# carlhenrikrolf/gym-cellular

Hardware: NVIDIA B200
Metric: env-steps/sec (higher is better)
Workload: dtype int8/int32 state, f32 reward

## Files before the change

gym_cellular_b200/_lib.py:

```python
import ctypes as C
import os

_PKG = os.path.dirname(os.path.abspath(__file__))
LIB_PATH = os.path.join(os.environ.get("GC_B200_LIB_DIR") or os.path.join(_PKG, "lib"), "libgymcellular_b200.so")

ABI_VERSION = 2
KIND_CELLULAR, KIND_GRIDWORLD = 0, 1
F_NOISE, F_RNG_EPISODIC, F_REWARD_LOG2, F_GENERIC_KERNEL = 1, 4, 16, 32
MAX_CELLS, MAX_LEVELS, N_STATS = 16, 8, 8
STAT_STEPS, STAT_UNSAFE, STAT_COUNT, STAT_TRUNCATED, STAT_REWARD_Q24 = range(5)
OK, ERR_INVALID, ERR_CUDA, ERR_STATE, ERR_ACTION = 0, -1, -2, -3, -4
POLICY_RANDOM, POLICY_TABLE = 0, 1

EXPORTS = ["gc_abi_version", "gc_last_error", "gc_create", "gc_destroy", "gc_set_tables", "gc_set_final_obs",
           "gc_set_global_step", "gc_get_global_step", "gc_sync_global_step", "gc_launch_count", "gc_reset", "gc_step",
           "gc_bind_step", "gc_step_bound", "gc_step_many", "gc_prepare_step_many", "gc_step_host", "gc_rollout", "gc_collect", "gc_poll_status", "gc_encode",
           "gc_decode", "gc_encode_mixed", "gc_decode_mixed", "gc_reset_packed", "gc_step_packed", "gc_bind_step_packed",
           "gc_step_host_packed", "gc_pack_cells", "gc_unpack_cells"]
FLAG_UNSAFE, FLAG_TRUNCATED, FLAG_COUNT_SHIFT = 1, 2, 2


class GcConfig(C.Structure):
    _fields_ = [("struct_size", C.c_uint32), ("kind", C.c_int32), ("device", C.c_int32),
                ("n_cells", C.c_int32), ("n_states", C.c_int32), ("n_actions", C.c_int32),
                ("max_episode_steps", C.c_int32), ("flags", C.c_uint32),
                ("n_envs", C.c_int64), ("ld", C.c_int64), ("env_id_offset", C.c_int64),
                ("seed", C.c_uint64), ("noise_prob", C.c_double), ("dispersal_prob", C.c_double)]


class GcCellTables(C.Structure):
    _fields_ = [("move", C.c_void_p), ("noisy", C.c_void_p), ("draws", C.c_void_p),
                ("reward", C.c_void_p), ("side_effects", C.c_void_p), ("counted", C.c_void_p),
                ("initial_state", C.c_void_p), ("reward_noisy", C.c_void_p), ("radix", C.c_void_p)]


class GcRecord(C.Structure):
    _fields_ = [("struct_size", C.c_uint32), ("obs", C.c_void_p), ("action", C.c_void_p), ("reward", C.c_void_p),
                ("flags", C.c_void_p), ("next_obs", C.c_void_p)]


class GcError(RuntimeError):
    def __init__(self, code, message):
        super().__init__(f"libgymcellular_b200 error {code}: {message}")
        self.code = code
        self.message = message


_lib = None


def load():
    global _lib
    if _lib is not None:
        return _lib
    if not os.path.exists(LIB_PATH):
        raise ImportError(
            f"{LIB_PATH} is missing: the CUDA extension has not been built and there is no CPU "
            "fallback.  Run `python -m gym_cellular_b200.build` (needs nvcc).")
    L = C.CDLL(LIB_PATH)
    vp, i64 = C.c_void_p, C.c_int64
    L.gc_abi_version.restype = C.c_int
    L.gc_last_error.restype = C.c_char_p
    L.gc_create.argtypes = [C.POINTER(GcConfig), C.POINTER(vp)]
    L.gc_destroy.argtypes = [vp]
    L.gc_set_tables.argtypes = [vp, C.POINTER(GcCellTables)]
    L.gc_set_final_obs.argtypes = [vp, vp]
    L.gc_set_global_step.argtypes = [vp, i64]
    L.gc_get_global_step.argtypes = [vp]
    L.gc_get_global_step.restype = i64
    L.gc_sync_global_step.argtypes = [vp, vp]
    L.gc_launch_count.argtypes = [vp]
    L.gc_launch_count.restype = i64
    L.gc_reset.argtypes = [vp] * 6
    L.gc_step.argtypes = [vp, i64, i64] + [vp] * 13
    L.gc_bind_step.argtypes = [vp, C.c_int32] + [vp] * 11
    L.gc_step_bound.argtypes = [vp, C.c_int32, vp]
    L.gc_step_host.argtypes = [vp] * 21 + [i64]
    L.gc_rollout.argtypes = [vp, C.c_int32, C.c_int32] + [vp] * 8
    L.gc_collect.argtypes = [vp, C.c_int32, C.c_int32, vp, C.c_double, vp, vp, vp, C.POINTER(GcRecord), vp, vp]
    L.gc_poll_status.argtypes = [vp, vp]
    L.gc_encode.argtypes = [C.c_int, i64, i64, C.c_int32, C.c_int32, vp, vp, vp]
    L.gc_decode.argtypes = [C.c_int, i64, i64, C.c_int32, C.c_int32, vp, vp, vp]
    i32 = C.c_int32
    L.gc_step_many.argtypes = [vp, vp, i32, i32, vp]
    L.gc_prepare_step_many.argtypes = [vp, vp, i32]
    L.gc_encode_mixed.argtypes = [C.c_int, i64, i64, i32, vp, vp, vp, vp, vp]
    L.gc_decode_mixed.argtypes = [C.c_int, i64, i64, i32, vp, vp, vp, vp, vp]
    L.gc_reset_packed.argtypes = [vp] * 6
    L.gc_step_packed.argtypes = [vp, i64, i64] + [vp] * 10
    L.gc_bind_step_packed.argtypes = [vp, i32] + [vp] * 9
    L.gc_step_host_packed.argtypes = [vp] * 13 + [i64]
    L.gc_pack_cells.argtypes = [C.c_int, i64, i64, i32, vp, vp, vp]
    L.gc_unpack_cells.argtypes = [C.c_int, i64, i64, i32, vp, vp, vp]
    if L.gc_abi_version() != ABI_VERSION:
        raise ImportError(f"ABI version mismatch: library {L.gc_abi_version()} != binding {ABI_VERSION}")
    _lib = L
    return L


def check(rc):
    if rc != 0:
        raise GcError(rc, load().gc_last_error().decode())
```

gym_cellular_b200/csrc/gc_api.cu:

```cuda
#include <cmath>
#include <cstdarg>
#include <cstdio>
#include <cstdlib>
#include <cstring>
#include <memory>
#include <new>

#include <nvtx3/nvToolsExt.h>

#include "gc_internal.h"

namespace {

thread_local char g_err[512] = "";

struct NvtxRange {
    explicit NvtxRange(const char *name) { nvtxRangePushA(name); }
    ~NvtxRange() { nvtxRangePop(); }
};
#define GC_NVTX(name) NvtxRange nvtx_range_(name)

int fail(int code, const char *fmt, ...)
{
    va_list ap;
    va_start(ap, fmt);
    vsnprintf(g_err, sizeof(g_err), fmt, ap);
    va_end(ap);
    return code;
}

#define GC_CUDA(call)                                                                         \
    do {                                                                                      \
        cudaError_t e_ = (call);                                                              \
        if (e_ != cudaSuccess)                                                                \
            return fail(GC_ERR_CUDA, "%s failed: %s (%s:%d)", #call, cudaGetErrorString(e_),   \
                        __FILE__, __LINE__);                                                  \
    } while (0)

constexpr int kHostStreams = 3;
constexpr int kManyGraphs = 4;
constexpr int kManyGraphSteps = 16;

class DeviceGuard {
public:
    explicit DeviceGuard(int device) : prev_(-1), err_(cudaSuccess)
    {
        err_ = cudaGetDevice(&prev_);
        if (err_ == cudaSuccess && prev_ != device) err_ = cudaSetDevice(device); else prev_ = -1;
    }
    ~DeviceGuard() { if (prev_ >= 0) cudaSetDevice(prev_); }
    cudaError_t error() const { return err_; }
private:
    int prev_;
    cudaError_t err_;
};

#define GC_ON_DEVICE(dev)                                                                      \
    DeviceGuard guard_(dev);                                                                   \
    if (guard_.error() != cudaSuccess)                                                         \
        return fail(GC_ERR_CUDA, "cannot switch to device %d: %s", (dev), cudaGetErrorString(guard_.error()))

unsigned long long threshold_of(double p)
{
    if (!(p > 0.0)) return 0ull;
    if (p >= 1.0) return 1ull << 32;
    return static_cast<unsigned long long>(std::ceil(p * 4294967296.0));
}

}

struct gc_env {
    gc_config cfg;
    CellTables tab;
    GridParams grid;
    bool tables_set;
    int n_sm;
    int64_t global_step;
    int64_t launches;
    unsigned long long *d_status;
    uint32_t *d_step;
    uint32_t *d_done;
    uint2 *d_pair_lut;
    uint2 *d_packed_lut;
    uint2 *d_pair8_lut;
    bool pair8_ok;
    int8_t *final_state;
    bool fast_ok;
    StepIO bound[GC_MAX_BINDINGS];
    PackedIO bound_packed[GC_MAX_BINDINGS];
    int bound_set[GC_MAX_BINDINGS];
    cudaStream_t hstream[kHostStreams];
    cudaEvent_t hevent[kHostStreams];
    bool host_ready;
    struct ManyGraph { int32_t slots[GC_MAX_BINDINGS]; int32_t n_slots, n_steps; cudaGraphExec_t exec; } many[kManyGraphs];
    int n_many;
};

namespace {

int check_env(const gc_env *env)
{
    if (!env) return fail(GC_ERR_INVALID, "env is NULL");
    return GC_OK;
}

int check_range(const gc_env *env, int64_t begin, int64_t count)
{
    const int64_t n = env->cfg.n_envs;
    if (begin < 0 || count < 0 || begin + count > n)
        return fail(GC_ERR_INVALID, "env range [%lld, %lld) outside [0, %lld)", (long long)begin,
                    (long long)(begin + count), (long long)n);
    if (begin % 16 != 0)
        return fail(GC_ERR_INVALID, "env_begin must be a multiple of 16");
    if ((begin + count) % 16 != 0 && begin + count != n)
        return fail(GC_ERR_INVALID, "env range must end on a multiple of 16 or at n_envs");
    return GC_OK;
}

StepIO make_io(const gc_env *env, int64_t begin, int64_t count, const int8_t *actions, int8_t *state,
               int32_t *t, float *reward, uint32_t *index, uint8_t *terminated, uint8_t *truncated,
               uint8_t *unsafe, uint8_t *count_out, int8_t *se_row, const double *replay, int64_t *stats)
{
    StepIO io;
    io.actions = actions; io.state = state; io.t = t; io.reward = reward; io.index = index;
    io.terminated = terminated; io.truncated = truncated; io.unsafe = unsafe; io.count = count_out;
    io.se_row = se_row; io.replay = replay;
    io.final_state = env->final_state;
    io.stats = reinterpret_cast<unsigned long long *>(stats);
    io.status = env->d_status;
    io.begin = begin; io.end = begin + count; io.ld = env->cfg.ld;
    io.env_id_offset = env->cfg.env_id_offset;
    io.seed_lo = static_cast<uint32_t>(env->cfg.seed);
    io.seed_hi = static_cast<uint32_t>(env->cfg.seed >> 32);
    for (int r = 0; r < 10; ++r) {
        io.round_key[2 * r] = io.seed_lo + static_cast<uint32_t>(r) * 0x9E3779B9u;
        io.round_key[2 * r + 1] = io.seed_hi + static_cast<uint32_t>(r) * 0xBB67AE85u;
    }
    io.rng_counter = static_cast<uint32_t>(env->global_step);
    io.step_ctr = env->d_step;
    io.done_ctr = nullptr;
    io.episodic = (env->cfg.flags & GC_F_RNG_EPISODIC) ? 1 : 0;
    io.max_episode_steps = env->cfg.max_episode_steps;
    return io;
}

PackedIO make_packed_io(const gc_env *env, int64_t begin, int64_t count, const uint32_t *actions, uint32_t *state,
                        int32_t *t, float *reward, uint32_t *index, uint8_t *flags, uint32_t *final_state,
                        uint32_t *se_row, int64_t *stats)
{
    PackedIO io;
    io.actions = actions; io.state = state; io.t = t; io.reward = reward; io.index = index; io.flags = flags;
    io.final_state = final_state; io.se_row = se_row;
    io.stats = reinterpret_cast<unsigned long long *>(stats);
    io.status = env->d_status;
    io.begin = begin; io.end = begin + count; io.ld = env->cfg.ld;
    io.env_id_offset = env->cfg.env_id_offset;
    const uint32_t lo = static_cast<uint32_t>(env->cfg.seed), hi = static_cast<uint32_t>(env->cfg.seed >> 32);
    for (int r = 0; r < 10; ++r) {
        io.round_key[2 * r] = lo + static_cast<uint32_t>(r) * 0x9E3779B9u;
        io.round_key[2 * r + 1] = hi + static_cast<uint32_t>(r) * 0xBB67AE85u;
    }
    io.rng_counter = static_cast<uint32_t>(env->global_step);
    io.step_ctr = env->d_step;
    io.done_ctr = nullptr;
    io.episodic = (env->cfg.flags & GC_F_RNG_EPISODIC) ? 1 : 0;
    io.max_episode_steps = env->cfg.max_episode_steps;
    return io;
}

int check_packed(const gc_env *env)
{
    if (env->cfg.kind != GC_KIND_CELLULAR || !env->fast_ok)
        return fail(GC_ERR_INVALID, "the packed layout covers the cellular family with n_states, n_actions <= 4 "
                                    "(and equal side-effect tables for the cells j >= 2)");
    return GC_OK;
}

int launch_packed(gc_env *env, const PackedIO &io, cudaStream_t st)
{
    if (io.end <= io.begin) return GC_OK;
    const bool draws = (env->cfg.flags & GC_F_NOISE) && env->tab.noise_thr_nz;
    cudaError_t e = gc_launch_cell_packed_step(env->tab, io, env->d_packed_lut, draws, env->n_sm, st);
    if (e != cudaSuccess) return fail(GC_ERR_CUDA, "packed step kernel launch failed: %s", cudaGetErrorString(e));
    env->launches += 1;
    return GC_OK;
}

void drop_many_graphs(gc_env *env)
{
    for (int i = 0; i < env->n_many; ++i)
        if (env->many[i].exec) cudaGraphExecDestroy(env->many[i].exec);
    env->n_many = 0;
}

struct HostDrain {
    gc_env *env;
    bool done = false;
    ~HostDrain()
    {
        if (done) return;
        for (int i = 0; i < kHostStreams; ++i) cudaStreamSynchronize(env->hstream[i]);
        cudaGetLastError();
    }
};

int host_streams(gc_env *env)
{
    if (!env->host_ready) {
        for (int i = 0; i < kHostStreams; ++i) {
            GC_CUDA(cudaStreamCreateWithFlags(&env->hstream[i], cudaStreamNonBlocking));
            GC_CUDA(cudaEventCreateWithFlags(&env->hevent[i], cudaEventDisableTiming));
        }
        env->host_ready = true;
    }
    return GC_OK;
}

int tick_global_step(gc_env *env, cudaStream_t st)
{
    cudaError_t e = gc_launch_tick(env->d_step, 1u, st);
    if (e != cudaSuccess) return fail(GC_ERR_CUDA, "step-counter kernel launch failed: %s", cudaGetErrorString(e));
    env->global_step += 1;
    return GC_OK;
}

int launch_step(gc_env *env, const StepIO &io, cudaStream_t st)
{
    if (io.end <= io.begin) return GC_OK;
    cudaError_t e;
    if (env->cfg.kind == GC_KIND_CELLULAR) {
        const bool draws = (env->cfg.flags & GC_F_NOISE) && env->tab.noise_thr_nz;
        const int mode = io.replay ? GC_RNG_REPLAY : (draws ? GC_RNG_PHILOX : GC_RNG_NONE);
        static const bool use_tma = [] { const char *v = std::getenv("GC_B200_TMA"); return v && v[0] == '1'; }();
        if (env->fast_ok && use_tma && mode == GC_RNG_NONE && !io.se_row && !io.final_state && env->cfg.n_cells >= 8)
            e = gc_launch_cell_tma_step(env->tab, io, env->d_pair_lut, env->n_sm, st);
        else if (env->fast_ok)
            e = gc_launch_cell_pair_step(env->tab, io, env->d_pair_lut, mode, env->n_sm, st);
        else if (env->pair8_ok && mode != GC_RNG_REPLAY)
            e = gc_launch_cell_pair8_step(env->tab, io, env->d_pair8_lut, mode, env->n_sm, st);
        else
            e = gc_launch_cell_step(env->tab, io, mode, env->n_sm, st);
    } else {
        e = gc_launch_grid_step(env->grid, io, io.replay ? GC_RNG_REPLAY : GC_RNG_PHILOX, env->n_sm, st);
    }
    if (e != cudaSuccess) return fail(GC_ERR_CUDA, "step kernel launch failed: %s", cudaGetErrorString(e));
    env->launches += 1;
    return GC_OK;
}

}

extern "C" {

int gc_abi_version(void) { return GC_ABI_VERSION; }

const char *gc_last_error(void) { return g_err; }

int gc_create(const gc_config *cfg, gc_env **out)
{
    GC_NVTX("gc_create");
    if (!cfg || !out) return fail(GC_ERR_INVALID, "cfg/out is NULL");
    if (cfg->struct_size != sizeof(gc_config))
        return fail(GC_ERR_INVALID, "gc_config.struct_size %u != %zu (ABI mismatch)", cfg->struct_size, sizeof(gc_config));
    if (cfg->n_envs < 1) return fail(GC_ERR_INVALID, "n_envs must be >= 1");
    if (cfg->ld < cfg->n_envs || cfg->ld % 16 != 0)
        return fail(GC_ERR_INVALID, "ld must be a multiple of 16 and >= n_envs");
    if (cfg->max_episode_steps < 0) return fail(GC_ERR_INVALID, "max_episode_steps must be >= 0");
    if (cfg->n_cells >= 1 && cfg->ld > (int64_t(1) << 31) / cfg->n_cells)
        return fail(GC_ERR_INVALID, "n_cells * ld must not exceed 2^31 (%d cells: at most %lld envs per handle)", cfg->n_cells,
                    (long long)((int64_t(1) << 31) / cfg->n_cells));
    if (cfg->env_id_offset < 0 || cfg->env_id_offset % 4 != 0)
        return fail(GC_ERR_INVALID, "env_id_offset must be a non-negative multiple of 4");
    if (cfg->kind == GC_KIND_CELLULAR) {
        if (cfg->n_cells < 1 || cfg->n_cells > GC_MAX_CELLS)
            return fail(GC_ERR_INVALID, "n_cells must be in 1..%d", GC_MAX_CELLS);
        if (cfg->n_states < 2 || cfg->n_states > GC_MAX_LEVELS || cfg->n_actions < 1 || cfg->n_actions > GC_MAX_LEVELS)
            return fail(GC_ERR_INVALID, "n_states must be in 2..%d and n_actions in 1..%d", GC_MAX_LEVELS, GC_MAX_LEVELS);
        if (cfg->n_cells * std::log2((double)cfg->n_states) > 32.0 + 1e-9)
            return fail(GC_ERR_INVALID, "n_states^n_cells does not fit the 32-bit tabular index");
    } else if (cfg->kind == GC_KIND_GRIDWORLD) {
        if (cfg->n_cells != 2 || cfg->n_states != 20 || cfg->n_actions != 5)
            return fail(GC_ERR_INVALID, "grid world is 2 jurisdictions x 20 codes x 5 actions");
    } else {
        return fail(GC_ERR_INVALID, "unknown kind %d", cfg->kind);
    }
    int n_dev = 0;
    GC_CUDA(cudaGetDeviceCount(&n_dev));
    if (cfg->device < 0 || cfg->device >= n_dev)
        return fail(GC_ERR_INVALID, "device %d not in [0, %d)", cfg->device, n_dev);
    GC_ON_DEVICE(cfg->device);
    int n_sm = 0;
    GC_CUDA(cudaDeviceGetAttribute(&n_sm, cudaDevAttrMultiProcessorCount, cfg->device));
    gc_env *env = new (std::nothrow) gc_env();
    if (!env) return fail(GC_ERR_INVALID, "out of host memory");
    std::memset(env, 0, sizeof(*env));
    env->cfg = *cfg;
    env->n_sm = n_sm;
    env->grid.dispersal_thr = threshold_of(cfg->dispersal_prob);
    env->grid.dispersal_thr_nz = env->grid.dispersal_thr != 0ull;
    env->grid.dispersal_thr_m1 = env->grid.dispersal_thr_nz ? static_cast<uint32_t>(env->grid.dispersal_thr - 1ull) : 0u;
    env->grid.dispersal_prob = cfg->dispersal_prob;
    env->tables_set = (cfg->kind == GC_KIND_GRIDWORLD);
    cudaError_t e = cudaMalloc(&env->d_status, 2 * sizeof(unsigned long long));
    if (e == cudaSuccess) e = cudaMemset(env->d_status, 0, 2 * sizeof(unsigned long long));
    if (e == cudaSuccess) {
        env->d_step = reinterpret_cast<uint32_t *>(env->d_status + 1);
        env->d_done = env->d_step + 1;
    }
    if (e == cudaSuccess && cfg->kind == GC_KIND_GRIDWORLD) {
        std::unique_ptr<uint32_t[]> lut(new (std::nothrow) uint32_t[GC_GRID_LUT_ENTRIES]);
        uint32_t *d_lut = nullptr;
        if (!lut) e = cudaErrorMemoryAllocation;
        if (e == cudaSuccess) {
            gc_build_grid_lut(lut.get());
            e = cudaMalloc(&d_lut, GC_GRID_LUT_ALLOC * sizeof(uint32_t));
        }
        if (e == cudaSuccess) e = cudaMemset(d_lut, 0, GC_GRID_LUT_ALLOC * sizeof(uint32_t));
        if (e == cudaSuccess) e = cudaMemcpy(d_lut, lut.get(), GC_GRID_LUT_ENTRIES * sizeof(uint32_t), cudaMemcpyHostToDevice);
        env->grid.lut = d_lut;
    }
    if (e != cudaSuccess) {
        if (env->d_status) cudaFree(env->d_status);
        if (env->grid.lut) cudaFree(const_cast<uint32_t *>(env->grid.lut));
        delete env;
        return fail(GC_ERR_CUDA, "device table allocation failed: %s", cudaGetErrorString(e));
    }
    *out = env;
    return GC_OK;
}

int gc_destroy(gc_env *env)
{
    if (!env) return GC_OK;
    DeviceGuard guard_(env->cfg.device);
    drop_many_graphs(env);
    if (env->host_ready)
        for (int i = 0; i < kHostStreams; ++i) {
            cudaStreamDestroy(env->hstream[i]);
            cudaEventDestroy(env->hevent[i]);
        }
    if (env->d_status) cudaFree(env->d_status);
    if (env->d_pair_lut) cudaFree(env->d_pair_lut);
    if (env->d_packed_lut) cudaFree(env->d_packed_lut);
    if (env->d_pair8_lut) cudaFree(env->d_pair8_lut);
    if (env->grid.lut) cudaFree(const_cast<uint32_t *>(env->grid.lut));
    delete env;
    return GC_OK;
}

int gc_set_tables(gc_env *env, const gc_cell_tables *t)
{
    GC_NVTX("gc_set_tables");
    if (int rc = check_env(env)) return rc;
    if (env->cfg.kind != GC_KIND_CELLULAR) return fail(GC_ERR_INVALID, "tables apply to the cellular family only");
    if (!t || !t->move || !t->reward || !t->side_effects || !t->counted || !t->initial_state)
        return fail(GC_ERR_INVALID, "move, reward, side_effects, counted and initial_state are required");
    const int C = env->cfg.n_cells, S = env->cfg.n_states, A = env->cfg.n_actions;
    const bool noise = (env->cfg.flags & GC_F_NOISE) != 0;
    if (noise && (!t->noisy || !t->draws)) return fail(GC_ERR_INVALID, "GC_F_NOISE needs the noisy and draws tables");
    CellTables tab;
    std::memset(&tab, 0, sizeof(tab));
    for (int s = 0; s < S; ++s)
        for (int a = 0; a < A; ++a) {
            const int mv = t->move[s * A + a];
            const int nz = t->noisy ? t->noisy[s * A + a] : mv;
            const int dr = (noise && t->draws) ? (t->draws[s * A + a] != 0) : 0;
            if (mv < 0 || mv >= S || nz < 0 || nz >= S)
                return fail(GC_ERR_INVALID, "move/noisy[%d][%d] outside [0, %d)", s, a, S);
            tab.sa[s * GC_LVL_PAD + a] = (uint32_t)mv | ((uint32_t)nz << 4) | ((uint32_t)dr << 8);
            tab.reward[s * GC_LVL_PAD + a] = t->reward[s * A + a];
            tab.reward_noisy[s * GC_LVL_PAD + a] = (t->reward_noisy ? t->reward_noisy : t->reward)[s * A + a];
        }
    for (int j = 0; j < C; ++j)
        for (int s0 = 0; s0 < S; ++s0)
            for (int sp = 0; sp < S; ++sp) {
                const int code = t->side_effects[(j * S + s0) * S + sp];
                if (code < 0 || code > 2) return fail(GC_ERR_INVALID, "side_effects code %d not in {0,1,2}", code);
                tab.se[j][s0 * GC_LVL_PAD + sp] = (uint8_t)code;
            }
    bool ragged = false;
    if (t->radix) {
        double bits = 0.0;
        for (int c = 0; c < C; ++c) {
            if (t->radix[c] < 1 || t->radix[c] > S) return fail(GC_ERR_INVALID, "radix[%d] = %d not in 1..n_states", c, t->radix[c]);
            bits += std::log2((double)t->radix[c]);
            ragged = ragged || t->radix[c] != S;
        }
        if (bits > 32.0 + 1e-9) return fail(GC_ERR_INVALID, "the ragged state space does not fit the 32-bit tabular index");
    }
    uint32_t place = 1, init_index = 0;
    for (int c = 0; c < C; ++c) {
        const int lv = t->initial_state[c];
        const int radix_c = t->radix ? t->radix[c] : S;
        if (lv < 0 || lv >= radix_c) return fail(GC_ERR_INVALID, "initial_state[%d] outside [0, %d)", c, radix_c);
        tab.place[c] = place;
        tab.init[c] = (int8_t)lv;
        init_index += (uint32_t)lv * place;
        place *= (uint32_t)radix_c;
    }
    tab.init_index = init_index;
    for (int s = 0; s < S; ++s) if (t->counted[s]) tab.counted_mask |= 1u << s;
    tab.n_cells = C; tab.n_states = S; tab.n_actions = A;
    tab.reward_log2 = (env->cfg.flags & GC_F_REWARD_LOG2) ? 1 : 0;
    tab.noise_thr = threshold_of(env->cfg.noise_prob);
    tab.noise_prob = env->cfg.noise_prob;

    tab.noise_thr_nz = tab.noise_thr != 0ull;
    tab.noise_thr_m1 = tab.noise_thr_nz ? static_cast<uint32_t>(tab.noise_thr - 1ull) : 0u;
    {
        uint32_t k16 = static_cast<uint32_t>(tab.noise_thr >> 16), r16 = static_cast<uint32_t>(tab.noise_thr & 0xFFFFull);
        if (k16 > 65535u) { k16 = 65535u; r16 = 1u << 16; }
        tab.noise_kk15 = (k16 & 0x7FFFu) * 0x00010001u;
        tab.noise_kmask = (k16 & 0x8000u) ? 0xFFFFFFFFu : 0u;
        tab.noise_kk = k16 * 0x00010001u;
        tab.noise_r16 = r16;
    }

    bool fast_ok = S <= 4 && A <= 4 && !ragged && !(env->cfg.flags & GC_F_GENERIC_KERNEL);
    for (int j = 3; j < C && fast_ok; ++j)
        if (std::memcmp(t->side_effects + (size_t)j * S * S, t->side_effects + (size_t)2 * S * S, (size_t)S * S) != 0)
            fast_ok = false;
    if (fast_ok) {
        uint2 lut[GC_PAIR_LUT_ENTRIES];
        gc_build_pair_lut(t, C, S, A, noise, lut, &tab.unsafe_rows);
        uint32_t p4 = 1;
        for (int i = 0; i < 4; ++i) { tab.place4[i] = p4; p4 *= (uint32_t)S; }
        GC_ON_DEVICE(env->cfg.device);
        if (!env->d_pair_lut) GC_CUDA(cudaMalloc(&env->d_pair_lut, sizeof(lut)));
        GC_CUDA(cudaMemcpy(env->d_pair_lut, lut, sizeof(lut), cudaMemcpyHostToDevice));
        gc_build_packed_lut(t, C, S, A, noise, lut);
        tab.init_packed = 0;
        for (int c = 0; c < C; ++c) tab.init_packed |= (uint32_t)(tab.init[c] & 3) << (2 * c);
        if (!env->d_packed_lut) GC_CUDA(cudaMalloc(&env->d_packed_lut, sizeof(lut)));
        GC_CUDA(cudaMemcpy(env->d_packed_lut, lut, sizeof(lut), cudaMemcpyHostToDevice));
    }
    bool pair8_ok = !fast_ok && S <= 8 && A <= 8 && !ragged && !(env->cfg.flags & GC_F_GENERIC_KERNEL);
    for (int j = 3; j < C && pair8_ok; ++j)
        if (std::memcmp(t->side_effects + (size_t)j * S * S, t->side_effects + (size_t)2 * S * S, (size_t)S * S) != 0)
            pair8_ok = false;
    if (pair8_ok) {
        std::unique_ptr<uint2[]> lut8(new (std::nothrow) uint2[GC_PAIR8_ENTRIES]);
        if (!lut8) return fail(GC_ERR_INVALID, "out of host memory");
        gc_build_pair8_lut(t, C, S, A, noise, lut8.get(), &tab.unsafe_rows8, &tab.unsafe01_rows8);
        GC_ON_DEVICE(env->cfg.device);
        if (!env->d_pair8_lut) GC_CUDA(cudaMalloc(&env->d_pair8_lut, GC_PAIR8_ENTRIES * sizeof(uint2)));
        GC_CUDA(cudaMemcpy(env->d_pair8_lut, lut8.get(), GC_PAIR8_ENTRIES * sizeof(uint2), cudaMemcpyHostToDevice));
    }
    drop_many_graphs(env);
    env->tab = tab;
    env->fast_ok = fast_ok;
    env->pair8_ok = pair8_ok;
    env->tables_set = true;
    return GC_OK;
}

int gc_set_final_obs(gc_env *env, int8_t *final_state)
{
    if (int rc = check_env(env)) return rc;
    env->final_state = final_state;
    drop_many_graphs(env);
    for (int i = 0; i < GC_MAX_BINDINGS; ++i)
        if (env->bound_set[i] == 1) env->bound[i].final_state = final_state;
    return GC_OK;
}

int gc_set_global_step(gc_env *env, int64_t step)
{
    if (int rc = check_env(env)) return rc;
    env->global_step = step;
    const uint32_t v = static_cast<uint32_t>(step);
    GC_ON_DEVICE(env->cfg.device);
    GC_CUDA(cudaMemcpy(env->d_step, &v, sizeof(v), cudaMemcpyHostToDevice));
    return GC_OK;
}

int64_t gc_get_global_step(const gc_env *env) { return env ? env->global_step : -1; }

int gc_sync_global_step(gc_env *env, void *stream)
{
    if (int rc = check_env(env)) return rc;
    GC_ON_DEVICE(env->cfg.device);
    uint32_t v = 0;
    GC_CUDA(cudaMemcpyAsync(&v, env->d_step, sizeof(v), cudaMemcpyDeviceToHost, static_cast<cudaStream_t>(stream)));
    GC_CUDA(cudaStreamSynchronize(static_cast<cudaStream_t>(stream)));
    env->global_step = (env->global_step & ~0xFFFFFFFFll) | v;
    return GC_OK;
}

int64_t gc_launch_count(const gc_env *env) { return env ? env->launches : -1; }

int gc_reset(gc_env *env, const uint8_t *mask, int8_t *state, int32_t *t, uint32_t *index, void *stream)
{
    GC_NVTX("gc_reset");
    if (int rc = check_env(env)) return rc;
    if (!env->tables_set) return fail(GC_ERR_STATE, "gc_set_tables has not been called");
    if (!state || !t) return fail(GC_ERR_INVALID, "state/t is NULL");
    GC_ON_DEVICE(env->cfg.device);
    int8_t init[GC_MAX_CELLS] = {0};
    uint32_t init_index;
    if (env->cfg.kind == GC_KIND_GRIDWORLD) {
        init[0] = 15; init[1] = 18; init_index = 15 + 20 * 18;
    } else {
        std::memcpy(init, env->tab.init, sizeof(init));
        init_index = env->tab.init_index;
    }
    const int64_t n_pad = (env->cfg.n_envs + 3) / 4 * 4;
    cudaError_t e = gc_launch_reset(env->cfg.n_cells, init, init_index, mask, state, t, index, n_pad,
                                    env->cfg.ld, static_cast<cudaStream_t>(stream));
    if (e != cudaSuccess) return fail(GC_ERR_CUDA, "reset kernel launch failed: %s", cudaGetErrorString(e));
    env->launches += 1;
    return GC_OK;
}

int gc_step(gc_env *env, int64_t env_begin, int64_t env_count, const int8_t *actions, int8_t *state,
            int32_t *t, float *reward, uint32_t *index, uint8_t *terminated, uint8_t *truncated,
            uint8_t *unsafe, uint8_t *count, int8_t *se_row, const double *replay_u, int64_t *stats,
            void *stream)
{
    GC_NVTX("gc_step");
    if (int rc = check_env(env)) return rc;
    if (!env->tables_set) return fail(GC_ERR_STATE, "gc_set_tables has not been called");
    if (!actions || !state || !t || !reward || !index || !terminated || !truncated || !unsafe || !count)
        return fail(GC_ERR_INVALID, "a required device pointer is NULL");
    if (int rc = check_range(env, env_begin, env_count)) return rc;
    GC_ON_DEVICE(env->cfg.device);
    StepIO io = make_io(env, env_begin, env_count, actions, state, t, reward, index, terminated,
                        truncated, unsafe, count, se_row, replay_u, stats);
    const bool full = env_begin == 0 && env_count == env->cfg.n_envs;
    if (full) io.done_ctr = env->d_done;
    if (int rc = launch_step(env, io, static_cast<cudaStream_t>(stream))) return rc;
    if (full) {
        env->global_step += 1;
    } else if (env_begin + env_count == env->cfg.n_envs) {
        if (int rc = tick_global_step(env, static_cast<cudaStream_t>(stream))) return rc;
    }
    return GC_OK;
}

int gc_bind_step(gc_env *env, int32_t slot, const int8_t *actions, int8_t *state, int32_t *t, float *reward,
                 uint32_t *index, uint8_t *terminated, uint8_t *truncated, uint8_t *unsafe, uint8_t *count,
                 int8_t *se_row, int64_t *stats)
{
    if (int rc = check_env(env)) return rc;
    if (slot < 0 || slot >= GC_MAX_BINDINGS) return fail(GC_ERR_INVALID, "slot must be in [0, %d)", GC_MAX_BINDINGS);
    if (!actions || !state || !t || !reward || !index || !terminated || !truncated || !unsafe || !count)
        return fail(GC_ERR_INVALID, "a required device pointer is NULL");
    env->bound[slot] = make_io(env, 0, env->cfg.n_envs, actions, state, t, reward, index, terminated, truncated,
                               unsafe, count, se_row, nullptr, stats);
    env->bound[slot].done_ctr = env->d_done;
    env->bound_set[slot] = 1;
    drop_many_graphs(env);
    return GC_OK;
}

namespace {
int launch_bound(gc_env *env, int32_t slot, cudaStream_t st)
{
    if (slot < 0 || slot >= GC_MAX_BINDINGS || !env->bound_set[slot])
        return fail(GC_ERR_INVALID, "no binding in slot %d", slot);
    if (int rc = env->bound_set[slot] == 2 ? launch_packed(env, env->bound_packed[slot], st)
                                           : launch_step(env, env->bound[slot], st))
        return rc;
    env->global_step += 1;
    return GC_OK;
}
}

int gc_step_bound(gc_env *env, int32_t slot, void *stream)
{
    if (!env) return fail(GC_ERR_INVALID, "gc_step_bound: env is NULL");
    if (!env->tables_set) return fail(GC_ERR_STATE, "gc_set_tables has not been called");
    GC_ON_DEVICE(env->cfg.device);
    return launch_bound(env, slot, static_cast<cudaStream_t>(stream));
}

namespace {
const gc_env::ManyGraph *many_graph(gc_env *env, const int32_t *slots, int32_t n_slots)
{
    for (int i = 0; i < env->n_many; ++i)
        if (env->many[i].n_slots == n_slots && std::memcmp(env->many[i].slots, slots, n_slots * sizeof(int32_t)) == 0)
            return &env->many[i];
    if (n_slots > GC_MAX_BINDINGS || host_streams(env) != GC_OK) return nullptr;
    if (env->n_many == kManyGraphs) drop_many_graphs(env);
    static const int graph_steps = [] {
        const char *v = std::getenv("GC_B200_STEP_MANY_GRAPH_STEPS");
        const int k = v ? std::atoi(v) : 0;
        return k > 0 ? k : kManyGraphSteps;
    }();
    const int32_t passes = (graph_steps + n_slots - 1) / n_slots;
    cudaStream_t cap = env->hstream[0];
    const int64_t launches = env->launches, step = env->global_step;
    if (cudaStreamBeginCapture(cap, cudaStreamCaptureModeRelaxed) != cudaSuccess) { cudaGetLastError(); return nullptr; }
    int rc = GC_OK;
    for (int32_t p = 0; p < passes && rc == GC_OK; ++p)
        for (int32_t i = 0; i < n_slots && rc == GC_OK; ++i) rc = launch_bound(env, slots[i], cap);
    cudaGraph_t graph = nullptr;
    cudaError_t e = cudaStreamEndCapture(cap, &graph);
    env->launches = launches; env->global_step = step;
    cudaGraphExec_t exec = nullptr;
    if (rc == GC_OK && e == cudaSuccess && graph) e = cudaGraphInstantiate(&exec, graph, 0);
    if (graph) cudaGraphDestroy(graph);
    if (rc != GC_OK || e != cudaSuccess || !exec) { cudaGetLastError(); return nullptr; }
    gc_env::ManyGraph &m = env->many[env->n_many++];
    std::memcpy(m.slots, slots, n_slots * sizeof(int32_t));
    m.n_slots = n_slots;
    m.n_steps = passes * n_slots;
    m.exec = exec;
    return &m;
}

constexpr int64_t kManyGraphMaxEnvs = 1 << 21;

bool many_graphs_enabled(const gc_env *env)
{
    static const bool on = [] { const char *v = std::getenv("GC_B200_STEP_MANY_GRAPH"); return !(v && v[0] == '0'); }();
    return on && env->cfg.n_envs <= kManyGraphMaxEnvs;
}

bool many_fusable(const gc_env *env, const int32_t *slots, int32_t n_slots)
{
    const char *v = std::getenv("GC_B200_STEP_MANY_FUSED");
    if ((v && v[0] == '0') || env->cfg.n_envs > kManyGraphMaxEnvs || env->final_state) return false;
    if (env->cfg.kind == GC_KIND_CELLULAR) {
        if (!env->fast_ok || env->cfg.n_cells > GC_MANY_MAX_CELLS) return false;
    }
    const int layout = env->bound_set[slots[0]];
    for (int32_t i = 0; i < n_slots; ++i)
        if (env->bound_set[slots[i]] != layout) return false;
    if (layout == 2) {
        if (env->cfg.kind != GC_KIND_CELLULAR) return false;
        const PackedIO &a = env->bound_packed[slots[0]];
        for (int32_t i = 1; i < n_slots; ++i) {
            const PackedIO &b = env->bound_packed[slots[i]];
            if (a.state != b.state || a.t != b.t || a.reward != b.reward || a.index != b.index || a.flags != b.flags ||
                a.se_row != b.se_row || a.stats != b.stats || a.final_state != b.final_state)
                return false;
        }
        return a.final_state == nullptr;
    }
    const StepIO &a = env->bound[slots[0]];
    for (int32_t i = 1; i < n_slots; ++i) {
        const StepIO &b = env->bound[slots[i]];
        if (a.state != b.state || a.t != b.t || a.reward != b.reward || a.index != b.index || a.terminated != b.terminated ||
            a.truncated != b.truncated || a.unsafe != b.unsafe || a.count != b.count || a.se_row != b.se_row ||
            a.stats != b.stats || a.final_state != b.final_state)
            return false;
    }
    return a.final_state == nullptr && a.replay == nullptr;
}

constexpr int32_t kManyFusedMaxSteps = 4096;

int launch_many_fused(gc_env *env, const int32_t *slots, int32_t n_slots, int32_t first, int32_t n_steps, cudaStream_t st)
{
    const bool draws = (env->cfg.flags & GC_F_NOISE) && env->tab.noise_thr_nz;
    if (env->bound_set[slots[0]] == 2) {
        PackedManyIO pio;
        pio.io = env->bound_packed[slots[0]];
        for (int32_t i = 0; i < GC_MAX_BINDINGS; ++i)
            pio.tape[i] = i < n_slots ? env->bound_packed[slots[(first + i) % n_slots]].actions : nullptr;
        pio.n_tape = n_slots;
        pio.n_steps = n_steps;
        const cudaError_t e = gc_launch_cell_packed_many(env->tab, pio, env->d_packed_lut, draws, env->n_sm, st);
        if (e != cudaSuccess) return fail(GC_ERR_CUDA, "many-step kernel launch failed: %s", cudaGetErrorString(e));
        env->launches += 1;
        env->global_step += n_steps;
        return GC_OK;
    }
    ManyIO mio;
    mio.io = env->bound[slots[0]];
    for (int32_t i = 0; i < n_slots; ++i) mio.tape[i] = env->bound[slots[(first + i) % n_slots]].actions;
    for (int32_t i = n_slots; i < GC_MAX_BINDINGS; ++i) mio.tape[i] = nullptr;
    mio.n_tape = n_slots;
    mio.n_steps = n_steps;
    const cudaError_t e = env->cfg.kind == GC_KIND_CELLULAR
        ? gc_launch_cell_pair_many(env->tab, mio, env->d_pair_lut, draws ? GC_RNG_PHILOX : GC_RNG_NONE, env->n_sm, st)
        : gc_launch_grid_many(env->grid, mio, env->n_sm, st);
    if (e != cudaSuccess) return fail(GC_ERR_CUDA, "many-step kernel launch failed: %s", cudaGetErrorString(e));
    env->launches += 1;
    env->global_step += n_steps;
    return GC_OK;
}
}

int gc_prepare_step_many(gc_env *env, const int32_t *slots, int32_t n_slots)
{
    if (!env || !slots || n_slots < 1) return fail(GC_ERR_INVALID, "gc_prepare_step_many: bad arguments");
    if (!env->tables_set) return fail(GC_ERR_STATE, "gc_set_tables has not been called");
    for (int32_t i = 0; i < n_slots; ++i)
        if (slots[i] < 0 || slots[i] >= GC_MAX_BINDINGS || !env->bound_set[slots[i]])
            return fail(GC_ERR_INVALID, "no binding in slot %d", slots[i]);
    GC_ON_DEVICE(env->cfg.device);
    if (n_slots <= GC_MAX_BINDINGS && many_fusable(env, slots, n_slots)) return GC_OK;
    if (many_graphs_enabled(env) && n_slots >= 2) many_graph(env, slots, n_slots);
    return GC_OK;
}

int gc_step_many(gc_env *env, const int32_t *slots, int32_t n_slots, int32_t n_steps, void *stream)
{
    GC_NVTX("gc_step_many");
    if (!env || !slots || n_slots < 1 || n_steps < 0) return fail(GC_ERR_INVALID, "gc_step_many: bad arguments");
    if (!env->tables_set) return fail(GC_ERR_STATE, "gc_set_tables has not been called");
    GC_ON_DEVICE(env->cfg.device);
    cudaStream_t st = static_cast<cudaStream_t>(stream);
    int32_t done = 0;
    for (int32_t i = 0; i < n_slots; ++i)
        if (slots[i] < 0 || slots[i] >= GC_MAX_BINDINGS || !env->bound_set[slots[i]])
            return fail(GC_ERR_INVALID, "no binding in slot %d", slots[i]);
    if (n_steps >= 2 && n_slots <= GC_MAX_BINDINGS && many_fusable(env, slots, n_slots)) {
        for (; done < n_steps;) {
            const int32_t k = n_steps - done < kManyFusedMaxSteps ? n_steps - done : kManyFusedMaxSteps;
            if (int rc = launch_many_fused(env, slots, n_slots, done % n_slots, k, st)) return rc;
            done += k;
        }
        return GC_OK;
    }
    cudaStreamCaptureStatus capturing = cudaStreamCaptureStatusNone;
    if (many_graphs_enabled(env) && n_slots >= 2 && n_steps >= 2 * n_slots &&
        cudaStreamIsCapturing(st, &capturing) == cudaSuccess && capturing == cudaStreamCaptureStatusNone) {
        if (const gc_env::ManyGraph *m = many_graph(env, slots, n_slots)) {
            for (; done + m->n_steps <= n_steps; done += m->n_steps) {
                GC_CUDA(cudaGraphLaunch(m->exec, st));
                env->launches += m->n_steps;
                env->global_step += m->n_steps;
            }
        }
    }
    for (int32_t i = done; i < n_steps; ++i)
        if (int rc = launch_bound(env, slots[i % n_slots], st)) return rc;
    return GC_OK;
}

int gc_step_host(gc_env *env, const int8_t *h_actions, int8_t *h_state, float *h_reward,
                 uint32_t *h_index, uint8_t *h_terminated, uint8_t *h_truncated, uint8_t *h_unsafe,
                 uint8_t *h_count, int8_t *h_se_row, int8_t *d_actions, int8_t *d_state, int32_t *d_t,
                 float *d_reward, uint32_t *d_index, uint8_t *d_terminated, uint8_t *d_truncated,
                 uint8_t *d_unsafe, uint8_t *d_count, int8_t *d_se_row, int64_t *d_stats,
                 int64_t chunk_envs)
{
    GC_NVTX("gc_step_host");
    if (int rc = check_env(env)) return rc;
    if (!env->tables_set) return fail(GC_ERR_STATE, "gc_set_tables has not been called");
    if (!h_actions || !d_actions || !d_state || !d_t || !d_reward || !d_index || !d_terminated ||
        !d_truncated || !d_unsafe || !d_count)
        return fail(GC_ERR_INVALID, "a required pointer is NULL");
    if (h_se_row && !d_se_row) return fail(GC_ERR_INVALID, "h_se_row needs d_se_row");
    GC_ON_DEVICE(env->cfg.device);
    if (int rc = host_streams(env)) return rc;
    const int64_t n = env->cfg.n_envs, ld = env->cfg.ld;
    const int C = env->cfg.n_cells;
    if (chunk_envs <= 0) chunk_envs = 1 << 20;
    chunk_envs = (chunk_envs + 15) / 16 * 16;
    HostDrain drain{env};
    int k = 0;
    for (int64_t b = 0; b < n; b += chunk_envs, ++k) {
        const int64_t cnt = (b + chunk_envs < n) ? chunk_envs : (n - b);
        const int64_t cnt_pad = (cnt + 3) / 4 * 4;
        cudaStream_t st = env->hstream[k % kHostStreams];
        GC_CUDA(cudaMemcpy2DAsync(d_actions + b, ld, h_actions + b, ld, cnt_pad, C, cudaMemcpyHostToDevice, st));
        const StepIO io = make_io(env, b, cnt, d_actions, d_state, d_t, d_reward, d_index, d_terminated,
                                  d_truncated, d_unsafe, d_count, d_se_row, nullptr, d_stats);
        if (int rc = launch_step(env, io, st)) return rc;
        if (h_state) GC_CUDA(cudaMemcpy2DAsync(h_state + b, ld, d_state + b, ld, cnt, C, cudaMemcpyDeviceToHost, st));
        if (h_reward) GC_CUDA(cudaMemcpyAsync(h_reward + b, d_reward + b, cnt * sizeof(float), cudaMemcpyDeviceToHost, st));
        if (h_index) GC_CUDA(cudaMemcpyAsync(h_index + b, d_index + b, cnt * sizeof(uint32_t), cudaMemcpyDeviceToHost, st));
        if (h_terminated) GC_CUDA(cudaMemcpyAsync(h_terminated + b, d_terminated + b, cnt, cudaMemcpyDeviceToHost, st));
        if (h_truncated) GC_CUDA(cudaMemcpyAsync(h_truncated + b, d_truncated + b, cnt, cudaMemcpyDeviceToHost, st));
        if (h_unsafe) GC_CUDA(cudaMemcpyAsync(h_unsafe + b, d_unsafe + b, cnt, cudaMemcpyDeviceToHost, st));
        if (h_count) GC_CUDA(cudaMemcpyAsync(h_count + b, d_count + b, cnt, cudaMemcpyDeviceToHost, st));
        if (h_se_row)
            GC_CUDA(cudaMemcpy2DAsync(h_se_row + b, ld, d_se_row + b, ld, cnt, C, cudaMemcpyDeviceToHost, st));
    }
    for (int i = 0; i < kHostStreams && i < k; ++i) GC_CUDA(cudaStreamSynchronize(env->hstream[i]));
    if (int rc = tick_global_step(env, env->hstream[0])) return rc;
    GC_CUDA(cudaStreamSynchronize(env->hstream[0]));
    drain.done = true;
    return GC_OK;
}

namespace {

RolloutIO make_rollout_io(const gc_env *env, int32_t n_steps, int32_t policy_kind, const int32_t *policy, int8_t *state,
                          int32_t *t, uint32_t *index, int64_t *stats)
{
    RolloutIO io;
    std::memset(&io, 0, sizeof(io));
    io.state = state; io.t = t; io.index = index; io.policy = policy;
    io.stats = reinterpret_cast<unsigned long long *>(stats);
    io.status = env->d_status;
    io.n = env->cfg.n_envs; io.ld = env->cfg.ld; io.env_id_offset = env->cfg.env_id_offset;
    const uint32_t lo = static_cast<uint32_t>(env->cfg.seed), hi = static_cast<uint32_t>(env->cfg.seed >> 32);
    for (int r = 0; r < 10; ++r) {
        io.round_key[2 * r] = lo + static_cast<uint32_t>(r) * 0x9E3779B9u;
        io.round_key[2 * r + 1] = hi + static_cast<uint32_t>(r) * 0xBB67AE85u;
    }
    io.step_ctr = env->d_step; io.done_ctr = env->d_done;
    io.episodic = (env->cfg.flags & GC_F_RNG_EPISODIC) ? 1 : 0;
    io.max_episode_steps = env->cfg.max_episode_steps;
    io.n_steps = n_steps; io.policy_kind = policy_kind;
    return io;
}

bool misaligned(const void *p) { return p && (reinterpret_cast<uintptr_t>(p) & 15u) != 0; }

}

int gc_rollout(gc_env *env, int32_t n_steps, int32_t policy_kind, const int32_t *policy, int8_t *state,
               int32_t *t, uint32_t *index, float *ret, int32_t *n_unsafe, int64_t *stats, void *stream)
{
    GC_NVTX("gc_rollout");
    if (int rc = check_env(env)) return rc;
    if (!env->tables_set) return fail(GC_ERR_STATE, "gc_set_tables has not been called");
    if (!state || !t || !index || !ret || !n_unsafe) return fail(GC_ERR_INVALID, "a required device pointer is NULL");
    if (n_steps < 1) return fail(GC_ERR_INVALID, "n_steps must be >= 1");
    if (policy_kind != GC_POLICY_RANDOM && policy_kind != GC_POLICY_TABLE) return fail(GC_ERR_INVALID, "unknown policy kind");
    if (policy_kind == GC_POLICY_TABLE && !policy) return fail(GC_ERR_INVALID, "GC_POLICY_TABLE needs a policy table");
    if (env->cfg.kind == GC_KIND_CELLULAR && !env->fast_ok)
        return fail(GC_ERR_INVALID, "gc_rollout supports the cellular family with n_states, n_actions <= 4 only");
    GC_ON_DEVICE(env->cfg.device);
    RolloutIO io = make_rollout_io(env, n_steps, policy_kind, policy, state, t, index, stats);
    io.ret = ret; io.n_unsafe = n_unsafe;
    cudaError_t e;
    if (env->cfg.kind == GC_KIND_CELLULAR)
        e = gc_launch_cell_rollout(env->tab, io, env->d_pair_lut, (env->cfg.flags & GC_F_NOISE) != 0, env->n_sm,
                                   static_cast<cudaStream_t>(stream));
    else
        e = gc_launch_grid_rollout(env->grid, io, env->n_sm, static_cast<cudaStream_t>(stream));
    if (e != cudaSuccess) return fail(GC_ERR_CUDA, "rollout kernel launch failed: %s", cudaGetErrorString(e));
    env->launches += 1;
    env->global_step += n_steps;
    return GC_OK;
}


int gc_collect(gc_env *env, int32_t n_steps, int32_t policy_kind, const int32_t *policy, double epsilon,
               int8_t *state, int32_t *t, uint32_t *index, const gc_record *record, int64_t *stats, void *stream)
{
    GC_NVTX("gc_collect");
    if (int rc = check_env(env)) return rc;
    if (!env->tables_set) return fail(GC_ERR_STATE, "gc_set_tables has not been called");
    if (!state || !t || !index || !record) return fail(GC_ERR_INVALID, "a required pointer is NULL");
    if (n_steps < 1) return fail(GC_ERR_INVALID, "n_steps must be >= 1");
    if (policy_kind != GC_POLICY_RANDOM && policy_kind != GC_POLICY_TABLE) return fail(GC_ERR_INVALID, "unknown policy kind");
    if (policy_kind == GC_POLICY_TABLE && !policy) return fail(GC_ERR_INVALID, "GC_POLICY_TABLE needs a policy table");
    if (!(epsilon >= 0.0 && epsilon <= 1.0)) return fail(GC_ERR_INVALID, "epsilon must lie in [0, 1] (got %g)", epsilon);
    if (policy_kind == GC_POLICY_RANDOM && epsilon != 0.0)
        return fail(GC_ERR_INVALID, "epsilon applies to GC_POLICY_TABLE only (GC_POLICY_RANDOM needs epsilon 0)");
    if (record->struct_size != sizeof(gc_record))
        return fail(GC_ERR_INVALID, "record->struct_size %u != sizeof(gc_record) %zu", record->struct_size, sizeof(gc_record));
    if (misaligned(record->obs) || misaligned(record->action) || misaligned(record->reward) || misaligned(record->flags) ||
        misaligned(record->next_obs))
        return fail(GC_ERR_INVALID, "record pointers must be 16-byte aligned");
    if (env->cfg.kind == GC_KIND_CELLULAR && !env->fast_ok)
        return fail(GC_ERR_INVALID, "gc_collect supports the cellular family with n_states, n_actions <= 4 only");
    GC_ON_DEVICE(env->cfg.device);
    RolloutIO io = make_rollout_io(env, n_steps, policy_kind, policy, state, t, index, stats);
    io.rec_obs = record->obs; io.rec_action = record->action; io.rec_reward = record->reward;
    io.rec_flags = record->flags; io.rec_next_obs = record->next_obs;
    unsigned long long joint = 1;
    for (int c = 0; c < env->cfg.n_cells; ++c) joint *= static_cast<unsigned long long>(env->cfg.n_actions);
    io.joint_actions = joint;
    const unsigned long long thr = threshold_of(epsilon);
    io.explore_thr_nz = thr != 0 ? 1u : 0u;
    io.explore_thr_m1 = static_cast<uint32_t>(thr - 1);
    cudaError_t e;
    if (env->cfg.kind == GC_KIND_CELLULAR)
        e = gc_launch_cell_collect(env->tab, io, env->d_pair_lut, (env->cfg.flags & GC_F_NOISE) != 0, env->n_sm,
                                   static_cast<cudaStream_t>(stream));
    else
        e = gc_launch_grid_collect(env->grid, io, env->n_sm, static_cast<cudaStream_t>(stream));
    if (e != cudaSuccess) return fail(GC_ERR_CUDA, "collect kernel launch failed: %s", cudaGetErrorString(e));
    env->launches += 1;
    env->global_step += n_steps;
    return GC_OK;
}

int gc_poll_status(gc_env *env, void *stream)
{
    GC_NVTX("gc_poll_status");
    if (int rc = check_env(env)) return rc;
    GC_ON_DEVICE(env->cfg.device);
    unsigned long long word = 0;
    cudaStream_t st = static_cast<cudaStream_t>(stream);
    GC_CUDA(cudaMemcpyAsync(&word, env->d_status, sizeof(word), cudaMemcpyDeviceToHost, st));
    GC_CUDA(cudaStreamSynchronize(st));
    if (word) {
        GC_CUDA(cudaMemsetAsync(env->d_status, 0, sizeof(word), st));
        return fail(GC_ERR_ACTION, "'position': a grid-world action named no go-to position in any jurisdiction");
    }
    return GC_OK;
}

int gc_encode(int device, int64_t n, int64_t ld, int32_t n_cells, int32_t radix, const int8_t *cells,
              uint32_t *index, void *stream)
{
    if (!cells || !index || n < 0 || ld < n || ld % 16 != 0 || n_cells < 1 || radix < 1)
        return fail(GC_ERR_INVALID, "gc_encode: bad arguments");
    GC_ON_DEVICE(device);
    cudaError_t e = gc_launch_encode((n + 3) / 4 * 4, ld, n_cells, (uint32_t)radix, cells, index,
                                     static_cast<cudaStream_t>(stream));
    if (e != cudaSuccess) return fail(GC_ERR_CUDA, "encode kernel launch failed: %s", cudaGetErrorString(e));
// ... 172 lines not shown
```

gym_cellular_b200/csrc/gc_cell_fast.cu:

```cuda
#include "gc_device.cuh"

namespace {


#ifndef GC_PAIR_MINB
#define GC_PAIR_MINB 4
#endif
#ifndef GC_PAIR_MINB_NARROW
#define GC_PAIR_MINB_NARROW GC_PAIR_MINB
#endif
constexpr int pair_min_blocks(int c, int rng)
{
#ifdef GC_PAIR_MINB_ALL
    return GC_PAIR_MINB_ALL;
#endif
    if (rng != GC_RNG_NONE && c > 4) return 3;
    if (rng == GC_RNG_NONE && ((c >= 4 && c <= 8) || c == 10 || c == 11)) return GC_PAIR_MINB < 3 ? GC_PAIR_MINB : 3;
    return c < 4 ? GC_PAIR_MINB_NARROW : GC_PAIR_MINB;
}

#ifndef GC_PAIR_REP_LOG2
#define GC_PAIR_REP_LOG2 0
#endif
#ifndef GC_PAIR_REP_MIN_C
#define GC_PAIR_REP_MIN_C 12
#endif
__host__ __device__ constexpr int pair_rep_log2(int c, int rng)
{
    return (rng == GC_RNG_NONE && c >= GC_PAIR_REP_MIN_C) ? GC_PAIR_REP_LOG2 : 0;
}

struct EnvAcc {
    float r[kEPT];
    uint32_t sum01, sum23;
    uint32_t or01, or23;
    uint32_t idx[kEPT];
    uint32_t s0w, s1w;
};

template <int N, int C, int RNG, bool WITH_SE, bool FIRST>
__device__ __forceinline__ void do_cells(const CellTables &tab, const StepIO &io, const uint2 *s_pair,
                                         const uint2 *s_single, const uint8_t (*s_se)[GC_TBL], int c0,
                                         uint32_t e0, int rem, uint32_t gid_lo, uint32_t gid_hi, uint32_t step_counter,
                                         const int (&tin)[kEPT], uint32_t keep, const uint32_t (&sw)[4],
                                         const uint32_t (&aw)[4], const uint32_t (&fire16)[kEPT], EnvAcc &acc,
                                         uint32_t (&next)[4])
{
    uint32_t fb[kEPT] = {0, 0, 0, 0};
    if (RNG == GC_RNG_PHILOX && C > GC_NARROW_CELLS) {
#pragma unroll
        for (int e = 0; e < kEPT; ++e) fb[e] = (fire16[e] >> c0) & 15u;
    } else if (RNG == GC_RNG_PHILOX) {
#pragma unroll
        for (int e = 0; e < kEPT; ++e) {
            uint32_t w[4];
            const uint32_t ctr = io.episodic ? static_cast<uint32_t>(tin[e]) : step_counter;
            philox4x32_10(gid_lo | e, gid_hi, ctr, static_cast<uint32_t>(c0 >> 2), io.round_key, w);
            const uint32_t thr = tab.noise_thr_m1;
            fb[e] = (w[0] <= thr ? 1u : 0u) | (w[1] <= thr ? 2u : 0u) | (w[2] <= thr ? 4u : 0u) | (w[3] <= thr ? 8u : 0u);
        }
    } else if (RNG == GC_RNG_REPLAY) {
#pragma unroll
        for (int e = 0; e < kEPT; ++e)
            if (e < rem)
#pragma unroll
                for (int i = 0; i < N; ++i)
                    fb[e] |= (io.replay[static_cast<size_t>(e0 + e) * C + c0 + i] < tab.noise_prob ? 1u : 0u) << i;
    }
    const uint32_t ld = static_cast<uint32_t>(io.ld);
    uint32_t q = 0;
    uint32_t rows[4];
#pragma unroll
    for (int i = 0; i < N; i += 2) {
        const bool pair = i + 1 < N;
        uint32_t inf[kEPT];
        if (pair) {
            const uint32_t pidx = ((aw[i + 1] & 0x03030303u) * 4u + (sw[i + 1] & 0x03030303u)) * 16u +
                                  (aw[i] & 0x03030303u) * 4u + (sw[i] & 0x03030303u);
#pragma unroll
            for (int e = 0; e < kEPT; ++e) {
                uint32_t ix = byte_of(pidx, e);
                if (RNG != GC_RNG_NONE) ix |= ((fb[e] >> i) & 3u) << 8;
                const uint2 ent = s_pair[ix << pair_rep_log2(C, RNG)];
                if (FIRST && i == 0) acc.r[e] = __uint_as_float(ent.y); else acc.r[e] += __uint_as_float(ent.y);
                inf[e] = ent.x;
            }
        } else {
            const uint32_t sidx = (aw[i] & 0x03030303u) * 4u + (sw[i] & 0x03030303u);
#pragma unroll
            for (int e = 0; e < kEPT; ++e) {
                uint32_t ix = byte_of(sidx, e) & 15u;
                if (RNG != GC_RNG_NONE) ix |= ((fb[e] >> i) & 1u) << 4;
                const uint2 ent = s_single[ix];
                if (FIRST && i == 0) acc.r[e] = __uint_as_float(ent.y); else acc.r[e] += __uint_as_float(ent.y);
                inf[e] = ent.x;
            }
        }
        const uint32_t w01 = prmt(inf[0], inf[1], 0x5410), w23 = prmt(inf[2], inf[3], 0x5410);
        acc.sum01 += w01; acc.sum23 += w23;
        const uint32_t keep_bits = (FIRST && i == 0) ? 0x10001000u : 0x0F000F00u;
        acc.or01 |= w01 & keep_bits; acc.or23 |= w23 & keep_bits;
        const uint32_t u = prmt(inf[0], inf[1], 0x7362), v = prmt(inf[2], inf[3], 0x7362);
        rows[i] = prmt(u, v, 0x5410);
        if (pair) rows[i + 1] = prmt(u, v, 0x7632);
        if (FIRST && i == 0) { acc.s0w = rows[0]; acc.s1w = pair ? rows[1] : rows[0]; }
    }
#pragma unroll
    for (int i = 0; i < N; ++i) {
        if (WITH_SE) {
            uint32_t sew = 0;
#pragma unroll
            for (int e = 0; e < kEPT; ++e) {
                const uint32_t s0n = byte_of(acc.s0w, e);
                const uint32_t partner = (FIRST && i == 0) ? byte_of(acc.s1w, e) : byte_of(rows[i], e);
                sew |= static_cast<uint32_t>(s_se[c0 + i][(s0n * GC_LVL_PAD + partner) & (GC_TBL - 1)]) << (8 * e);
            }
            st_stream_u32(io.se_row + ((c0 + i) * ld + e0), sew);
        }
        const uint32_t out = (rows[i] & keep) | ((0x01010101u * static_cast<uint8_t>(tab.init[c0 + i])) & ~keep);
        next[i] = out;
        st_stream_u32(io.state + ((c0 + i) * ld + e0), out);
        if (io.final_state) st_stream_u32(io.final_state + ((c0 + i) * ld + e0), rows[i]);
        q += out * tab.place4[i];
    }
    const uint32_t place = tab.place[c0];
#pragma unroll
    for (int e = 0; e < kEPT; ++e) acc.idx[e] += byte_of(q, e) * place;
}

template <int N>
__device__ __forceinline__ void load_cells(const StepIO &io, int c0, uint32_t e0, uint32_t (&sw)[4], uint32_t (&aw)[4])
{
    const uint32_t ld = static_cast<uint32_t>(io.ld);
#pragma unroll
    for (int i = 0; i < N; ++i) {
        sw[i] = ld_stream_u32(io.state + ((c0 + i) * ld + e0));
        aw[i] = ld_stream_u32(io.actions + ((c0 + i) * ld + e0));
    }
}

template <int C, int RNG, bool WITH_SE>
__global__ void __launch_bounds__(kThreads, pair_min_blocks(C, RNG))
cell_pair_kernel(const __grid_constant__ CellTables tab, const __grid_constant__ StepIO io,
                 const uint2 *__restrict__ lut)
{
    constexpr int NG = C / 4, R = C % 4;
    constexpr int N_PAIR = (RNG == GC_RNG_NONE) ? 256 : GC_PAIR_LUT_PAIRS;
    constexpr int N_SINGLE = (RNG == GC_RNG_NONE) ? 16 : 32;
    constexpr int REP_LOG2 = pair_rep_log2(C, RNG), REP = 1 << REP_LOG2;
    __shared__ uint2 s_pair_all[N_PAIR * REP];
    const uint2 *const s_pair = s_pair_all + (threadIdx.x & (REP - 1));
    __shared__ uint2 s_single[N_SINGLE];
    __shared__ uint8_t s_se[WITH_SE ? C : 1][GC_TBL];
    __shared__ unsigned long long s_stats[5];

    __shared__ StepCounterShared s_ctr;

    const uint32_t stride = gridDim.x * kThreads * kEPT, e_end = static_cast<uint32_t>(io.end);
#ifndef GC_PAIR_PREFETCH_WIDE
#define GC_PAIR_PREFETCH_WIDE 0
#endif
    constexpr bool PREFETCH = NG == 0 || GC_PAIR_PREFETCH_WIDE;
    constexpr int G0 = NG > 0 ? 4 : R;
    uint32_t e0 = static_cast<uint32_t>(io.begin) + (blockIdx.x * kThreads + threadIdx.x) * kEPT;
    constexpr int LUT_PER_THREAD = N_PAIR / kThreads;
    uint2 lut_pair[LUT_PER_THREAD], lut_single = make_uint2(0u, 0u);
#pragma unroll
    for (int k = 0; k < LUT_PER_THREAD; ++k) lut_pair[k] = lut[threadIdx.x + k * kThreads];
    if (threadIdx.x < N_SINGLE) lut_single = lut[GC_PAIR_LUT_PAIRS + threadIdx.x];
    pdl_launch_dependents();
    pdl_wait();
    uint32_t ps[4], pa[4];
    int4 pt = make_int4(0, 0, 0, 0);
    if constexpr (PREFETCH) if (e0 < e_end) {
        load_cells<G0>(io, 0, e0, ps, pa);
        pt = ld_stream_v4(io.t + e0);
    }
    step_counter_read(io, &s_ctr);
#pragma unroll
    for (int k = 0; k < LUT_PER_THREAD; ++k)
#pragma unroll
        for (int r = 0; r < REP; ++r) s_pair_all[((threadIdx.x + k * kThreads) << REP_LOG2) + r] = lut_pair[k];
    if (threadIdx.x < N_SINGLE) s_single[threadIdx.x] = lut_single;
    if (WITH_SE)
        for (int i = threadIdx.x; i < C * GC_TBL; i += kThreads) s_se[i / GC_TBL][i % GC_TBL] = tab.se[i / GC_TBL][i % GC_TBL];
    if (threadIdx.x < 5) s_stats[threadIdx.x] = 0;
    __syncthreads();

    const uint32_t step_now = step_counter_arrive(io, &s_ctr);
    const uint32_t step_counter = (RNG == GC_RNG_PHILOX) ? step_now : 0u;
    uint32_t st_steps = 0, st_unsafe = 0, st_count = 0, st_trunc = 0;
    long long st_reward = 0;
#pragma unroll 1
    for (; e0 < e_end; e0 += stride) {
        const int rem = static_cast<int>(e_end - e0 < kEPT ? e_end - e0 : kEPT);
        const uint64_t gid0 = static_cast<uint64_t>(io.env_id_offset) + e0;
        const uint32_t gid_lo = static_cast<uint32_t>(gid0), gid_hi = static_cast<uint32_t>(gid0 >> 32);

        uint32_t sa[4], aa[4], sb[4], ab[4];
        int4 t4;
        if constexpr (PREFETCH) {
#pragma unroll
            for (int i = 0; i < 4; ++i) { sa[i] = ps[i]; aa[i] = pa[i]; }
            t4 = pt;
            if (NG > 1) load_cells<4>(io, 4, e0, sb, ab); else if (NG == 1 && R > 0) load_cells<R>(io, 4, e0, sb, ab);
            if (e0 + stride < e_end) {
                load_cells<G0>(io, 0, e0 + stride, ps, pa);
                pt = ld_stream_v4(io.t + (e0 + stride));
            }
        } else {
            load_cells<4>(io, 0, e0, sa, aa);
            t4 = ld_stream_v4(io.t + e0);
            if (NG > 1) load_cells<4>(io, 4, e0, sb, ab); else if (R > 0) load_cells<R>(io, 4, e0, sb, ab);
        }

        const int tin[kEPT] = {t4.x, t4.y, t4.z, t4.w};
        int tn[kEPT] = {t4.x + 1, t4.y + 1, t4.z + 1, t4.w + 1};
        uint32_t trunc_w = 0, keep = 0xFFFFFFFFu;
        if (io.max_episode_steps > 0) {
#pragma unroll
            for (int e = 0; e < kEPT; ++e)
                if (tn[e] >= io.max_episode_steps) { tn[e] = 0; trunc_w |= 1u << (8 * e); keep &= ~(0xFFu << (8 * e)); }
        }
        uint32_t fire16[kEPT] = {0, 0, 0, 0};
        if (RNG == GC_RNG_PHILOX && C > GC_NARROW_CELLS) {
#pragma unroll
            for (int e = 0; e < kEPT; ++e)
                fire16[e] = fire_bits_wide<(C + 7) / 8>(tab, gid_lo | e, gid_hi, io.episodic ? static_cast<uint32_t>(tin[e]) : step_counter,
                                                        io.round_key);
        }
        EnvAcc acc;
#pragma unroll
        for (int e = 0; e < kEPT; ++e) { acc.r[e] = 0.f; acc.idx[e] = 0; }
        acc.sum01 = acc.sum23 = acc.or01 = acc.or23 = acc.s0w = acc.s1w = 0;
        uint32_t nx[4];

        if (NG == 0) {
            do_cells<R, C, RNG, WITH_SE, true>(tab, io, s_pair, s_single, s_se, 0, e0, rem, gid_lo, gid_hi, step_counter, tin, keep, sa, aa, fire16, acc, nx);
        } else {
            do_cells<4, C, RNG, WITH_SE, true>(tab, io, s_pair, s_single, s_se, 0, e0, rem, gid_lo, gid_hi, step_counter, tin, keep, sa, aa, fire16, acc, nx);
#pragma unroll 1
            for (int g = 1; g < NG; ++g) {
#pragma unroll
                for (int i = 0; i < 4; ++i) { sa[i] = sb[i]; aa[i] = ab[i]; }
                if (g + 1 < NG) load_cells<4>(io, 4 * (g + 1), e0, sb, ab);
                else if (R > 0) load_cells<R>(io, 4 * NG, e0, sb, ab);
                do_cells<4, C, RNG, WITH_SE, false>(tab, io, s_pair, s_single, s_se, 4 * g, e0, rem, gid_lo, gid_hi, step_counter, tin, keep, sa, aa, fire16, acc, nx);
            }
            if (R > 0)
                do_cells<R, C, RNG, WITH_SE, false>(tab, io, s_pair, s_single, s_se, 4 * NG, e0, rem, gid_lo, gid_hi, step_counter, tin, keep, sb, ab, fire16, acc, nx);
        }

        float rout[kEPT];
        log2_1p_x4(tab.reward_log2, acc.r, rout);
        const uint32_t count_w = prmt(acc.sum01, acc.sum23, 0x6420) & 0x1F1F1F1Fu;
        const uint32_t present = prmt(acc.or01, acc.or23, 0x7531);
        const uint32_t nib = acc.s0w | (acc.s0w >> 4);
        const uint32_t rowmask = prmt(tab.unsafe_rows, 0u, prmt(nib, 0u, 0x4420) & 0x3333u);
        const uint32_t unsafe_w = ((((present & rowmask) + 0x0F0F0F0Fu) | present) >> 4) & 0x01010101u;
#pragma unroll
        for (int e = 0; e < kEPT; ++e)
            if (e < rem) st_reward += __float2int_rn(rout[e] * 16777216.0f);
        {
            const uint32_t vb = valid_bytes(rem);
            st_steps += rem;
            st_unsafe = add_bytes(unsafe_w & vb, st_unsafe);
            st_count = add_bytes(count_w & vb, st_count);
            st_trunc = add_bytes(trunc_w & vb, st_trunc);
        }
        st_stream_v4(io.t + e0, make_int4(tn[0], tn[1], tn[2], tn[3]));
        st_stream_v4(io.reward + e0, make_int4(__float_as_int(rout[0]), __float_as_int(rout[1]),
                                               __float_as_int(rout[2]), __float_as_int(rout[3])));
        st_stream_v4(io.index + e0, make_int4(acc.idx[0], acc.idx[1], acc.idx[2], acc.idx[3]));
        st_stream_u32(io.terminated + e0, 0u);
        st_stream_u32(io.truncated + e0, trunc_w);
        st_stream_u32(io.unsafe + e0, unsafe_w);
        st_stream_u32(io.count + e0, count_w);
    }
    if (io.stats) {
        const ThreadStats ts = {st_steps, st_unsafe, st_count, st_trunc, st_reward};
        block_flush_stats(ts, s_stats, io.stats);
    }
    step_counter_finish(io, &s_ctr);
}

template <int C, int RNG>
cudaError_t launch_pair_cr(const CellTables &tab, const StepIO &io, const uint2 *lut, int n_sm, cudaStream_t st)
{
    const int64_t n = io.end - io.begin;
    if (io.se_row)
        return launch_step_kernel(cell_pair_kernel<C, RNG, true>, grid_for<cell_pair_kernel<C, RNG, true>>(n, n_sm), kThreads, 0, st, tab, io, lut);
    else
        return launch_step_kernel(cell_pair_kernel<C, RNG, false>, grid_for<cell_pair_kernel<C, RNG, false>>(n, n_sm), kThreads, 0, st, tab, io, lut);
    return cudaGetLastError();
}

#ifndef GC_MANY_SMALL_THREADS
#define GC_MANY_SMALL_THREADS 64
#endif
template <int C, int RNG, bool WITH_SE, int THREADS>
__global__ void __launch_bounds__(THREADS, 256 / THREADS * 2)
cell_pair_many_kernel(const __grid_constant__ CellTables tab, const __grid_constant__ ManyIO mio, const uint2 *__restrict__ lut)
{
    const StepIO &io = mio.io;
    constexpr int NG = C / 4, R = C % 4, G = (C + 3) / 4;
    constexpr int N_PAIR = (RNG == GC_RNG_NONE) ? 256 : GC_PAIR_LUT_PAIRS;
    constexpr int N_SINGLE = (RNG == GC_RNG_NONE) ? 16 : 32;
    __shared__ uint2 s_pair[N_PAIR];
    __shared__ uint2 s_single[N_SINGLE];
    __shared__ uint8_t s_se[WITH_SE ? C : 1][GC_TBL];
    __shared__ unsigned long long s_stats[5];
    __shared__ StepCounterShared s_ctr;

    for (int i = threadIdx.x; i < N_PAIR; i += THREADS) s_pair[i] = lut[i];
    if (threadIdx.x < N_SINGLE) s_single[threadIdx.x] = lut[GC_PAIR_LUT_PAIRS + threadIdx.x];
    if (WITH_SE)
        for (int i = threadIdx.x; i < C * GC_TBL; i += THREADS) s_se[i / GC_TBL][i % GC_TBL] = tab.se[i / GC_TBL][i % GC_TBL];
    if (threadIdx.x < 5) s_stats[threadIdx.x] = 0;
    pdl_launch_dependents();
    pdl_wait();
    step_counter_read(io, &s_ctr);
    __syncthreads();
    const uint32_t step0 = step_counter_arrive(io, &s_ctr);

    const uint32_t ld = static_cast<uint32_t>(io.ld);
    const uint32_t stride = gridDim.x * THREADS * kEPT, e_end = static_cast<uint32_t>(io.end);
    uint32_t st_steps = 0, st_unsafe = 0, st_count = 0, st_trunc = 0;
    long long st_reward = 0;
#pragma unroll 1
    for (uint32_t e0 = static_cast<uint32_t>(io.begin) + (blockIdx.x * THREADS + threadIdx.x) * kEPT; e0 < e_end; e0 += stride) {
        const int rem = static_cast<int>(e_end - e0 < kEPT ? e_end - e0 : kEPT);
        const uint64_t gid0 = static_cast<uint64_t>(io.env_id_offset) + e0;
        const uint32_t gid_lo = static_cast<uint32_t>(gid0), gid_hi = static_cast<uint32_t>(gid0 >> 32);
        uint32_t sw[G][4], an[G][4];
#pragma unroll
        for (int c = 0; c < C; ++c) {
            sw[c / 4][c % 4] = ld_stream_u32(io.state + (c * ld + e0));
            an[c / 4][c % 4] = ld_stream_u32(mio.tape[0] + (c * ld + e0));
        }
        const int4 t4 = ld_stream_v4(io.t + e0);
        int t[kEPT] = {t4.x, t4.y, t4.z, t4.w};
        int slot = 0;
#pragma unroll 1
        for (int k = 0; k < mio.n_steps; ++k) {
            uint32_t aa[G][4];
#pragma unroll
            for (int c = 0; c < C; ++c) aa[c / 4][c % 4] = an[c / 4][c % 4];
            slot = slot + 1 == mio.n_tape ? 0 : slot + 1;
            if (k + 1 < mio.n_steps) {
                const int8_t *const nxt = mio.tape[slot];
#pragma unroll
                for (int c = 0; c < C; ++c) an[c / 4][c % 4] = ld_stream_u32(nxt + (c * ld + e0));
            }
            const int tin[kEPT] = {t[0], t[1], t[2], t[3]};
            int tn[kEPT] = {t[0] + 1, t[1] + 1, t[2] + 1, t[3] + 1};
            uint32_t trunc_w = 0, keep = 0xFFFFFFFFu;
            if (io.max_episode_steps > 0) {
#pragma unroll
                for (int e = 0; e < kEPT; ++e)
                    if (tn[e] >= io.max_episode_steps) { tn[e] = 0; trunc_w |= 1u << (8 * e); keep &= ~(0xFFu << (8 * e)); }
            }
            const uint32_t step_counter = (RNG == GC_RNG_PHILOX) ? step0 + static_cast<uint32_t>(k) : 0u;
            uint32_t fire16[kEPT] = {0, 0, 0, 0};
            if (RNG == GC_RNG_PHILOX && C > GC_NARROW_CELLS) {
#pragma unroll
                for (int e = 0; e < kEPT; ++e)
                    fire16[e] = fire_bits_wide<(C + 7) / 8>(tab, gid_lo | e, gid_hi, io.episodic ? static_cast<uint32_t>(tin[e]) : step_counter,
                                                            io.round_key);
            }
            EnvAcc acc;
#pragma unroll
            for (int e = 0; e < kEPT; ++e) { acc.r[e] = 0.f; acc.idx[e] = 0; }
            acc.sum01 = acc.sum23 = acc.or01 = acc.or23 = acc.s0w = acc.s1w = 0;
            uint32_t nx[G][4];
            if constexpr (NG == 0) {
                do_cells<R, C, RNG, WITH_SE, true>(tab, io, s_pair, s_single, s_se, 0, e0, rem, gid_lo, gid_hi, step_counter, tin, keep, sw[0], aa[0], fire16, acc, nx[0]);
            } else {
                do_cells<4, C, RNG, WITH_SE, true>(tab, io, s_pair, s_single, s_se, 0, e0, rem, gid_lo, gid_hi, step_counter, tin, keep, sw[0], aa[0], fire16, acc, nx[0]);
#pragma unroll
                for (int g = 1; g < NG; ++g)
                    do_cells<4, C, RNG, WITH_SE, false>(tab, io, s_pair, s_single, s_se, 4 * g, e0, rem, gid_lo, gid_hi, step_counter, tin, keep, sw[g], aa[g], fire16, acc, nx[g]);
                if constexpr (R > 0)
                    do_cells<R, C, RNG, WITH_SE, false>(tab, io, s_pair, s_single, s_se, 4 * NG, e0, rem, gid_lo, gid_hi, step_counter, tin, keep, sw[NG], aa[NG], fire16, acc, nx[NG]);
            }
            float rout[kEPT];
            log2_1p_x4(tab.reward_log2, acc.r, rout);
            const uint32_t count_w = prmt(acc.sum01, acc.sum23, 0x6420) & 0x1F1F1F1Fu;
            const uint32_t present = prmt(acc.or01, acc.or23, 0x7531);
            const uint32_t nib = acc.s0w | (acc.s0w >> 4);
            const uint32_t rowmask = prmt(tab.unsafe_rows, 0u, prmt(nib, 0u, 0x4420) & 0x3333u);
            const uint32_t unsafe_w = ((((present & rowmask) + 0x0F0F0F0Fu) | present) >> 4) & 0x01010101u;
#pragma unroll
            for (int e = 0; e < kEPT; ++e)
                if (e < rem) st_reward += __float2int_rn(rout[e] * 16777216.0f);
            {
                const uint32_t vb = valid_bytes(rem);
                st_steps += rem;
                st_unsafe = add_bytes(unsafe_w & vb, st_unsafe);
                st_count = add_bytes(count_w & vb, st_count);
                st_trunc = add_bytes(trunc_w & vb, st_trunc);
            }
            st_stream_v4(io.t + e0, make_int4(tn[0], tn[1], tn[2], tn[3]));
            st_stream_v4(io.reward + e0, make_int4(__float_as_int(rout[0]), __float_as_int(rout[1]),
                                                   __float_as_int(rout[2]), __float_as_int(rout[3])));
            st_stream_v4(io.index + e0, make_int4(acc.idx[0], acc.idx[1], acc.idx[2], acc.idx[3]));
            st_stream_u32(io.terminated + e0, 0u);
            st_stream_u32(io.truncated + e0, trunc_w);
            st_stream_u32(io.unsafe + e0, unsafe_w);
            st_stream_u32(io.count + e0, count_w);
#pragma unroll
            for (int c = 0; c < C; ++c) sw[c / 4][c % 4] = nx[c / 4][c % 4];
#pragma unroll
            for (int e = 0; e < kEPT; ++e) t[e] = tn[e];
        }
    }
    if (io.stats) {
        const ThreadStats ts = {st_steps, st_unsafe, st_count, st_trunc, st_reward};
        block_flush_stats(ts, s_stats, io.stats);
    }
    if (threadIdx.x == 0 && io.done_ctr != nullptr && s_ctr.arrived == gridDim.x - 1) {
        *io.done_ctr = 0u;
        *const_cast<uint32_t *>(io.step_ctr) = s_ctr.step + static_cast<uint32_t>(mio.n_steps);
    }
}

template <int C, int RNG, bool WITH_SE, int THREADS>
cudaError_t launch_pair_many_t(const CellTables &tab, const ManyIO &mio, const uint2 *lut, int n_sm, cudaStream_t st)
{
    const int64_t n = mio.io.end - mio.io.begin;
    return launch_step_kernel(cell_pair_many_kernel<C, RNG, WITH_SE, THREADS>,
                              grid_for<cell_pair_many_kernel<C, RNG, WITH_SE, THREADS>, THREADS>(n, n_sm), THREADS, 0, st, tab, mio, lut);
}

template <int C, int RNG>
cudaError_t launch_pair_many_cr(const CellTables &tab, const ManyIO &mio, const uint2 *lut, int n_sm, cudaStream_t st)
{
    const int64_t n = mio.io.end - mio.io.begin;
    const bool small = (n + kThreads * kEPT - 1) / (kThreads * kEPT) < n_sm;
    if (mio.io.se_row)
        return small ? launch_pair_many_t<C, RNG, true, GC_MANY_SMALL_THREADS>(tab, mio, lut, n_sm, st)
                     : launch_pair_many_t<C, RNG, true, kThreads>(tab, mio, lut, n_sm, st);
    return small ? launch_pair_many_t<C, RNG, false, GC_MANY_SMALL_THREADS>(tab, mio, lut, n_sm, st)
                 : launch_pair_many_t<C, RNG, false, kThreads>(tab, mio, lut, n_sm, st);
}

template <int C>
cudaError_t launch_pair_c(const CellTables &tab, const StepIO &io, const uint2 *lut, int rng_mode, int n_sm,
                          cudaStream_t st)
{
    switch (rng_mode) {
    case GC_RNG_NONE: return launch_pair_cr<C, GC_RNG_NONE>(tab, io, lut, n_sm, st);
    case GC_RNG_PHILOX: return launch_pair_cr<C, GC_RNG_PHILOX>(tab, io, lut, n_sm, st);
    default: return launch_pair_cr<C, GC_RNG_REPLAY>(tab, io, lut, n_sm, st);
    }
}

}

cudaError_t gc_launch_cell_pair_step(const CellTables &tab, const StepIO &io, const uint2 *lut, int rng_mode,
                                     int n_sm, cudaStream_t st)
{
    switch (tab.n_cells) {
#define GC_CASE(C) case C: return launch_pair_c<C>(tab, io, lut, rng_mode, n_sm, st);
        GC_CASE(1) GC_CASE(2) GC_CASE(3) GC_CASE(4) GC_CASE(5) GC_CASE(6) GC_CASE(7) GC_CASE(8)
        GC_CASE(9) GC_CASE(10) GC_CASE(11) GC_CASE(12) GC_CASE(13) GC_CASE(14) GC_CASE(15) GC_CASE(16)
#undef GC_CASE
    default: return cudaErrorInvalidValue;
    }
}

cudaError_t gc_launch_cell_pair_many(const CellTables &tab, const ManyIO &mio, const uint2 *lut, int rng_mode, int n_sm,
                                     cudaStream_t st)
{
    if (rng_mode != GC_RNG_NONE && rng_mode != GC_RNG_PHILOX) return cudaErrorInvalidValue;
    switch (tab.n_cells) {
#define GC_CASE(C) case C: return rng_mode == GC_RNG_PHILOX ? launch_pair_many_cr<C, GC_RNG_PHILOX>(tab, mio, lut, n_sm, st) \
                                                            : launch_pair_many_cr<C, GC_RNG_NONE>(tab, mio, lut, n_sm, st);
        GC_CASE(1) GC_CASE(2) GC_CASE(3) GC_CASE(4) GC_CASE(5) GC_CASE(6) GC_CASE(7) GC_CASE(8)
#undef GC_CASE
    default: return cudaErrorInvalidValue;
    }
}
```

gym_cellular_b200/csrc/gc_cell_packed.cu:

```cuda
#include "gc_device.cuh"

namespace {

constexpr int kPackThreads = 256;

__device__ __forceinline__ uint32_t bitselect(uint32_t a, uint32_t b, uint32_t m)
{
    uint32_t d;
    asm("lop3.b32 %0, %1, %2, %3, 0xE4;" : "=r"(d) : "r"(a), "r"(b), "r"(m));
    return d;
}

__device__ __forceinline__ uint2 lds64(uint32_t addr)
{
    uint2 v;
    asm("ld.shared.v2.u32 {%0, %1}, [%2];" : "=r"(v.x), "=r"(v.y) : "r"(addr));
    return v;
}

#ifndef GC_PACKED_MINB
#define GC_PACKED_MINB 4
#endif

__host__ __device__ constexpr int packed_rep_log2(int rng, bool big) { return big ? (rng == GC_RNG_NONE ? 4 : 2) : 0; }
__host__ __device__ constexpr int packed_pairs(int rng) { return rng == GC_RNG_NONE ? 256 : GC_PAIR_LUT_PAIRS; }
__host__ __device__ constexpr int packed_singles(int rng) { return rng == GC_RNG_NONE ? 16 : 32; }
constexpr size_t packed_smem_bytes(int rng, bool big)
{
    return (static_cast<size_t>(packed_pairs(rng) + packed_singles(rng)) << packed_rep_log2(rng, big)) * sizeof(uint2) +
           GC_MAX_CELLS * GC_TBL;
}

__host__ __device__ constexpr int packed_min_blocks(int c, int rng, bool extra)
{
    return (rng != GC_RNG_NONE || extra || c == 15) ? (GC_PACKED_MINB < 3 ? GC_PACKED_MINB : 3) : GC_PACKED_MINB;
}

template <int C, int RNG, bool EXTRA>
__device__ __forceinline__ void packed_word(const CellTables &tab, const PackedIO &io, const uint8_t (*s_se)[GC_TBL],
                                            uint32_t pair_base, uint32_t single_base, uint32_t lut_mul, uint32_t e0, int rem,
                                            uint32_t gid_lo, uint32_t gid_hi, uint32_t step_counter,
                                            const uint32_t (&sw4)[kEPT], const uint32_t (&aw4)[kEPT], const int (&tin)[kEPT],
                                            uint32_t &st_steps, uint32_t &st_unsafe, uint32_t &st_count, uint32_t &st_trunc,
                                            long long &st_reward, uint32_t (&nstate)[kEPT], int (&tn)[kEPT])
{
    constexpr int NP = C / 2;
    constexpr bool ODD = (C & 1) != 0;
    uint32_t fin[kEPT], idx[kEPT], sew[kEPT];
    uint32_t flags_w = 0;
    float rew[kEPT];
#pragma unroll
    for (int e = 0; e < kEPT; ++e) {
        const uint32_t sw = sw4[e], aw = aw4[e];
        uint32_t fire = 0;
        if (RNG == GC_RNG_PHILOX) {
            const uint32_t ctr = io.episodic ? static_cast<uint32_t>(tin[e]) : step_counter;
            if (C > GC_NARROW_CELLS) {
                fire = fire_bits_wide<(C + 7) / 8>(tab, gid_lo | e, gid_hi, ctr, io.round_key);
            } else {
                const uint32_t thr = tab.noise_thr_m1;
                uint32_t w[4];
                philox4x32_10(gid_lo | e, gid_hi, ctr, 0u, io.round_key, w);
                fire = (w[0] <= thr ? 1u : 0u) | (w[1] <= thr ? 2u : 0u) | (w[2] <= thr ? 4u : 0u) | (w[3] <= thr ? 8u : 0u);
            }
        }
        const uint32_t x = bitselect(aw << 4, sw, 0xF0F0F0F0u);
        const uint32_t y = bitselect(aw, sw >> 4, 0xF0F0F0F0u);
        constexpr int NL = NP + (ODD ? 1 : 0);
        uint32_t info[NL];
        float r = 0.f;
#pragma unroll
        for (int i = 0; i < NP; ++i) {
            uint32_t ix = prmt((i & 1) ? y : x, 0u, 0x4440u + (i >> 1));
            if (RNG != GC_RNG_NONE) ix |= ((fire >> (2 * i)) & 3u) << 8;
            const uint2 ent = lds64(ix * lut_mul + pair_base);
            r = (i == 0) ? __uint_as_float(ent.y) : r + __uint_as_float(ent.y);
            info[i] = ent.x;
        }
        if (ODD) {
            const uint32_t b = prmt((NP & 1) ? y : x, 0u, 0x4440u + (NP >> 1));
            uint32_t ix = (b & 3u) | ((b >> 2) & 12u);
            if (RNG != GC_RNG_NONE) ix |= ((fire >> (2 * NP)) & 1u) << 4;
            const uint2 ent = lds64(ix * lut_mul + single_base);
            r = (NP == 0) ? __uint_as_float(ent.y) : r + __uint_as_float(ent.y);
            info[NP] = ent.x;
        }
        uint32_t ns = 0, acc = 0;
#pragma unroll
        for (int i = NL - 1; i >= 0; --i) {
            ns = __funnelshift_l(info[i], ns, 4);
            acc += info[i];
        }
        const uint32_t lv = acc - info[0];
        const uint32_t uns2 = ((lv >> (5u * (ns & 3u))) & 31u) ? 1u : 0u;
        const uint32_t uns = ((info[0] >> 25) & 1u) | uns2;
        const uint32_t cnt = (acc >> 20) & 31u;
        uint32_t se_code = 0;
        if (EXTRA && io.se_row) {
            const uint32_t s0n = ns & 3u;
#pragma unroll
            for (int j = 0; j < C; ++j) {
                const uint32_t p = (j == 0) ? (C > 1 ? 1 : 0) : j;
                const uint32_t sp = (ns >> (2 * p)) & 3u;
                se_code |= static_cast<uint32_t>(s_se[j][s0n * GC_LVL_PAD + sp]) << (2 * j);
            }
        }
        nstate[e] = ns; tn[e] = tin[e] + 1;
        if (EXTRA) { fin[e] = ns; sew[e] = se_code; }
        rew[e] = r;
        flags_w |= (uns | (cnt << 2)) << (8 * e);
    }
    if (io.max_episode_steps > 0) {
#pragma unroll
        for (int e = 0; e < kEPT; ++e)
            if (tn[e] >= io.max_episode_steps) { tn[e] = 0; nstate[e] = tab.init_packed; flags_w |= 2u << (8 * e); }
    }
#pragma unroll
    for (int e = 0; e < kEPT; ++e) {
        const uint32_t out = nstate[e];
        if (EXTRA) {
            uint32_t ix = out;
            if (io.index && tab.n_states != 4) {
                ix = 0;
#pragma unroll
                for (int c = 0; c < C; ++c) ix += ((out >> (2 * c)) & 3u) * tab.place[c];
            }
            idx[e] = ix;
        }
    }
    float rout[kEPT];
    log2_1p_x4(tab.reward_log2, rew, rout);
#pragma unroll
    for (int e = 0; e < kEPT; ++e)
        if (e < rem) st_reward += __float2int_rn(rout[e] * 16777216.0f);
    {
        const uint32_t fw = flags_w & valid_bytes(rem);
        st_steps += rem;
        st_unsafe += __popc(fw & 0x01010101u);
        st_trunc += __popc(fw & 0x02020202u);
        st_count = add_bytes((fw >> 2) & 0x1F1F1F1Fu, st_count);
    }
    st_stream_v4(io.state + e0, make_int4(nstate[0], nstate[1], nstate[2], nstate[3]));
    st_stream_v4(io.t + e0, make_int4(tn[0], tn[1], tn[2], tn[3]));
    st_stream_v4(io.reward + e0, make_int4(__float_as_int(rout[0]), __float_as_int(rout[1]),
                                           __float_as_int(rout[2]), __float_as_int(rout[3])));
    st_stream_u32(io.flags + e0, flags_w);
    if (EXTRA) {
        if (io.index) st_stream_v4(io.index + e0, make_int4(idx[0], idx[1], idx[2], idx[3]));
        if (io.final_state) st_stream_v4(io.final_state + e0, make_int4(fin[0], fin[1], fin[2], fin[3]));
        if (io.se_row) st_stream_v4(io.se_row + e0, make_int4(sew[0], sew[1], sew[2], sew[3]));
    } else if (io.index) {
        st_stream_v4(io.index + e0, make_int4(nstate[0], nstate[1], nstate[2], nstate[3]));
    }
}

template <int C, int RNG, bool EXTRA>
__global__ void __launch_bounds__(kPackThreads, packed_min_blocks(C, RNG, EXTRA))
cell_packed_kernel(const __grid_constant__ CellTables tab, const __grid_constant__ PackedIO io,
                   const uint2 *__restrict__ lut, const int REP_LOG2)
{
    constexpr int N_PAIR = packed_pairs(RNG), N_SINGLE = packed_singles(RNG);
    extern __shared__ __align__(16) uint2 s_tab[];
    uint2 *const s_pair = s_tab;
    uint2 *const s_single = s_tab + (N_PAIR << REP_LOG2);
    uint8_t (*const s_se)[GC_TBL] = reinterpret_cast<uint8_t (*)[GC_TBL]>(s_single + (N_SINGLE << REP_LOG2));
    __shared__ unsigned long long s_stats[5];
    __shared__ StepCounterShared s_ctr;
    const uint32_t REP = 1u << REP_LOG2;

    const uint32_t stride = gridDim.x * kPackThreads * kEPT, e_end = static_cast<uint32_t>(io.end);
    uint32_t e0 = static_cast<uint32_t>(io.begin) + (blockIdx.x * kPackThreads + threadIdx.x) * kEPT;
    for (int i = threadIdx.x; i < (N_PAIR << REP_LOG2); i += kPackThreads) s_pair[i] = lut[i >> REP_LOG2];
    for (int i = threadIdx.x; i < (N_SINGLE << REP_LOG2); i += kPackThreads) s_single[i] = lut[GC_PAIR_LUT_PAIRS + (i >> REP_LOG2)];
    if (EXTRA && io.se_row)
        for (int i = threadIdx.x; i < C * GC_TBL; i += kPackThreads) s_se[i / GC_TBL][i % GC_TBL] = tab.se[i / GC_TBL][i % GC_TBL];
    if (threadIdx.x < 5) s_stats[threadIdx.x] = 0;
    pdl_launch_dependents();
    pdl_wait();
    int4 ps = make_int4(0, 0, 0, 0), pa = ps, pt = ps;
    if (e0 < e_end) {
        ps = ld_stream_v4(io.state + e0);
        pa = ld_stream_v4(io.actions + e0);
        pt = ld_stream_v4(io.t + e0);
    }
    step_counter_read(io, &s_ctr);
    __syncthreads();
    const uint32_t step_now = step_counter_arrive(io, &s_ctr);
    const uint32_t step_counter = (RNG == GC_RNG_PHILOX) ? step_now : 0u;
    const uint32_t rep = threadIdx.x & (REP - 1u);
    const uint32_t lut_mul = 8u << REP_LOG2;
    const uint32_t pair_base = static_cast<uint32_t>(__cvta_generic_to_shared(s_pair)) + rep * 8u;
    const uint32_t single_base = static_cast<uint32_t>(__cvta_generic_to_shared(s_single)) + rep * 8u;

    uint32_t st_steps = 0, st_unsafe = 0, st_count = 0, st_trunc = 0;
    long long st_reward = 0;
    for (; e0 < e_end; e0 += stride) {
        const int rem = static_cast<int>(e_end - e0 < kEPT ? e_end - e0 : kEPT);
        const uint64_t gid0 = static_cast<uint64_t>(io.env_id_offset) + e0;
        const uint32_t gid_lo = static_cast<uint32_t>(gid0), gid_hi = static_cast<uint32_t>(gid0 >> 32);
        const uint32_t sw4[kEPT] = {(uint32_t)ps.x, (uint32_t)ps.y, (uint32_t)ps.z, (uint32_t)ps.w};
        const uint32_t aw4[kEPT] = {(uint32_t)pa.x, (uint32_t)pa.y, (uint32_t)pa.z, (uint32_t)pa.w};
        const int tin[kEPT] = {pt.x, pt.y, pt.z, pt.w};
        if (e0 + stride < e_end) {
            ps = ld_stream_v4(io.state + (e0 + stride));
            pa = ld_stream_v4(io.actions + (e0 + stride));
            pt = ld_stream_v4(io.t + (e0 + stride));
        }
        uint32_t nstate[kEPT];
        int tn[kEPT];
        packed_word<C, RNG, EXTRA>(tab, io, s_se, pair_base, single_base, lut_mul, e0, rem, gid_lo, gid_hi, step_counter, sw4, aw4, tin,
                                   st_steps, st_unsafe, st_count, st_trunc, st_reward, nstate, tn);
    }
    if (io.stats) {
        const ThreadStats ts = {st_steps, st_unsafe, st_count, st_trunc, st_reward};
        block_flush_stats(ts, s_stats, io.stats);
    }
    step_counter_finish(io, &s_ctr);
}

#ifndef GC_MANY_SMALL_THREADS
#define GC_MANY_SMALL_THREADS 64
#endif
template <int C, int RNG, bool EXTRA, int THREADS>
__global__ void __launch_bounds__(THREADS, 256 / THREADS * 2)
cell_packed_many_kernel(const __grid_constant__ CellTables tab, const __grid_constant__ PackedManyIO mio,
                        const uint2 *__restrict__ lut, const int REP_LOG2)
{
    const PackedIO &io = mio.io;
    constexpr int N_PAIR = packed_pairs(RNG), N_SINGLE = packed_singles(RNG);
    extern __shared__ __align__(16) uint2 s_tab[];
    uint2 *const s_pair = s_tab;
    uint2 *const s_single = s_tab + (N_PAIR << REP_LOG2);
    uint8_t (*const s_se)[GC_TBL] = reinterpret_cast<uint8_t (*)[GC_TBL]>(s_single + (N_SINGLE << REP_LOG2));
    __shared__ unsigned long long s_stats[5];
    __shared__ StepCounterShared s_ctr;
    const uint32_t REP = 1u << REP_LOG2;
    const uint32_t stride = gridDim.x * THREADS * kEPT, e_end = static_cast<uint32_t>(io.end);
    for (int i = threadIdx.x; i < (N_PAIR << REP_LOG2); i += THREADS) s_pair[i] = lut[i >> REP_LOG2];
    for (int i = threadIdx.x; i < (N_SINGLE << REP_LOG2); i += THREADS) s_single[i] = lut[GC_PAIR_LUT_PAIRS + (i >> REP_LOG2)];
    if (EXTRA && io.se_row)
        for (int i = threadIdx.x; i < C * GC_TBL; i += THREADS) s_se[i / GC_TBL][i % GC_TBL] = tab.se[i / GC_TBL][i % GC_TBL];
    if (threadIdx.x < 5) s_stats[threadIdx.x] = 0;
    pdl_launch_dependents();
    pdl_wait();
    step_counter_read(io, &s_ctr);
    __syncthreads();
    const uint32_t step0 = step_counter_arrive(io, &s_ctr);
    const uint32_t rep = threadIdx.x & (REP - 1u);
    const uint32_t lut_mul = 8u << REP_LOG2;
    const uint32_t pair_base = static_cast<uint32_t>(__cvta_generic_to_shared(s_pair)) + rep * 8u;
    const uint32_t single_base = static_cast<uint32_t>(__cvta_generic_to_shared(s_single)) + rep * 8u;

    uint32_t st_steps = 0, st_unsafe = 0, st_count = 0, st_trunc = 0;
    long long st_reward = 0;
#pragma unroll 1
    for (uint32_t e0 = static_cast<uint32_t>(io.begin) + (blockIdx.x * THREADS + threadIdx.x) * kEPT; e0 < e_end; e0 += stride) {
        const int rem = static_cast<int>(e_end - e0 < kEPT ? e_end - e0 : kEPT);
        const uint64_t gid0 = static_cast<uint64_t>(io.env_id_offset) + e0;
        const uint32_t gid_lo = static_cast<uint32_t>(gid0), gid_hi = static_cast<uint32_t>(gid0 >> 32);
        const int4 ps = ld_stream_v4(io.state + e0), pt = ld_stream_v4(io.t + e0);
        int4 an = ld_stream_v4(mio.tape[0] + e0);
        uint32_t sw4[kEPT] = {(uint32_t)ps.x, (uint32_t)ps.y, (uint32_t)ps.z, (uint32_t)ps.w};
        int tin[kEPT] = {pt.x, pt.y, pt.z, pt.w};
        int slot = 0;
#pragma unroll 1
        for (int k = 0; k < mio.n_steps; ++k) {
            const uint32_t aw4[kEPT] = {(uint32_t)an.x, (uint32_t)an.y, (uint32_t)an.z, (uint32_t)an.w};
            slot = slot + 1 == mio.n_tape ? 0 : slot + 1;
            if (k + 1 < mio.n_steps) an = ld_stream_v4(mio.tape[slot] + e0);
            const uint32_t step_counter = (RNG == GC_RNG_PHILOX) ? step0 + static_cast<uint32_t>(k) : 0u;
            uint32_t nstate[kEPT];
            int tn[kEPT];
            packed_word<C, RNG, EXTRA>(tab, io, s_se, pair_base, single_base, lut_mul, e0, rem, gid_lo, gid_hi, step_counter, sw4, aw4,
                                       tin, st_steps, st_unsafe, st_count, st_trunc, st_reward, nstate, tn);
#pragma unroll
            for (int e = 0; e < kEPT; ++e) { sw4[e] = nstate[e]; tin[e] = tn[e]; }
        }
    }
    if (io.stats) {
        const ThreadStats ts = {st_steps, st_unsafe, st_count, st_trunc, st_reward};
        block_flush_stats(ts, s_stats, io.stats);
    }
    if (threadIdx.x == 0 && io.done_ctr != nullptr && s_ctr.arrived == gridDim.x - 1) {
        *io.done_ctr = 0u;
        *const_cast<uint32_t *>(io.step_ctr) = s_ctr.step + static_cast<uint32_t>(mio.n_steps);
    }
}

template <int C, int RNG, bool EXTRA, int THREADS>
cudaError_t launch_packed_many_t(const CellTables &tab, const PackedManyIO &mio, const uint2 *lut, int n_sm, cudaStream_t st)
{
    const auto kernel = cell_packed_many_kernel<C, RNG, EXTRA, THREADS>;
    const int64_t n = mio.io.end - mio.io.begin;
    const size_t smem = packed_smem_bytes(RNG, true);
    static int per_sm = 0;
    if (per_sm == 0 &&
        (cudaOccupancyMaxActiveBlocksPerMultiprocessor(&per_sm, kernel, THREADS, smem) != cudaSuccess || per_sm < 1))
        per_sm = 1;
    const int64_t need = (n + THREADS * kEPT - 1) / (THREADS * kEPT);
    const int64_t cap = static_cast<int64_t>(n_sm) * per_sm;
    const int grid = static_cast<int>(need < cap ? (need < 1 ? 1 : need) : cap);
    return launch_step_kernel(kernel, grid, THREADS, smem, st, tab, mio, lut, packed_rep_log2(RNG, true));
}

template <int C, int RNG, bool EXTRA>
cudaError_t launch_packed_many_cre(const CellTables &tab, const PackedManyIO &mio, const uint2 *lut, int n_sm, cudaStream_t st)
{
    const int64_t n = mio.io.end - mio.io.begin;
    const bool small = (n + kPackThreads * kEPT - 1) / (kPackThreads * kEPT) < n_sm;
    return small ? launch_packed_many_t<C, RNG, EXTRA, GC_MANY_SMALL_THREADS>(tab, mio, lut, n_sm, st)
                 : launch_packed_many_t<C, RNG, EXTRA, kPackThreads>(tab, mio, lut, n_sm, st);
}

template <int C, int RNG>
cudaError_t launch_packed_many_cr(const CellTables &tab, const PackedManyIO &mio, const uint2 *lut, int n_sm, cudaStream_t st)
{
    const PackedIO &io = mio.io;
    const bool extra = io.final_state || io.se_row || (io.index && tab.n_states != 4);
    return extra ? launch_packed_many_cre<C, RNG, true>(tab, mio, lut, n_sm, st)
                 : launch_packed_many_cre<C, RNG, false>(tab, mio, lut, n_sm, st);
}

#ifndef GC_PACKED_BIG_ENVS
#define GC_PACKED_BIG_ENVS (1 << 21)
#endif

template <int C, int RNG, bool EXTRA>
cudaError_t launch_packed_cre(const CellTables &tab, const PackedIO &io, const uint2 *lut, int n_sm, cudaStream_t st)
{
    const auto kernel = cell_packed_kernel<C, RNG, EXTRA>;
    const int64_t n = io.end - io.begin;
    const bool big = n >= GC_PACKED_BIG_ENVS;
    const size_t smem = packed_smem_bytes(RNG, big);
    static int per_sm[2] = {0, 0};
    if (per_sm[big] == 0 &&
        (cudaOccupancyMaxActiveBlocksPerMultiprocessor(&per_sm[big], kernel, kPackThreads, smem) != cudaSuccess || per_sm[big] < 1))
        per_sm[big] = 1;
    const int64_t need = (n + kPackThreads * kEPT - 1) / (kPackThreads * kEPT);
    const int64_t cap = static_cast<int64_t>(n_sm) * per_sm[big];
    const int grid = static_cast<int>(need < cap ? (need < 1 ? 1 : need) : cap);
    return launch_step_kernel(kernel, grid, kPackThreads, smem, st, tab, io, lut, packed_rep_log2(RNG, big));
}

template <int C, int RNG>
cudaError_t launch_packed_cr(const CellTables &tab, const PackedIO &io, const uint2 *lut, int n_sm, cudaStream_t st)
{
    const bool extra = io.final_state || io.se_row || (io.index && tab.n_states != 4);
    return extra ? launch_packed_cre<C, RNG, true>(tab, io, lut, n_sm, st)
                 : launch_packed_cre<C, RNG, false>(tab, io, lut, n_sm, st);
}

__global__ void __launch_bounds__(kPackThreads)
reset_packed_kernel(uint32_t init_packed, uint32_t init_index, const uint8_t *__restrict__ mask, uint32_t *state,
                    int32_t *t, uint32_t *index, int64_t n)
{
    const int64_t stride = static_cast<int64_t>(gridDim.x) * kPackThreads;
    for (int64_t e = static_cast<int64_t>(blockIdx.x) * kPackThreads + threadIdx.x; e < n; e += stride) {
        if (mask != nullptr && mask[e] == 0) continue;
        state[e] = init_packed;
        t[e] = 0;
        if (index) index[e] = init_index;
    }
}

__global__ void __launch_bounds__(kPackThreads)
pack_kernel(int64_t n, int64_t ld, int n_cells, const int8_t *__restrict__ cells, uint32_t *__restrict__ packed)
{
    const int64_t stride = static_cast<int64_t>(gridDim.x) * kPackThreads * kEPT;
    for (int64_t e0 = (static_cast<int64_t>(blockIdx.x) * kPackThreads + threadIdx.x) * kEPT; e0 < n; e0 += stride) {
        uint32_t w[kEPT] = {0, 0, 0, 0};
        for (int c = 0; c < n_cells; ++c) {
            const uint32_t row = ld_stream_u32(cells + c * ld + e0);
#pragma unroll
            for (int e = 0; e < kEPT; ++e) w[e] |= (byte_of(row, e) & 3u) << (2 * c);
        }
        st_stream_v4(packed + e0, make_int4(w[0], w[1], w[2], w[3]));
    }
}

__global__ void __launch_bounds__(kPackThreads)
unpack_kernel(int64_t n, int64_t ld, int n_cells, const uint32_t *__restrict__ packed, int8_t *__restrict__ cells)
{
    const int64_t stride = static_cast<int64_t>(gridDim.x) * kPackThreads * kEPT;
    for (int64_t e0 = (static_cast<int64_t>(blockIdx.x) * kPackThreads + threadIdx.x) * kEPT; e0 < n; e0 += stride) {
        const int4 v = ld_stream_v4(packed + e0);
        const uint32_t w[kEPT] = {(uint32_t)v.x, (uint32_t)v.y, (uint32_t)v.z, (uint32_t)v.w};
        for (int c = 0; c < n_cells; ++c) {
            uint32_t row = 0;
#pragma unroll
            for (int e = 0; e < kEPT; ++e) row |= ((w[e] >> (2 * c)) & 3u) << (8 * e);
            st_stream_u32(cells + c * ld + e0, row);
        }
    }
}

int aux_grid(int64_t n, int per_thread)
{
    const int64_t need = (n + static_cast<int64_t>(kPackThreads) * per_thread - 1) / (static_cast<int64_t>(kPackThreads) * per_thread);
    return static_cast<int>(need < 1 ? 1 : (need > 65535 ? 65535 : need));
}

}

cudaError_t gc_launch_cell_packed_step(const CellTables &tab, const PackedIO &io, const uint2 *lut, bool noise,
                                       int n_sm, cudaStream_t st)
{
    switch (tab.n_cells) {
#define GC_CASE(C)                                                                                  \
    case C:                                                                                         \
        return noise ? launch_packed_cr<C, GC_RNG_PHILOX>(tab, io, lut, n_sm, st)                   \
                     : launch_packed_cr<C, GC_RNG_NONE>(tab, io, lut, n_sm, st);
        GC_CASE(1) GC_CASE(2) GC_CASE(3) GC_CASE(4) GC_CASE(5) GC_CASE(6) GC_CASE(7) GC_CASE(8)
        GC_CASE(9) GC_CASE(10) GC_CASE(11) GC_CASE(12) GC_CASE(13) GC_CASE(14) GC_CASE(15) GC_CASE(16)
#undef GC_CASE
    default: return cudaErrorInvalidValue;
    }
}

cudaError_t gc_launch_cell_packed_many(const CellTables &tab, const PackedManyIO &mio, const uint2 *lut, bool noise, int n_sm,
                                       cudaStream_t st)
{
    switch (tab.n_cells) {
#define GC_CASE(C)                                                                                  \
    case C:                                                                                         \
        return noise ? launch_packed_many_cr<C, GC_RNG_PHILOX>(tab, mio, lut, n_sm, st)             \
                     : launch_packed_many_cr<C, GC_RNG_NONE>(tab, mio, lut, n_sm, st);
        GC_CASE(1) GC_CASE(2) GC_CASE(3) GC_CASE(4) GC_CASE(5) GC_CASE(6) GC_CASE(7) GC_CASE(8)
#undef GC_CASE
    default: return cudaErrorInvalidValue;
    }
}

cudaError_t gc_launch_reset_packed(uint32_t init_packed, uint32_t init_index, const uint8_t *mask, uint32_t *state,
                                   int32_t *t, uint32_t *index, int64_t n, cudaStream_t st)
{
    reset_packed_kernel<<<aux_grid(n, 1), kPackThreads, 0, st>>>(init_packed, init_index, mask, state, t, index, n);
    return cudaGetLastError();
}

cudaError_t gc_launch_pack(int64_t n, int64_t ld, int n_cells, const int8_t *cells, uint32_t *packed, cudaStream_t st)
{
    pack_kernel<<<aux_grid(n, kEPT), kPackThreads, 0, st>>>(n, ld, n_cells, cells, packed);
    return cudaGetLastError();
}

cudaError_t gc_launch_unpack(int64_t n, int64_t ld, int n_cells, const uint32_t *packed, int8_t *cells, cudaStream_t st)
{
    unpack_kernel<<<aux_grid(n, kEPT), kPackThreads, 0, st>>>(n, ld, n_cells, packed, cells);
    return cudaGetLastError();
}
```

gym_cellular_b200/csrc/gc_cell_pair8.cu:

```cuda
#include "gc_device.cuh"

namespace {

#ifndef GC_PAIR8_MINB
#define GC_PAIR8_MINB 4
#endif

template <int RNG, bool WITH_SE>
#ifndef GC_PAIR8_NOISE_MINB
#define GC_PAIR8_NOISE_MINB 4
#endif
__global__ void __launch_bounds__(kThreads, RNG == GC_RNG_NONE ? GC_PAIR8_MINB : GC_PAIR8_NOISE_MINB)
cell_pair8_kernel(const __grid_constant__ CellTables tab, const __grid_constant__ StepIO io, const uint2 *__restrict__ lut)
{
    constexpr bool NOISE = RNG == GC_RNG_PHILOX;
    constexpr int N_SINGLE = NOISE ? 128 : 64;
    __shared__ uint2 s_pair[NOISE ? 1 : GC_PAIR8_PAIRS];
    __shared__ uint2 s_single[N_SINGLE];
    __shared__ uint8_t s_se[WITH_SE ? GC_MAX_CELLS : 1][GC_TBL];
    __shared__ unsigned long long s_stats[5];
    __shared__ StepCounterShared s_ctr;
    const int C = tab.n_cells;
    const uint32_t ld = static_cast<uint32_t>(io.ld);
    const uint32_t stride = gridDim.x * kThreads * kEPT, e_end = static_cast<uint32_t>(io.end);
    uint32_t e0 = static_cast<uint32_t>(io.begin) + (blockIdx.x * kThreads + threadIdx.x) * kEPT;

    if constexpr (!NOISE)
        for (int i = threadIdx.x; i < GC_PAIR8_PAIRS; i += kThreads) s_pair[i] = lut[i];
    if (threadIdx.x < N_SINGLE) s_single[threadIdx.x] = lut[GC_PAIR8_PAIRS + threadIdx.x];
    if constexpr (WITH_SE)
        for (int i = threadIdx.x; i < tab.n_cells * GC_TBL; i += kThreads) s_se[i / GC_TBL][i % GC_TBL] = tab.se[i / GC_TBL][i % GC_TBL];
    if (threadIdx.x < 5) s_stats[threadIdx.x] = 0;
    pdl_launch_dependents();
    pdl_wait();
    step_counter_read(io, &s_ctr);
    __syncthreads();
    [[maybe_unused]] const uint32_t step_counter = step_counter_arrive(io, &s_ctr);

    uint32_t st_steps = 0, st_unsafe = 0, st_count = 0, st_trunc = 0;
    long long st_reward = 0;
#pragma unroll 1
    for (; e0 < e_end; e0 += stride) {
        const int rem = static_cast<int>(e_end - e0 < kEPT ? e_end - e0 : kEPT);
        uint32_t sw[4] = {0, 0, 0, 0}, aw[4] = {0, 0, 0, 0};
#pragma unroll
        for (int i = 0; i < 4; ++i)
            if (i < C) { sw[i] = ld_stream_u32(io.state + (i * ld + e0)); aw[i] = ld_stream_u32(io.actions + (i * ld + e0)); }
        const int4 t4 = ld_stream_v4(io.t + e0);
        int tn[kEPT] = {t4.x + 1, t4.y + 1, t4.z + 1, t4.w + 1};
        uint32_t trunc_w = 0, keep = 0xFFFFFFFFu;
        if (io.max_episode_steps > 0) {
#pragma unroll
            for (int e = 0; e < kEPT; ++e)
                if (tn[e] >= io.max_episode_steps) { tn[e] = 0; trunc_w |= 1u << (8 * e); keep &= ~(0xFFu << (8 * e)); }
        }
        float r[kEPT] = {0.f, 0.f, 0.f, 0.f};
        uint32_t idx[kEPT] = {0, 0, 0, 0};
        uint32_t sum01 = 0, sum23 = 0;
        uint32_t or01 = 0, or23 = 0;
        uint32_t s0w = 0;
        [[maybe_unused]] uint32_t s1w = 0;
        [[maybe_unused]] uint32_t fire[kEPT] = {0, 0, 0, 0};
        if constexpr (NOISE) {
            const uint64_t gid0 = static_cast<uint64_t>(io.env_id_offset) + e0;
            const uint32_t gid_lo = static_cast<uint32_t>(gid0), gid_hi = static_cast<uint32_t>(gid0 >> 32);
            const int tin[kEPT] = {t4.x, t4.y, t4.z, t4.w};
#pragma unroll
            for (int e = 0; e < kEPT; ++e) {
                const uint32_t ctr = io.episodic ? static_cast<uint32_t>(tin[e]) : step_counter;
                if (C > GC_NARROW_CELLS) {
                    fire[e] = fire_bits_wide<2>(tab, gid_lo | e, gid_hi, ctr, io.round_key);
                } else {
                    uint32_t w[4];
                    philox4x32_10(gid_lo | e, gid_hi, ctr, 0u, io.round_key, w);
                    const uint32_t thr = tab.noise_thr_m1;
                    fire[e] = (w[0] <= thr ? 1u : 0u) | (w[1] <= thr ? 2u : 0u) | (w[2] <= thr ? 4u : 0u) | (w[3] <= thr ? 8u : 0u);
                }
            }
        }

        [[maybe_unused]] auto emit_se = [&](int j, uint32_t partner_row) {
            uint32_t sew = 0;
#pragma unroll
            for (int e = 0; e < kEPT; ++e)
                sew |= static_cast<uint32_t>(s_se[j][((byte_of(s0w, e) & 7u) * GC_LVL_PAD + (byte_of(partner_row, e) & 7u))]) << (8 * e);
            st_stream_u32(io.se_row + (j * ld + e0), sew);
        };
        auto account = [&](const uint2 (&ent)[kEPT], int c, bool pair, uint32_t keep_bits) {
#pragma unroll
            for (int e = 0; e < kEPT; ++e) r[e] += __uint_as_float(ent[e].y);
            const uint32_t w01 = prmt(ent[0].x, ent[1].x, 0x5410), w23 = prmt(ent[2].x, ent[3].x, 0x5410);
            sum01 += w01 & 0x001F001Fu; sum23 += w23 & 0x001F001Fu;
            or01 |= w01 & keep_bits; or23 |= w23 & keep_bits;
            const uint32_t u = prmt(ent[0].x, ent[1].x, 0x7362), v = prmt(ent[2].x, ent[3].x, 0x7362);
            const uint32_t row_c = prmt(u, v, 0x5410), row_d = prmt(u, v, 0x7632);
            if (c == 0) s0w = row_c;
            if (NOISE && c == 1) s1w = row_c;
            if constexpr (WITH_SE) {
                if (c == 0) {
                    if (pair) { emit_se(0, row_d); emit_se(1, row_d); }
                    else if (C == 1) emit_se(0, row_c);
                } else if (c == 1) {
                    emit_se(0, row_c); emit_se(1, row_c);
                } else {
                    emit_se(c, row_c);
                    if (pair) emit_se(c + 1, row_d);
                }
            }
            const uint32_t out_c = (row_c & keep) | ((0x01010101u * static_cast<uint8_t>(tab.init[c])) & ~keep);
            st_stream_u32(io.state + (c * ld + e0), out_c);
            if (io.final_state) st_stream_u32(io.final_state + (c * ld + e0), row_c);
            const uint32_t pc = tab.place[c];
#pragma unroll
            for (int e = 0; e < kEPT; ++e) idx[e] += byte_of(out_c, e) * pc;
            if (pair) {
                const uint32_t out_d = (row_d & keep) | ((0x01010101u * static_cast<uint8_t>(tab.init[c + 1])) & ~keep);
                st_stream_u32(io.state + ((c + 1) * ld + e0), out_d);
                if (io.final_state) st_stream_u32(io.final_state + ((c + 1) * ld + e0), row_d);
                const uint32_t pd = tab.place[c + 1];
#pragma unroll
                for (int e = 0; e < kEPT; ++e) idx[e] += byte_of(out_d, e) * pd;
            }
        };
        auto do_pair = [&](int c, int i) {
            const uint32_t code_c = (aw[i] & 0x07070707u) * 8u + (sw[i] & 0x07070707u);
            uint2 ent[kEPT];
            if (c + 1 < C) {
                const uint32_t code_d = (aw[i + 1] & 0x07070707u) * 8u + (sw[i + 1] & 0x07070707u);
                const uint32_t p02 = (code_c & 0x00FF00FFu) + (code_d & 0x00FF00FFu) * 64u;
                const uint32_t p13 = ((code_c >> 8) & 0x00FF00FFu) + ((code_d >> 8) & 0x00FF00FFu) * 64u;
                ent[0] = s_pair[p02 & 0xFFFu]; ent[2] = s_pair[(p02 >> 16) & 0xFFFu];
                ent[1] = s_pair[p13 & 0xFFFu]; ent[3] = s_pair[(p13 >> 16) & 0xFFFu];
                account(ent, c, true, c == 0 ? 0x00800080u : 0xFF00FF00u);
            } else {
#pragma unroll
                for (int e = 0; e < kEPT; ++e) ent[e] = s_single[byte_of(code_c, e) & 63u];
                account(ent, c, false, c == 0 ? 0x00800080u : 0xFF00FF00u);
            }
        };
        auto do_single = [&](int c, int i) {
            const uint32_t code = (aw[i] & 0x07070707u) * 8u + (sw[i] & 0x07070707u);
            uint2 ent[kEPT];
#pragma unroll
            for (int e = 0; e < kEPT; ++e) ent[e] = s_single[(byte_of(code, e) & 63u) | (((fire[e] >> c) & 1u) << 6)];
            account(ent, c, false, c >= 2 ? 0xFF00FF00u : 0u);
        };

#pragma unroll 1
        for (int c = 0; c < C; c += 4) {
            uint32_t ns[4] = {0, 0, 0, 0}, na[4] = {0, 0, 0, 0};
#pragma unroll
            for (int i = 0; i < 4; ++i)
                if (c + 4 + i < C) {
                    ns[i] = ld_stream_u32(io.state + ((c + 4 + i) * ld + e0));
                    na[i] = ld_stream_u32(io.actions + ((c + 4 + i) * ld + e0));
                }
            if constexpr (NOISE) {
#pragma unroll
                for (int i = 0; i < 4; ++i)
                    if (c + i < C) do_single(c + i, i);
            } else {
                do_pair(c, 0);
                if (c + 2 < C) do_pair(c + 2, 2);
            }
#pragma unroll
            for (int i = 0; i < 4; ++i) { sw[i] = ns[i]; aw[i] = na[i]; }
        }

        const uint32_t count_w = prmt(sum01, sum23, 0x6420) & 0x1F1F1F1Fu;
        const uint32_t present = prmt(or01, or23, 0x7531);
        uint32_t unsafe_w = NOISE ? 0u : (prmt(or01, or23, 0x6420) >> 7) & 0x01010101u;
#pragma unroll
        for (int e = 0; e < kEPT; ++e) {
            if constexpr (NOISE) {
                const uint32_t s1n = byte_of(C >= 2 ? s1w : s0w, e) & 7u;
                unsafe_w |= (static_cast<uint32_t>(tab.unsafe01_rows8 >> (8u * (byte_of(s0w, e) & 7u) + s1n)) & 1u) << (8 * e);
            }
            const uint32_t rowmask = static_cast<uint32_t>(tab.unsafe_rows8 >> (8u * (byte_of(s0w, e) & 7u))) & 0xFFu;
            unsafe_w |= ((byte_of(present, e) & rowmask) ? 1u : 0u) << (8 * e);
        }
        float rout[kEPT];
        log2_1p_x4(tab.reward_log2, r, rout);
#pragma unroll
        for (int e = 0; e < kEPT; ++e)
            if (e < rem) st_reward += __float2int_rn(rout[e] * 16777216.0f);
        {
            const uint32_t vb = valid_bytes(rem);
            st_steps += rem;
            st_unsafe = add_bytes(unsafe_w & vb, st_unsafe);
            st_count = add_bytes(count_w & vb, st_count);
            st_trunc = add_bytes(trunc_w & vb, st_trunc);
        }
        st_stream_v4(io.t + e0, make_int4(tn[0], tn[1], tn[2], tn[3]));
        st_stream_v4(io.reward + e0, make_int4(__float_as_int(rout[0]), __float_as_int(rout[1]),
                                               __float_as_int(rout[2]), __float_as_int(rout[3])));
        st_stream_v4(io.index + e0, make_int4(idx[0], idx[1], idx[2], idx[3]));
        st_stream_u32(io.terminated + e0, 0u);
        st_stream_u32(io.truncated + e0, trunc_w);
        st_stream_u32(io.unsafe + e0, unsafe_w);
        st_stream_u32(io.count + e0, count_w);
    }
    if (io.stats) {
        const ThreadStats ts = {st_steps, st_unsafe, st_count, st_trunc, st_reward};
        block_flush_stats(ts, s_stats, io.stats);
    }
    step_counter_finish(io, &s_ctr);
}

}

cudaError_t gc_launch_cell_pair8_step(const CellTables &tab, const StepIO &io, const uint2 *lut, int rng_mode, int n_sm,
                                      cudaStream_t st)
{
    const int64_t n = io.end - io.begin;
#define GC_PAIR8_LAUNCH(RNG, SE) \
    return launch_step_kernel(cell_pair8_kernel<RNG, SE>, grid_for<cell_pair8_kernel<RNG, SE>>(n, n_sm), kThreads, 0, st, tab, io, lut)
    if (rng_mode == GC_RNG_PHILOX) {
        if (io.se_row) GC_PAIR8_LAUNCH(GC_RNG_PHILOX, true);
        GC_PAIR8_LAUNCH(GC_RNG_PHILOX, false);
    }
    if (io.se_row) GC_PAIR8_LAUNCH(GC_RNG_NONE, true);
    GC_PAIR8_LAUNCH(GC_RNG_NONE, false);
#undef GC_PAIR8_LAUNCH
}
```

gym_cellular_b200/csrc/gc_device.cuh:

```cuda
#pragma once
#include "gc_internal.h"
#include <cstdlib>
#include <utility>

namespace {

constexpr int kThreads = 256;
constexpr int kEPT = 4;

__device__ __forceinline__ void philox4x32_10(uint32_t c0, uint32_t c1, uint32_t c2, uint32_t c3,
                                              const uint32_t (&rk)[20], uint32_t (&out)[4])
{
#pragma unroll
    for (int r = 0; r < 10; ++r) {
        const unsigned long long p0 = static_cast<unsigned long long>(0xD2511F53u) * c0;
        const unsigned long long p1 = static_cast<unsigned long long>(0xCD9E8D57u) * c2;
        c0 = static_cast<uint32_t>(p1 >> 32) ^ c1 ^ rk[2 * r];
        c1 = static_cast<uint32_t>(p1);
        c2 = static_cast<uint32_t>(p0 >> 32) ^ c3 ^ rk[2 * r + 1];
        c3 = static_cast<uint32_t>(p0);
    }
    out[0] = c0; out[1] = c1; out[2] = c2; out[3] = c3;
}

__device__ __forceinline__ uint32_t prmt(uint32_t a, uint32_t b, uint32_t sel) { return __byte_perm(a, b, sel); }


__device__ __forceinline__ void philox4x32_10_seeded(uint32_t (&c)[4], uint32_t k0, uint32_t k1)
{
#pragma unroll
    for (int r = 0; r < 10; ++r) {
        const unsigned long long p0 = static_cast<unsigned long long>(0xD2511F53u) * c[0];
        const unsigned long long p1 = static_cast<unsigned long long>(0xCD9E8D57u) * c[2];
        c[0] = static_cast<uint32_t>(p1 >> 32) ^ c[1] ^ k0;
        c[1] = static_cast<uint32_t>(p1);
        c[2] = static_cast<uint32_t>(p0 >> 32) ^ c[3] ^ k1;
        c[3] = static_cast<uint32_t>(p0);
        k0 += 0x9E3779B9u;
        k1 += 0xBB67AE85u;
    }
}

__device__ __noinline__ uint32_t noise_fire_with_ties(int n_blocks, uint32_t k16, uint32_t r16, uint32_t gid_lo, uint32_t gid_hi,
                                                      uint32_t ctr, uint32_t seed_lo, uint32_t seed_hi)
{
    uint32_t fire = 0, ties = 0;
#pragma unroll 1
    for (int b = 0; b < n_blocks; ++b) {
        uint32_t w[4] = {gid_lo, gid_hi, ctr, static_cast<uint32_t>(b)};
        philox4x32_10_seeded(w, seed_lo, seed_hi);
#pragma unroll
        for (int h = 0; h < 8; ++h) {
            const uint32_t half = (h & 1) ? w[h >> 1] >> 16 : w[h >> 1] & 0xFFFFu;
            if (half < k16) fire |= (1u << h) << (8 * b);
            if (half == k16) ties |= (1u << h) << (8 * b);
        }
    }
    while (ties) {
        const uint32_t c = static_cast<uint32_t>(__ffs(static_cast<int>(ties))) - 1u;
        ties &= ties - 1u;
        uint32_t lo[4] = {gid_lo, gid_hi, ctr, GC_NOISE_LOW_STREAM + c};
        philox4x32_10_seeded(lo, seed_lo, seed_hi);
        if ((lo[0] >> 16) < r16) fire |= 1u << c;
    }
    return fire;
}

template <int NB>
__device__ __forceinline__ uint32_t fire_bits_wide(const CellTables &tab, uint32_t gid_lo, uint32_t gid_hi, uint32_t ctr,
                                                   const uint32_t (&rk)[20])
{
    constexpr uint32_t H = 0x80008000u, L = 0x7FFF7FFFu, GATHER = 0x00008001u;
    uint32_t zmin = 0xFFFFFFFFu, fire = 0;
#pragma unroll
    for (int b = NB - 1; b >= 0; --b) {
        uint32_t w[4];
        philox4x32_10(gid_lo, gid_hi, ctr, static_cast<uint32_t>(b), rk, w);
#pragma unroll
        for (int i = 3; i >= 0; --i) {
            const uint32_t x = w[i];
            const uint32_t d = (x | H) - tab.noise_kk15;
            const uint32_t lt = ~((x & d) | ((x | d) & ~tab.noise_kmask)) & H;
            fire = __funnelshift_l(lt * GATHER, fire, 2);
        }
        zmin = __vimin3_u16x2(zmin, w[0] ^ tab.noise_kk, w[1] ^ tab.noise_kk);
        zmin = __vimin3_u16x2(zmin, w[2] ^ tab.noise_kk, w[3] ^ tab.noise_kk);
    }
    if (~(((zmin & L) + L) | zmin) & H)
        fire = noise_fire_with_ties(NB, tab.noise_kk & 0xFFFFu, tab.noise_r16, gid_lo, gid_hi, ctr, rk[0], rk[1]);
    return fire;
}

__device__ __forceinline__ uint32_t byte_of(uint32_t w, int e)
{
#ifdef GC_BYTE_OF_PRMT
    return __byte_perm(w, 0u, 0x4440u + static_cast<uint32_t>(e));
#else
    return (w >> (8 * e)) & 0xFFu;
#endif
}

__device__ __forceinline__ uint32_t ld_stream_u32(const void *p)
{
    return __ldcs(reinterpret_cast<const unsigned int *>(p));
}
__device__ __forceinline__ void st_stream_u32(void *p, uint32_t v)
{
    __stcs(reinterpret_cast<unsigned int *>(p), v);
}
__device__ __forceinline__ int4 ld_stream_v4(const void *p) { return __ldcs(reinterpret_cast<const int4 *>(p)); }
__device__ __forceinline__ void st_stream_v4(void *p, int4 v) { __stcs(reinterpret_cast<int4 *>(p), v); }

struct ThreadStats {
    uint32_t steps, unsafe, count, truncated;
    long long reward_q24;
};

template <class IO>
__device__ __forceinline__ uint32_t launch_step_counter(const IO &io)
{
    uint32_t v = io.rng_counter;
    if (io.step_ctr != nullptr) v = *reinterpret_cast<const volatile uint32_t *>(io.step_ctr);
    return v;
}

__device__ __forceinline__ void tick_step_counter(const uint32_t *step_ctr, uint32_t *done_ctr, uint32_t inc)
{
    if (done_ctr == nullptr) return;
    __syncthreads();
    if (threadIdx.x == 0) {
        const uint32_t arrived = atomicAdd(done_ctr, 1u);
        if (arrived == gridDim.x - 1) {
            *done_ctr = 0u;
            *const_cast<uint32_t *>(step_ctr) = *reinterpret_cast<const volatile uint32_t *>(step_ctr) + inc;
        }
    }
}

template <class IO>
__device__ __forceinline__ void tick_step_counter(const IO &io) { tick_step_counter(io.step_ctr, io.done_ctr, 1u); }

struct StepCounterShared { uint32_t step, arrived; };

template <class IO>
__device__ __forceinline__ void step_counter_read(const IO &io, StepCounterShared *s)
{
    if (threadIdx.x == 0) s->step = launch_step_counter(io);
}

template <class IO>
__device__ __forceinline__ uint32_t step_counter_arrive(const IO &io, StepCounterShared *s)
{
    if (threadIdx.x == 0 && io.done_ctr != nullptr) s->arrived = atomicAdd(io.done_ctr, 1u);
    return s->step;
}

template <class IO>
__device__ __forceinline__ void step_counter_finish(const IO &io, const StepCounterShared *s)
{
    if (threadIdx.x == 0 && io.done_ctr != nullptr && s->arrived == gridDim.x - 1) {
        *io.done_ctr = 0u;
        *const_cast<uint32_t *>(io.step_ctr) = s->step + 1u;
    }
}

__device__ __forceinline__ float log2_1p_small(float r)
{
    float s;
    asm("div.approx.ftz.f32 %0, %1, %2;" : "=f"(s) : "f"(r), "f"(2.0f + r));
    const float z = s * s;
    constexpr float k = 2.88539008177792681f;
    float p = k / 13.0f;
    p = fmaf(p, z, k / 11.0f);
    p = fmaf(p, z, k / 9.0f);
    p = fmaf(p, z, k / 7.0f);
    p = fmaf(p, z, k / 5.0f);
    p = fmaf(p, z, k / 3.0f);
    p = fmaf(p, z, k);
    return s * p;
}

__device__ __forceinline__ float log2_1p(float r)
{
    if (r >= -0.5f && r <= 1.0f) return log2_1p_small(r);
    return log1pf(r) * 1.44269504088896341f;
}

__device__ __forceinline__ void log2_1p_x4(int enabled, const float (&r)[4], float (&out)[4])
{
    if (!enabled) {
#pragma unroll
        for (int e = 0; e < 4; ++e) out[e] = r[e];
        return;
    }
    const float hi = fmaxf(fmaxf(r[0], r[1]), fmaxf(r[2], r[3])), lo = fminf(fminf(r[0], r[1]), fminf(r[2], r[3]));
    if (lo >= -0.5f && hi <= 1.0f) {
#pragma unroll
        for (int e = 0; e < 4; ++e) out[e] = log2_1p_small(r[e]);
    } else {
#pragma unroll
        for (int e = 0; e < 4; ++e) out[e] = log1pf(r[e]) * 1.44269504088896341f;
    }
}

__device__ __forceinline__ uint32_t valid_bytes(int rem) { return rem >= 4 ? 0xFFFFFFFFu : ((1u << (8 * rem)) - 1u); }

__device__ __forceinline__ uint32_t add_bytes(uint32_t w, uint32_t acc) { return __dp4a(w, 0x01010101u, acc); }

__device__ __forceinline__ unsigned long long warp_sum(unsigned long long v)
{
    const uint32_t lo = static_cast<uint32_t>(v), hi = static_cast<uint32_t>(v >> 32);
    const uint32_t a = __reduce_add_sync(0xffffffffu, lo & 0xFFFFu);
    const uint32_t b = __reduce_add_sync(0xffffffffu, lo >> 16);
    const uint32_t c = __reduce_add_sync(0xffffffffu, hi);
    return static_cast<unsigned long long>(a) + (static_cast<unsigned long long>(b) << 16) +
           (static_cast<unsigned long long>(c) << 32);
}

__device__ __forceinline__ unsigned long long warp_sum(uint32_t v)
{
    const uint32_t a = __reduce_add_sync(0xffffffffu, v & 0xFFFFu);
    const uint32_t b = __reduce_add_sync(0xffffffffu, v >> 16);
    return static_cast<unsigned long long>(a) + (static_cast<unsigned long long>(b) << 16);
}

__device__ __forceinline__ void block_flush_stats(const ThreadStats &ts, unsigned long long *s_stats,
                                                  unsigned long long *g_stats)
{
    const unsigned long long w[5] = {warp_sum(ts.steps), warp_sum(ts.unsafe), warp_sum(ts.count), warp_sum(ts.truncated),
                                     warp_sum(static_cast<unsigned long long>(ts.reward_q24))};
    if ((threadIdx.x & 31) == 0) {
#pragma unroll
        for (int i = 0; i < 5; ++i)
            if (w[i]) atomicAdd(&s_stats[i], w[i]);
    }
    __syncthreads();
    if (threadIdx.x < 5 && s_stats[threadIdx.x]) atomicAdd(&g_stats[threadIdx.x], s_stats[threadIdx.x]);
}

__device__ __forceinline__ void block_flush_stats_grid(uint32_t count, uint32_t truncated, uint32_t reward,
                                                       unsigned long long launch_steps, unsigned long long *s_stats,
                                                       unsigned long long *g_stats)
{
    const unsigned long long w[3] = {warp_sum(count), warp_sum(truncated), warp_sum(reward) << 24};
    if ((threadIdx.x & 31) == 0) {
#pragma unroll
        for (int i = 0; i < 3; ++i)
            if (w[i]) atomicAdd(&s_stats[2 + i], w[i]);
    }
    __syncthreads();
    if (threadIdx.x >= 2 && threadIdx.x < 5 && s_stats[threadIdx.x]) atomicAdd(&g_stats[threadIdx.x], s_stats[threadIdx.x]);
    if (blockIdx.x == 0 && threadIdx.x == 0) atomicAdd(&g_stats[0], launch_steps);
}

__device__ __forceinline__ void pdl_launch_dependents() { asm volatile("griddepcontrol.launch_dependents;" ::: "memory"); }
__device__ __forceinline__ void pdl_wait() { asm volatile("griddepcontrol.wait;" ::: "memory"); }

constexpr int kMaxDevices = 64;
inline int current_device_slot()
{
    int dev = 0;
    if (cudaGetDevice(&dev) != cudaSuccess || dev < 0) dev = 0;
    return dev < kMaxDevices ? dev : kMaxDevices - 1;
}

inline bool pdl_enabled()
{
    static const bool on = [] { const char *v = std::getenv("GC_B200_PDL"); return !(v && v[0] == '0'); }();
    return on;
}

template <typename... KArgs, typename... Args>
cudaError_t launch_step_kernel(void (*kernel)(KArgs...), int grid, int threads, size_t smem, cudaStream_t st, Args &&...args)
{
    cudaLaunchConfig_t cfg = {};
    cfg.gridDim = dim3(static_cast<unsigned>(grid));
    cfg.blockDim = dim3(static_cast<unsigned>(threads));
    cfg.dynamicSmemBytes = smem;
    cfg.stream = st;
    cudaLaunchAttribute attr[1];
    attr[0].id = cudaLaunchAttributeProgrammaticStreamSerialization;
    attr[0].val.programmaticStreamSerializationAllowed = 1;
    cfg.attrs = attr;
    cfg.numAttrs = pdl_enabled() ? 1 : 0;
    return cudaLaunchKernelEx(&cfg, kernel, std::forward<Args>(args)...);
}

#ifndef GC_OVERSUB
#define GC_OVERSUB 1
#endif
template <auto Kernel, int THREADS = kThreads>
int grid_for(int64_t n_envs, int n_sm)
{
    const auto kernel = Kernel;
    static int per_sm = 0;
    if (per_sm == 0 &&
        (cudaOccupancyMaxActiveBlocksPerMultiprocessor(&per_sm, kernel, THREADS, 0) != cudaSuccess || per_sm < 1))
        per_sm = 1;
    const int64_t need = (n_envs + THREADS * kEPT - 1) / (THREADS * kEPT);
    const int64_t cap = static_cast<int64_t>(n_sm) * per_sm * GC_OVERSUB;
    return static_cast<int>(need < cap ? (need < 1 ? 1 : need) : cap);
}

}
```

gym_cellular_b200/csrc/gc_grid.cu:

```cuda
#include "gc_device.cuh"

namespace {


#ifndef GC_GRID_THREADS
#define GC_GRID_THREADS 512
#endif
#ifndef GC_GRID_MINB
#define GC_GRID_MINB 2
#endif
#ifndef GC_GRID_SMALL_ITERS
#define GC_GRID_SMALL_ITERS 3
#endif
#ifndef GC_GRID_OVERSUB
#define GC_GRID_OVERSUB 1
#endif
constexpr int kGridThreads = GC_GRID_THREADS;
constexpr int kGridLutAlloc = GC_GRID_LUT_ALLOC;
constexpr int kGridSmemBytes = kGridLutAlloc * 4;

template <int RNG, bool LUT_GLOBAL>
__global__ void __launch_bounds__(kGridThreads, GC_GRID_MINB)
grid_step_kernel(const __grid_constant__ GridParams gp, const __grid_constant__ StepIO io)
{
    extern __shared__ __align__(16) uint32_t s_lut[];
    __shared__ unsigned long long s_stats[5];
    __shared__ StepCounterShared s_ctr;
    const uint32_t ld = static_cast<uint32_t>(io.ld);
    const uint32_t w_lo = blockIdx.x * kGridThreads, e_end = static_cast<uint32_t>(io.end);
    const uint32_t stride = gridDim.x * kGridThreads * kEPT;
    uint32_t e0 = static_cast<uint32_t>(io.begin) + (w_lo + threadIdx.x) * kEPT;
    constexpr int LUT_VEC = GC_GRID_LUT_ENTRIES / 4, LUT_PER_THREAD = (LUT_VEC + kGridThreads - 1) / kGridThreads;
    uint4 lut_reg[LUT_GLOBAL ? 1 : LUT_PER_THREAD];
    if (!LUT_GLOBAL) {
        const uint4 *src = reinterpret_cast<const uint4 *>(gp.lut);
#pragma unroll
        for (int k = 0; k < LUT_PER_THREAD; ++k) {
            const int i = threadIdx.x + k * kGridThreads;
            if (i < LUT_VEC) lut_reg[k] = src[i];
        }
    }
    pdl_launch_dependents();
    pdl_wait();
    uint32_t p_s0 = 0, p_s1 = 0, p_a0 = 0, p_a1 = 0;
    int4 p_t = make_int4(0, 0, 0, 0);
    if (e0 < e_end) {
        p_s0 = ld_stream_u32(io.state + e0); p_s1 = ld_stream_u32(io.state + (ld + e0));
        p_a0 = ld_stream_u32(io.actions + e0); p_a1 = ld_stream_u32(io.actions + (ld + e0));
        p_t = ld_stream_v4(io.t + e0);
    }
    step_counter_read(io, &s_ctr);
    if (!LUT_GLOBAL) {
        uint4 *dst = reinterpret_cast<uint4 *>(s_lut);
#pragma unroll
        for (int k = 0; k < LUT_PER_THREAD; ++k) {
            const int i = threadIdx.x + k * kGridThreads;
            if (i < LUT_VEC) dst[i] = lut_reg[k];
        }
    }
    if (threadIdx.x < 5) s_stats[threadIdx.x] = 0;
    __syncthreads();

    const uint32_t step_counter = step_counter_arrive(io, &s_ctr);
    uint32_t st_count = 0, st_trunc = 0, st_reward = 0, bad_bits = 0;
    for (; e0 < e_end; e0 += stride) {
        const int rem = static_cast<int>(e_end - e0 < kEPT ? e_end - e0 : kEPT);
        const uint64_t gid0 = static_cast<uint64_t>(io.env_id_offset) + e0;
        const uint32_t s0w = p_s0, s1w = p_s1;
        uint32_t a0w = p_a0, a1w = p_a1;
        const int4 t4 = p_t;
        if (e0 + stride < e_end) {
            const uint32_t en = e0 + stride;
            p_s0 = ld_stream_u32(io.state + en); p_s1 = ld_stream_u32(io.state + (ld + en));
            p_a0 = ld_stream_u32(io.actions + en); p_a1 = ld_stream_u32(io.actions + (ld + en));
            p_t = ld_stream_v4(io.t + en);
        }
        const int tin[kEPT] = {t4.x, t4.y, t4.z, t4.w};
        const uint32_t s0m = s0w & 0x1F1F1F1Fu, s1m = s1w & 0x1F1F1F1Fu;
        const uint32_t actw = (a0w & 0x07070707u) + (a1w & 0x07070707u) * 5u;
        const uint32_t i02 = ((s0m & 0x00FF00FFu) + 20u * (s1m & 0x00FF00FFu)) * 25u + (actw & 0x00FF00FFu);
        const uint32_t i13 = (((s0m >> 8) & 0x00FF00FFu) + 20u * ((s1m >> 8) & 0x00FF00FFu)) * 25u + ((actw >> 8) & 0x00FF00FFu);
        uint32_t ent[kEPT];
        if (LUT_GLOBAL) {
            ent[0] = __ldg(gp.lut + (i02 & 0xFFFFu)); ent[1] = __ldg(gp.lut + (i13 & 0xFFFFu));
            ent[2] = __ldg(gp.lut + (i02 >> 16)); ent[3] = __ldg(gp.lut + (i13 >> 16));
        } else {
            ent[0] = s_lut[i02 & 0xFFFFu]; ent[1] = s_lut[i13 & 0xFFFFu];
            ent[2] = s_lut[i02 >> 16]; ent[3] = s_lut[i13 >> 16];
        }
        uint32_t trig[kEPT];
        if (RNG == GC_RNG_PHILOX) {
            const uint64_t grp = gid0 >> 2;
            const bool same_t = !io.episodic || (tin[0] == tin[1] && tin[1] == tin[2] && tin[2] == tin[3]);
            if (same_t) {
                const uint32_t ctr = io.episodic ? static_cast<uint32_t>(tin[0]) : step_counter;
                philox4x32_10(static_cast<uint32_t>(grp), static_cast<uint32_t>(grp >> 32), ctr, 0u, io.round_key, trig);
            } else {
#pragma unroll 1
                for (int e = 0; e < kEPT; ++e) {
                    uint32_t w[4];
                    philox4x32_10(static_cast<uint32_t>(grp), static_cast<uint32_t>(grp >> 32),
                                  static_cast<uint32_t>(tin[e]), 0u, io.round_key, w);
                    trig[e] = w[e];
                }
            }
        }
        if (RNG == GC_RNG_PHILOX) {
            const uint32_t thr = gp.dispersal_thr_m1;
            if (gp.dispersal_thr_nz && (trig[0] <= thr || trig[1] <= thr || trig[2] <= thr || trig[3] <= thr)) {
#pragma unroll
                for (int e = 0; e < kEPT; ++e) {
                    uint32_t x = ent[e];
                    const uint32_t w = trig[e];
                    if (w <= thr && ((x >> 18) & 3u) < 2u) {
                        const uint32_t Nk = ((w >> 1) & 1u) | ((w & 1u) << 1);
                        const uint32_t sh = (w & 4u) << 1;
                        x = (x & ~(3u << sh)) | (Nk << sh);
                        const uint32_t Tp = (byte_of(s0w, e) & 3u) | ((byte_of(s1w, e) & 3u) << 8);
                        const uint32_t Np = x & 0x0303u;
                        const uint32_t rew = __popc(Tp & ~Np);
                        const uint32_t se1 = (Np & 3u) ? 1u : 0u, se0 = (se1 && (Np & 0x0300u)) ? 1u : 0u;
                        ent[e] = (x & ~((3u << 16) | (3u << 20))) | (rew << 16) | (se0 << 20) | (se1 << 21);
                    }
                }
            }
        } else {
#pragma unroll
            for (int e = 0; e < kEPT; ++e) {
                const uint32_t nb = (ent[e] >> 18) & 3u;
                const bool valid = e < rem;
                const double *u = io.replay + (valid ? static_cast<size_t>(e0 + e) * 6 : 0);
                if (nb < 2u && valid && u[0] < gp.dispersal_prob) {
                    const uint32_t b00 = static_cast<uint32_t>(u[1] * 2.0), b10 = static_cast<uint32_t>(u[3] * 2.0);
                    const uint32_t k = static_cast<uint32_t>(u[5] * 2.0);
                    const uint32_t T0 = byte_of(s0w, e) & 3u, T1 = byte_of(s1w, e) & 3u;
                    uint32_t nc0 = ent[e] & 0xFFu, nc1 = (ent[e] >> 8) & 0xFFu;
                    const uint32_t Nk = b10 | (b00 << 1);
                    if (k == 0u) nc0 = (nc0 & ~3u) | Nk; else nc1 = (nc1 & ~3u) | Nk;
                    const uint32_t N0 = nc0 & 3u, N1 = nc1 & 3u;
                    const uint32_t rew = __popc(T0 & ~N0) + __popc(T1 & ~N1);
                    const uint32_t se0 = (N0 > 0u && N1 > 0u) ? 1u : 0u, se1 = (N0 > 0u) ? 1u : 0u;
                    ent[e] = nc0 | (nc1 << 8) | (rew << 16) | (nb << 18) | (se0 << 20) | (se1 << 21) |
                             (ent[e] & (1u << 22));
                }
            }
        }
        const uint32_t m01 = prmt(ent[0], ent[1], 0x0062), m23 = prmt(ent[2], ent[3], 0x0062);
        const uint32_t miscw = prmt(m01, m23, 0x5410);
        const uint32_t vbytes = valid_bytes(rem);
        bad_bits |= miscw & vbytes;
        const uint32_t rew_w = miscw & 0x03030303u, count_w = (miscw >> 2) & 0x03030303u;
        const uint32_t se0w = (miscw >> 4) & 0x01010101u, se1w = (miscw >> 5) & 0x01010101u;
        const uint32_t u = prmt(ent[0], ent[1], 0x5140), v = prmt(ent[2], ent[3], 0x5140);
        uint32_t row0 = prmt(u, v, 0x5410), row1 = prmt(u, v, 0x7632);
        uint32_t trunc_w = 0;
        int tout[kEPT] = {tin[0] + 1, tin[1] + 1, tin[2] + 1, tin[3] + 1};
        if (io.final_state) {
            st_stream_u32(io.final_state + e0, row0);
            st_stream_u32(io.final_state + (ld + e0), row1);
        }
        if (io.max_episode_steps > 0) {
#pragma unroll
            for (int e = 0; e < kEPT; ++e) {
                const bool tr = tout[e] >= io.max_episode_steps;
                tout[e] = tr ? 0 : tout[e];
                trunc_w |= (tr ? 1u : 0u) << (8 * e);
            }
            const uint32_t gone = trunc_w * 0xFFu;
            row0 = (row0 & ~gone) | (0x0F0F0F0Fu & gone);
            row1 = (row1 & ~gone) | (0x12121212u & gone);
        }
        float rout[kEPT];
#pragma unroll
        for (int e = 0; e < kEPT; ++e) rout[e] = __uint_as_float(prmt(rew_w, 0x4B000000u, 0x7540u + e)) - 8388608.0f;
        const uint32_t x02 = (row0 & 0x00FF00FFu) + 20u * (row1 & 0x00FF00FFu);
        const uint32_t x13 = ((row0 >> 8) & 0x00FF00FFu) + 20u * ((row1 >> 8) & 0x00FF00FFu);
        const uint32_t iout[kEPT] = {x02 & 0xFFFFu, x13 & 0xFFFFu, x02 >> 16, x13 >> 16};
        {
            const uint32_t vb = valid_bytes(rem);
            st_count = add_bytes(count_w & vb, st_count);
            st_trunc = add_bytes(trunc_w & vb, st_trunc);
            st_reward = add_bytes(rew_w & vb, st_reward);
        }
        st_stream_u32(io.state + e0, row0);
        st_stream_u32(io.state + (ld + e0), row1);
        if (io.se_row) {
            st_stream_u32(io.se_row + e0, se0w);
            st_stream_u32(io.se_row + (ld + e0), se1w);
        }
        st_stream_v4(io.t + e0, make_int4(tout[0], tout[1], tout[2], tout[3]));
        st_stream_v4(io.reward + e0, make_int4(__float_as_int(rout[0]), __float_as_int(rout[1]),
                                               __float_as_int(rout[2]), __float_as_int(rout[3])));
        st_stream_v4(io.index + e0, make_int4(iout[0], iout[1], iout[2], iout[3]));
        st_stream_u32(io.terminated + e0, 0u);
        st_stream_u32(io.truncated + e0, trunc_w);
        st_stream_u32(io.unsafe + e0, 0u);
        st_stream_u32(io.count + e0, count_w);
    }
    if (bad_bits & 0x40404040u) atomicOr(io.status, 1ull);
    if (io.stats)
        block_flush_stats_grid(st_count, st_trunc, st_reward, static_cast<unsigned long long>(io.end - io.begin), s_stats, io.stats);
    step_counter_finish(io, &s_ctr);
}

__global__ void __launch_bounds__(kGridThreads, GC_GRID_MINB)
grid_many_kernel(const __grid_constant__ GridParams gp, const __grid_constant__ ManyIO mio)
{
    const StepIO &io = mio.io;
    extern __shared__ __align__(16) uint32_t s_lut[];
    __shared__ unsigned long long s_stats[5];
    __shared__ StepCounterShared s_ctr;
    const uint32_t ld = static_cast<uint32_t>(io.ld);
    const uint32_t e_end = static_cast<uint32_t>(io.end), stride = gridDim.x * kGridThreads * kEPT;
    {
        const uint4 *src = reinterpret_cast<const uint4 *>(gp.lut);
        uint4 *dst = reinterpret_cast<uint4 *>(s_lut);
        for (int i = threadIdx.x; i < kGridLutAlloc / 4; i += kGridThreads) dst[i] = src[i];
    }
    if (threadIdx.x < 5) s_stats[threadIdx.x] = 0;
    pdl_launch_dependents();
    pdl_wait();
    step_counter_read(io, &s_ctr);
    __syncthreads();
    const uint32_t step0 = step_counter_arrive(io, &s_ctr);
    uint32_t st_count = 0, st_trunc = 0, st_reward = 0, bad_bits = 0;
#pragma unroll 1
    for (uint32_t e0 = static_cast<uint32_t>(io.begin) + (blockIdx.x * kGridThreads + threadIdx.x) * kEPT; e0 < e_end; e0 += stride) {
        const int rem = static_cast<int>(e_end - e0 < kEPT ? e_end - e0 : kEPT);
        const uint64_t gid0 = static_cast<uint64_t>(io.env_id_offset) + e0;
        const uint64_t grp = gid0 >> 2;
        uint32_t s0w = ld_stream_u32(io.state + e0), s1w = ld_stream_u32(io.state + (ld + e0));
        uint32_t n_a0 = ld_stream_u32(mio.tape[0] + e0), n_a1 = ld_stream_u32(mio.tape[0] + (ld + e0));
        const int4 t4 = ld_stream_v4(io.t + e0);
        int tin[kEPT] = {t4.x, t4.y, t4.z, t4.w};
        int slot = 0;
#pragma unroll 1
        for (int k = 0; k < mio.n_steps; ++k) {
            const uint32_t a0w = n_a0, a1w = n_a1;
            slot = slot + 1 == mio.n_tape ? 0 : slot + 1;
            if (k + 1 < mio.n_steps) {
                const int8_t *const nxt = mio.tape[slot];
                n_a0 = ld_stream_u32(nxt + e0); n_a1 = ld_stream_u32(nxt + (ld + e0));
            }
            const uint32_t step_counter = step0 + static_cast<uint32_t>(k);
            const uint32_t s0m = s0w & 0x1F1F1F1Fu, s1m = s1w & 0x1F1F1F1Fu;
            const uint32_t actw = (a0w & 0x07070707u) + (a1w & 0x07070707u) * 5u;
            const uint32_t i02 = ((s0m & 0x00FF00FFu) + 20u * (s1m & 0x00FF00FFu)) * 25u + (actw & 0x00FF00FFu);
            const uint32_t i13 = (((s0m >> 8) & 0x00FF00FFu) + 20u * ((s1m >> 8) & 0x00FF00FFu)) * 25u + ((actw >> 8) & 0x00FF00FFu);
            uint32_t ent[kEPT];
            ent[0] = s_lut[i02 & 0xFFFFu]; ent[1] = s_lut[i13 & 0xFFFFu];
            ent[2] = s_lut[i02 >> 16]; ent[3] = s_lut[i13 >> 16];
            uint32_t trig[kEPT];
            const bool same_t = !io.episodic || (tin[0] == tin[1] && tin[1] == tin[2] && tin[2] == tin[3]);
            if (same_t) {
                const uint32_t ctr = io.episodic ? static_cast<uint32_t>(tin[0]) : step_counter;
                philox4x32_10(static_cast<uint32_t>(grp), static_cast<uint32_t>(grp >> 32), ctr, 0u, io.round_key, trig);
            } else {
#pragma unroll 1
                for (int e = 0; e < kEPT; ++e) {
                    uint32_t w[4];
                    philox4x32_10(static_cast<uint32_t>(grp), static_cast<uint32_t>(grp >> 32),
                                  static_cast<uint32_t>(tin[e]), 0u, io.round_key, w);
                    trig[e] = w[e];
                }
            }
            const uint32_t thr = gp.dispersal_thr_m1;
            if (gp.dispersal_thr_nz && (trig[0] <= thr || trig[1] <= thr || trig[2] <= thr || trig[3] <= thr)) {
#pragma unroll
                for (int e = 0; e < kEPT; ++e) {
                    uint32_t x = ent[e];
                    const uint32_t w = trig[e];
                    if (w <= thr && ((x >> 18) & 3u) < 2u) {
                        const uint32_t Nk = ((w >> 1) & 1u) | ((w & 1u) << 1);
                        const uint32_t sh = (w & 4u) << 1;
                        x = (x & ~(3u << sh)) | (Nk << sh);
                        const uint32_t Tp = (byte_of(s0w, e) & 3u) | ((byte_of(s1w, e) & 3u) << 8);
                        const uint32_t Np = x & 0x0303u;
                        const uint32_t rew = __popc(Tp & ~Np);
                        const uint32_t se1 = (Np & 3u) ? 1u : 0u, se0 = (se1 && (Np & 0x0300u)) ? 1u : 0u;
                        ent[e] = (x & ~((3u << 16) | (3u << 20))) | (rew << 16) | (se0 << 20) | (se1 << 21);
                    }
                }
            }
            const uint32_t m01 = prmt(ent[0], ent[1], 0x0062), m23 = prmt(ent[2], ent[3], 0x0062);
            const uint32_t miscw = prmt(m01, m23, 0x5410);
            const uint32_t vbytes = valid_bytes(rem);
            bad_bits |= miscw & vbytes;
            const uint32_t rew_w = miscw & 0x03030303u, count_w = (miscw >> 2) & 0x03030303u;
            const uint32_t se0w = (miscw >> 4) & 0x01010101u, se1w = (miscw >> 5) & 0x01010101u;
            const uint32_t u = prmt(ent[0], ent[1], 0x5140), v = prmt(ent[2], ent[3], 0x5140);
            uint32_t row0 = prmt(u, v, 0x5410), row1 = prmt(u, v, 0x7632);
            uint32_t trunc_w = 0;
            int tout[kEPT] = {tin[0] + 1, tin[1] + 1, tin[2] + 1, tin[3] + 1};
            if (io.max_episode_steps > 0) {
#pragma unroll
                for (int e = 0; e < kEPT; ++e) {
                    const bool tr = tout[e] >= io.max_episode_steps;
                    tout[e] = tr ? 0 : tout[e];
                    trunc_w |= (tr ? 1u : 0u) << (8 * e);
                }
                const uint32_t gone = trunc_w * 0xFFu;
                row0 = (row0 & ~gone) | (0x0F0F0F0Fu & gone);
                row1 = (row1 & ~gone) | (0x12121212u & gone);
            }
            float rout[kEPT];
#pragma unroll
            for (int e = 0; e < kEPT; ++e) rout[e] = __uint_as_float(prmt(rew_w, 0x4B000000u, 0x7540u + e)) - 8388608.0f;
            const uint32_t x02 = (row0 & 0x00FF00FFu) + 20u * (row1 & 0x00FF00FFu);
            const uint32_t x13 = ((row0 >> 8) & 0x00FF00FFu) + 20u * ((row1 >> 8) & 0x00FF00FFu);
            st_count = add_bytes(count_w & vbytes, st_count);
            st_trunc = add_bytes(trunc_w & vbytes, st_trunc);
            st_reward = add_bytes(rew_w & vbytes, st_reward);
            st_stream_u32(io.state + e0, row0);
            st_stream_u32(io.state + (ld + e0), row1);
            if (io.se_row) {
                st_stream_u32(io.se_row + e0, se0w);
                st_stream_u32(io.se_row + (ld + e0), se1w);
            }
            st_stream_v4(io.t + e0, make_int4(tout[0], tout[1], tout[2], tout[3]));
            st_stream_v4(io.reward + e0, make_int4(__float_as_int(rout[0]), __float_as_int(rout[1]),
                                                   __float_as_int(rout[2]), __float_as_int(rout[3])));
            st_stream_v4(io.index + e0, make_int4(x02 & 0xFFFFu, x13 & 0xFFFFu, x02 >> 16, x13 >> 16));
            st_stream_u32(io.terminated + e0, 0u);
            st_stream_u32(io.truncated + e0, trunc_w);
            st_stream_u32(io.unsafe + e0, 0u);
            st_stream_u32(io.count + e0, count_w);
            s0w = row0; s1w = row1;
#pragma unroll
            for (int e = 0; e < kEPT; ++e) tin[e] = tout[e];
        }
    }
    if (bad_bits & 0x40404040u) atomicOr(io.status, 1ull);
    if (io.stats)
        block_flush_stats_grid(st_count, st_trunc, st_reward,
                               static_cast<unsigned long long>(io.end - io.begin) * static_cast<unsigned long long>(mio.n_steps),
                               s_stats, io.stats);
    if (threadIdx.x == 0 && io.done_ctr != nullptr && s_ctr.arrived == gridDim.x - 1) {
        *io.done_ctr = 0u;
        *const_cast<uint32_t *>(io.step_ctr) = s_ctr.step + static_cast<uint32_t>(mio.n_steps);
    }
}

}

template <auto Kernel>
int grid_blocks(int64_t n, int n_sm, int smem_bytes, cudaError_t *err)
{
    static int per_sm_dev[kMaxDevices] = {};
    const int slot = current_device_slot();
    int per_sm = per_sm_dev[slot];
    if (per_sm == 0 || slot == kMaxDevices - 1) {
        *err = cudaFuncSetAttribute(Kernel, cudaFuncAttributeMaxDynamicSharedMemorySize, kGridSmemBytes);
        if (*err != cudaSuccess) return 0;
        if (cudaOccupancyMaxActiveBlocksPerMultiprocessor(&per_sm, Kernel, kGridThreads, smem_bytes) != cudaSuccess || per_sm < 1)
            per_sm = 1;
        per_sm_dev[slot] = per_sm;
    }
    const int64_t need = (n + kGridThreads * kEPT - 1) / (kGridThreads * kEPT);
    const int64_t cap = static_cast<int64_t>(n_sm) * per_sm * GC_GRID_OVERSUB;
    return static_cast<int>(need < cap ? (need < 1 ? 1 : need) : cap);
}

template <int RNG>
cudaError_t launch_grid(const GridParams &gp, const StepIO &io, int n_sm, cudaStream_t st)
{
    const int64_t n = io.end - io.begin;
    cudaError_t err = cudaSuccess;
    const int64_t wave = static_cast<int64_t>(n_sm) * GC_GRID_MINB * kGridThreads * kEPT;
    if (n <= wave * GC_GRID_SMALL_ITERS) {
        const int g = grid_blocks<grid_step_kernel<RNG, true>>(n, n_sm, 0, &err);
        if (err != cudaSuccess) return err;
        return launch_step_kernel(grid_step_kernel<RNG, true>, g, kGridThreads, 0, st, gp, io);
    } else {
        const int g = grid_blocks<grid_step_kernel<RNG, false>>(n, n_sm, kGridSmemBytes, &err);
        if (err != cudaSuccess) return err;
// ... 19 lines not shown
```

gym_cellular_b200/csrc/gc_internal.h:

```cpp
#pragma once
#include <cuda_runtime.h>
#include <stdint.h>

#include "gym_cellular_b200.h"

#define GC_LVL_PAD 8
#define GC_TBL (GC_LVL_PAD * GC_LVL_PAD)

#define GC_NARROW_CELLS 4
#define GC_NOISE_LOW_STREAM 0x20000000u

enum { GC_RNG_NONE = 0, GC_RNG_PHILOX = 1, GC_RNG_REPLAY = 2 };

struct StepIO {
    const int8_t *actions;
    int8_t       *state;
    int32_t      *t;
    float        *reward;
    uint32_t     *index;
    uint8_t      *terminated, *truncated, *unsafe, *count;
    int8_t       *se_row;
    int8_t       *final_state;
    const double *replay;
    unsigned long long *stats;
    unsigned long long *status;
    int64_t begin, end;
    int64_t ld;
    int64_t env_id_offset;
    uint32_t seed_lo, seed_hi;
    uint32_t round_key[20];
    uint32_t rng_counter;
    const uint32_t *step_ctr;
    uint32_t *done_ctr;
    int32_t  episodic;
    int32_t  max_episode_steps;
};

struct ManyIO {
    StepIO io;
    const int8_t *tape[GC_MAX_BINDINGS];
    int32_t n_tape, n_steps;
};
#define GC_MANY_MAX_CELLS 8

struct PackedIO {
    const uint32_t *actions;
    uint32_t *state;
    int32_t  *t;
    float    *reward;
    uint32_t *index;
    uint8_t  *flags;
    uint32_t *final_state;
    uint32_t *se_row;
    unsigned long long *stats;
    unsigned long long *status;
    int64_t begin, end, ld, env_id_offset;
    uint32_t round_key[20];
    uint32_t rng_counter;
    const uint32_t *step_ctr;
    uint32_t *done_ctr;
    int32_t episodic, max_episode_steps;
};

struct PackedManyIO {
    PackedIO io;
    const uint32_t *tape[GC_MAX_BINDINGS];
    int32_t n_tape, n_steps;
};

struct RolloutIO {
    int8_t       *state;
    int32_t      *t;
    uint32_t     *index;
    float        *ret;
    int32_t      *n_unsafe;
    const int32_t *policy;
    unsigned long long *stats;
    unsigned long long *status;
    int64_t n, ld, env_id_offset;
    uint32_t round_key[20];
    const uint32_t *step_ctr;
    uint32_t *done_ctr;
    int32_t episodic, max_episode_steps, n_steps, policy_kind;
    uint32_t *rec_obs, *rec_action, *rec_next_obs;
    float    *rec_reward;
    uint8_t  *rec_flags;
    unsigned long long joint_actions;
    uint32_t explore_thr_m1, explore_thr_nz;
};

struct CellTables {
    uint32_t sa[GC_TBL];
    float    reward[GC_TBL];
    float    reward_noisy[GC_TBL];
    uint8_t  se[GC_MAX_CELLS][GC_TBL];
    uint32_t place[GC_MAX_CELLS];
    uint32_t place4[4];
    uint32_t unsafe_rows;
    int8_t   init[GC_MAX_CELLS];
    uint32_t init_index;
    uint32_t counted_mask;
    int32_t  n_cells, n_states, n_actions;
    int32_t  reward_log2;
    unsigned long long noise_thr;
    uint32_t noise_thr_m1;
    uint32_t noise_thr_nz;
    uint32_t noise_kk15;
    uint32_t noise_kmask;
    uint32_t noise_kk;
    uint32_t noise_r16;
    double   noise_prob;
    uint32_t init_packed;
    unsigned long long unsafe_rows8;
    unsigned long long unsafe01_rows8;
};

struct GridParams {
    unsigned long long dispersal_thr;
    uint32_t dispersal_thr_m1, dispersal_thr_nz;
    double dispersal_prob;
    const uint32_t *lut;
};

#define GC_GRID_LUT_ENTRIES (400 * 25)
#define GC_GRID_LUT_ALLOC (((31 + 20 * 31) * 25 + 42 + 1 + 3) / 4 * 4)
void gc_build_grid_lut(uint32_t *lut);
void gc_build_pair_lut(const gc_cell_tables *t, int C, int S, int A, bool noise, uint2 *lut,
                       uint32_t *unsafe_rows);

cudaError_t gc_launch_cell_step(const CellTables &tab, const StepIO &io, int rng_mode, int n_sm,
                                cudaStream_t stream);
#define GC_PAIR_LUT_PAIRS 1024
#define GC_PAIR_LUT_ENTRIES (GC_PAIR_LUT_PAIRS + 32)
cudaError_t gc_launch_cell_pair_step(const CellTables &tab, const StepIO &io, const uint2 *lut, int rng_mode,
                                     int n_sm, cudaStream_t stream);
cudaError_t gc_launch_grid_many(const GridParams &gp, const ManyIO &mio, int n_sm, cudaStream_t stream);
cudaError_t gc_launch_cell_pair_many(const CellTables &tab, const ManyIO &mio, const uint2 *lut, int rng_mode, int n_sm,
                                     cudaStream_t stream);
cudaError_t gc_launch_cell_tma_step(const CellTables &tab, const StepIO &io, const uint2 *lut, int n_sm,
                                    cudaStream_t stream);
#define GC_PAIR8_PAIRS 4096
#define GC_PAIR8_ENTRIES (GC_PAIR8_PAIRS + 128)
void gc_build_pair8_lut(const gc_cell_tables *t, int C, int S, int A, bool noise, uint2 *lut, unsigned long long *unsafe_rows8,
                        unsigned long long *unsafe01_rows8);
cudaError_t gc_launch_cell_pair8_step(const CellTables &tab, const StepIO &io, const uint2 *lut, int rng_mode, int n_sm,
                                      cudaStream_t stream);
void gc_build_packed_lut(const gc_cell_tables *t, int C, int S, int A, bool noise, uint2 *lut);
cudaError_t gc_launch_cell_packed_step(const CellTables &tab, const PackedIO &io, const uint2 *lut, bool noise,
                                       int n_sm, cudaStream_t stream);
cudaError_t gc_launch_cell_packed_many(const CellTables &tab, const PackedManyIO &mio, const uint2 *lut, bool noise, int n_sm,
                                       cudaStream_t stream);
cudaError_t gc_launch_reset_packed(uint32_t init_packed, uint32_t init_index, const uint8_t *mask, uint32_t *state,
                                   int32_t *t, uint32_t *index, int64_t n, cudaStream_t stream);
cudaError_t gc_launch_pack(int64_t n, int64_t ld, int n_cells, const int8_t *cells, uint32_t *packed, cudaStream_t stream);
cudaError_t gc_launch_unpack(int64_t n, int64_t ld, int n_cells, const uint32_t *packed, int8_t *cells, cudaStream_t stream);
cudaError_t gc_launch_cell_rollout(const CellTables &tab, const RolloutIO &io, const uint2 *lut, bool noise,
                                   int n_sm, cudaStream_t stream);
cudaError_t gc_launch_grid_rollout(const GridParams &gp, const RolloutIO &io, int n_sm, cudaStream_t stream);
cudaError_t gc_launch_cell_collect(const CellTables &tab, const RolloutIO &io, const uint2 *lut, bool noise,
                                   int n_sm, cudaStream_t stream);
cudaError_t gc_launch_grid_collect(const GridParams &gp, const RolloutIO &io, int n_sm, cudaStream_t stream);
cudaError_t gc_launch_grid_step(const GridParams &gp, const StepIO &io, int rng_mode, int n_sm,
                                cudaStream_t stream);
cudaError_t gc_launch_reset(int n_cells, const int8_t *init, uint32_t init_index, const uint8_t *mask,
                            int8_t *state, int32_t *t, uint32_t *index, int64_t n, int64_t ld,
                            cudaStream_t stream);
cudaError_t gc_launch_encode_mixed(int64_t n, int64_t ld, int n_cells, const int32_t *radix, const int32_t *min,
                                   const int8_t *cells, uint32_t *index, cudaStream_t stream);
cudaError_t gc_launch_decode_mixed(int64_t n, int64_t ld, int n_cells, const int32_t *radix, const int32_t *min,
                                   const uint32_t *index, int8_t *cells, cudaStream_t stream);
cudaError_t gc_launch_tick(uint32_t *d_step, uint32_t inc, cudaStream_t stream);
cudaError_t gc_launch_encode(int64_t n, int64_t ld, int n_cells, uint32_t radix, const int8_t *cells,
                             uint32_t *index, cudaStream_t stream);
cudaError_t gc_launch_decode(int64_t n, int64_t ld, int n_cells, uint32_t radix, const uint32_t *index,
                             int8_t *cells, cudaStream_t stream);
```

gym_cellular_b200/csrc/gc_kernels.cu:

```cuda
#include "gc_device.cuh"

namespace {

template <int RNG>
__global__ void __launch_bounds__(kThreads, RNG == GC_RNG_PHILOX ? 3 : 4)
cell_step_kernel(const __grid_constant__ CellTables tab, const __grid_constant__ StepIO io)
{
    __shared__ uint2 s_sa[GC_TBL];
    __shared__ float s_rn[GC_TBL];
    __shared__ uint8_t s_se[GC_MAX_CELLS][GC_TBL];
    __shared__ unsigned long long s_stats[5];
    const int C = tab.n_cells;

    for (int i = threadIdx.x; i < GC_TBL; i += kThreads)
        s_sa[i] = make_uint2(tab.sa[i], __float_as_uint(tab.reward[i])), s_rn[i] = tab.reward_noisy[i];
    for (int i = threadIdx.x; i < C * GC_TBL; i += kThreads)
        s_se[i / GC_TBL][i % GC_TBL] = tab.se[i / GC_TBL][i % GC_TBL];
    if (threadIdx.x < 5) s_stats[threadIdx.x] = 0;
    __syncthreads();

    const uint32_t step_counter = (RNG == GC_RNG_PHILOX) ? launch_step_counter(io) : 0u;
    uint32_t st_steps = 0, st_unsafe = 0, st_count = 0, st_trunc = 0;
    long long st_reward = 0;
    const uint32_t ld = static_cast<uint32_t>(io.ld);
    const uint32_t stride = gridDim.x * kThreads * kEPT, e_end = static_cast<uint32_t>(io.end);
    for (uint32_t e0 = static_cast<uint32_t>(io.begin) + (blockIdx.x * kThreads + threadIdx.x) * kEPT;
         e0 < e_end; e0 += stride) {
        const int rem = static_cast<int>(e_end - e0 < kEPT ? e_end - e0 : kEPT);
        const uint64_t gid0 = static_cast<uint64_t>(io.env_id_offset) + e0;
        const uint32_t gid_lo = static_cast<uint32_t>(gid0), gid_hi = static_cast<uint32_t>(gid0 >> 32);
        uint32_t sw = ld_stream_u32(io.state + e0), aw = ld_stream_u32(io.actions + e0);
        const int4 t4 = ld_stream_v4(io.t + e0);
        const int tin[kEPT] = {t4.x, t4.y, t4.z, t4.w};
        int tn[kEPT] = {t4.x + 1, t4.y + 1, t4.z + 1, t4.w + 1};
        uint32_t trunc_w = 0, keep = 0xFFFFFFFFu;
        if (io.max_episode_steps > 0) {
#pragma unroll
            for (int e = 0; e < kEPT; ++e)
                if (tn[e] >= io.max_episode_steps) { tn[e] = 0; trunc_w |= 1u << (8 * e); keep &= ~(0xFFu << (8 * e)); }
        }
        float r[kEPT] = {0.f, 0.f, 0.f, 0.f};
        uint32_t idx[kEPT] = {0, 0, 0, 0};
        uint32_t unsafe_w = 0, count_w = 0, row0 = 0;
        uint32_t rnd[kEPT][4];
        uint32_t fire16[kEPT] = {0, 0, 0, 0};
        const bool wide = C > GC_NARROW_CELLS;
        if (RNG == GC_RNG_PHILOX && wide) {
#pragma unroll
            for (int e = 0; e < kEPT; ++e)
                fire16[e] = fire_bits_wide<2>(tab, gid_lo | e, gid_hi, io.episodic ? static_cast<uint32_t>(tin[e]) : step_counter,
                                              io.round_key);
        }

#pragma unroll 1
        for (int c = 0; c < C; ++c) {
            uint32_t sn = 0, an = 0;
            if (c + 1 < C) {
                sn = ld_stream_u32(io.state + ((c + 1) * ld + e0));
                an = ld_stream_u32(io.actions + ((c + 1) * ld + e0));
            }
            if (RNG == GC_RNG_PHILOX && !wide && (c & 3) == 0) {
#pragma unroll
                for (int e = 0; e < kEPT; ++e) {
                    const uint32_t ctr = io.episodic ? static_cast<uint32_t>(tin[e]) : step_counter;
                    philox4x32_10(gid_lo | e, gid_hi, ctr, static_cast<uint32_t>(c >> 2), io.round_key, rnd[e]);
                }
            }
            uint32_t row = 0, sew = 0;
#pragma unroll
            for (int e = 0; e < kEPT; ++e) {
                const uint32_t sa_ix = (byte_of(sw, e) * GC_LVL_PAD + byte_of(aw, e)) & (GC_TBL - 1);
                const uint2 ent = s_sa[sa_ix];
                bool fire = false;
                if (RNG == GC_RNG_PHILOX) {
                    const uint32_t word = (c & 3) == 0 ? rnd[e][0] : (c & 3) == 1 ? rnd[e][1] : (c & 3) == 2 ? rnd[e][2] : rnd[e][3];
                    fire = (ent.x & 0x100u) && tab.noise_thr_nz && (wide ? ((fire16[e] >> c) & 1u) != 0u : word <= tab.noise_thr_m1);
                } else if (RNG == GC_RNG_REPLAY) {
                    if (e < rem && (ent.x & 0x100u)) fire = io.replay[static_cast<size_t>(e0 + e) * C + c] < tab.noise_prob;
                }
                const uint32_t nxt = fire ? ((ent.x >> 4) & 15u) : (ent.x & 15u);
                r[e] += fire ? s_rn[sa_ix] : __uint_as_float(ent.y);
                row |= nxt << (8 * e);
                count_w += ((tab.counted_mask >> nxt) & 1u) << (8 * e);
            }
            if (c == 0) row0 = row;
            uint32_t sew0 = 0;
#pragma unroll
            for (int e = 0; e < kEPT; ++e) {
                const uint32_t s0n = byte_of(row0, e), sp = byte_of(row, e);
                if (c > 0) {
                    const uint32_t code = s_se[c][(s0n * GC_LVL_PAD + sp) & (GC_TBL - 1)];
                    sew |= code << (8 * e);
                    unsafe_w |= (code == 2u ? 1u : 0u) << (8 * e);
                }
                if (c == 1 || C == 1) {
                    const uint32_t code0 = s_se[0][(s0n * GC_LVL_PAD + sp) & (GC_TBL - 1)];
                    sew0 |= code0 << (8 * e);
                    unsafe_w |= (code0 == 2u ? 1u : 0u) << (8 * e);
                }
            }
            if (io.se_row) {
                if (c > 0) st_stream_u32(io.se_row + (c * ld + e0), sew);
                if (c == 1 || C == 1) st_stream_u32(io.se_row + e0, sew0);
            }
            const uint32_t out = (row & keep) | ((0x01010101u * static_cast<uint8_t>(tab.init[c])) & ~keep);
            st_stream_u32(io.state + (c * ld + e0), out);
            if (io.final_state) st_stream_u32(io.final_state + (c * ld + e0), row);
            const uint32_t place = tab.place[c];
#pragma unroll
            for (int e = 0; e < kEPT; ++e) idx[e] += byte_of(out, e) * place;
            sw = sn; aw = an;
        }

        float rout[kEPT];
#pragma unroll
        for (int e = 0; e < kEPT; ++e) {
            float rr = r[e];
            if (tab.reward_log2) rr = log2_1p(rr);
            rout[e] = rr;
            if (e < rem) st_reward += __float2int_rn(rr * 16777216.0f);
        }
        {
            const uint32_t vb = valid_bytes(rem);
            st_steps += rem;
            st_unsafe = add_bytes(unsafe_w & vb, st_unsafe);
            st_count = add_bytes(count_w & vb, st_count);
            st_trunc = add_bytes(trunc_w & vb, st_trunc);
        }
        st_stream_v4(io.t + e0, make_int4(tn[0], tn[1], tn[2], tn[3]));
        st_stream_v4(io.reward + e0, make_int4(__float_as_int(rout[0]), __float_as_int(rout[1]),
                                               __float_as_int(rout[2]), __float_as_int(rout[3])));
        st_stream_v4(io.index + e0, make_int4(idx[0], idx[1], idx[2], idx[3]));
        st_stream_u32(io.terminated + e0, 0u);
        st_stream_u32(io.truncated + e0, trunc_w);
        st_stream_u32(io.unsafe + e0, unsafe_w);
        st_stream_u32(io.count + e0, count_w);
    }
    if (io.stats) {
        const ThreadStats ts = {st_steps, st_unsafe, st_count, st_trunc, st_reward};
        block_flush_stats(ts, s_stats, io.stats);
    }
    tick_step_counter(io);
}

struct InitBlock { int8_t cells[GC_MAX_CELLS]; uint32_t index; int32_t n_cells; };

__global__ void __launch_bounds__(kThreads)
reset_kernel(const __grid_constant__ InitBlock ini, const uint8_t *__restrict__ mask, int8_t *state,
             int32_t *t, uint32_t *index, int64_t n, int64_t ld)
{
    const int64_t stride = static_cast<int64_t>(gridDim.x) * kThreads * kEPT;
    for (int64_t e0 = (static_cast<int64_t>(blockIdx.x) * kThreads + threadIdx.x) * kEPT; e0 < n; e0 += stride) {
        if (mask == nullptr) {
            for (int c = 0; c < ini.n_cells; ++c)
                *reinterpret_cast<uint32_t *>(state + c * ld + e0) = 0x01010101u * static_cast<uint8_t>(ini.cells[c]);
            *reinterpret_cast<int4 *>(t + e0) = make_int4(0, 0, 0, 0);
            if (index) *reinterpret_cast<uint4 *>(index + e0) = make_uint4(ini.index, ini.index, ini.index, ini.index);
        } else {
            const uint32_t m = *reinterpret_cast<const uint32_t *>(mask + e0);
            if (m == 0u) continue;
            uint32_t sel = 0;
#pragma unroll
            for (int e = 0; e < kEPT; ++e) if (byte_of(m, e)) sel |= 0xFFu << (8 * e);
            for (int c = 0; c < ini.n_cells; ++c) {
                uint32_t *w = reinterpret_cast<uint32_t *>(state + c * ld + e0);
                *w = (*w & ~sel) | ((0x01010101u * static_cast<uint8_t>(ini.cells[c])) & sel);
            }
#pragma unroll
            for (int e = 0; e < kEPT; ++e)
                if (byte_of(m, e)) { t[e0 + e] = 0; if (index) index[e0 + e] = ini.index; }
        }
    }
}

__global__ void tick_kernel(uint32_t *step, uint32_t inc) { *step += inc; }

__global__ void __launch_bounds__(kThreads)
encode_kernel(int64_t n, int64_t ld, int n_cells, uint32_t radix, const int8_t *__restrict__ cells,
              uint32_t *__restrict__ index)
{
    const int64_t stride = static_cast<int64_t>(gridDim.x) * kThreads * kEPT;
    for (int64_t e0 = (static_cast<int64_t>(blockIdx.x) * kThreads + threadIdx.x) * kEPT; e0 < n; e0 += stride) {
        uint32_t idx[kEPT] = {0, 0, 0, 0};
        uint32_t place = 1;
        for (int c = 0; c < n_cells; ++c) {
            const uint32_t w = ld_stream_u32(cells + c * ld + e0);
#pragma unroll
            for (int e = 0; e < kEPT; ++e) idx[e] += byte_of(w, e) * place;
            place *= radix;
        }
        st_stream_v4(index + e0, make_int4(idx[0], idx[1], idx[2], idx[3]));
    }
}

__global__ void __launch_bounds__(kThreads)
decode_kernel(int64_t n, int64_t ld, int n_cells, uint32_t radix, const uint32_t *__restrict__ index,
              int8_t *__restrict__ cells)
{
    const int64_t stride = static_cast<int64_t>(gridDim.x) * kThreads * kEPT;
    for (int64_t e0 = (static_cast<int64_t>(blockIdx.x) * kThreads + threadIdx.x) * kEPT; e0 < n; e0 += stride) {
        const int4 v = ld_stream_v4(index + e0);
        uint32_t idx[kEPT] = {static_cast<uint32_t>(v.x), static_cast<uint32_t>(v.y),
                              static_cast<uint32_t>(v.z), static_cast<uint32_t>(v.w)};
        for (int c = 0; c < n_cells; ++c) {
            uint32_t w = 0;
#pragma unroll
            for (int e = 0; e < kEPT; ++e) {
                w |= (idx[e] % radix) << (8 * e);
                idx[e] /= radix;
            }
            st_stream_u32(cells + c * ld + e0, w);
        }
    }
}

struct MixedRadix { uint32_t radix[GC_MAX_CELLS]; int32_t min[GC_MAX_CELLS]; int32_t n_cells; };

__global__ void __launch_bounds__(kThreads)
encode_mixed_kernel(const __grid_constant__ MixedRadix mr, int64_t n, int64_t ld, const int8_t *__restrict__ cells,
                    uint32_t *__restrict__ index)
{
    const int64_t stride = static_cast<int64_t>(gridDim.x) * kThreads * kEPT;
    for (int64_t e0 = (static_cast<int64_t>(blockIdx.x) * kThreads + threadIdx.x) * kEPT; e0 < n; e0 += stride) {
        uint32_t idx[kEPT] = {0, 0, 0, 0};
        uint32_t place = 1;
        for (int c = 0; c < mr.n_cells; ++c) {
            const uint32_t w = ld_stream_u32(cells + c * ld + e0);
#pragma unroll
            for (int e = 0; e < kEPT; ++e) {
                const int digit = static_cast<int>(static_cast<int8_t>(byte_of(w, e))) - mr.min[c];
                idx[e] += static_cast<uint32_t>(digit) * place;
            }
            place *= mr.radix[c];
        }
        st_stream_v4(index + e0, make_int4(idx[0], idx[1], idx[2], idx[3]));
    }
}

__global__ void __launch_bounds__(kThreads)
decode_mixed_kernel(const __grid_constant__ MixedRadix mr, int64_t n, int64_t ld, const uint32_t *__restrict__ index,
                    int8_t *__restrict__ cells)
{
    const int64_t stride = static_cast<int64_t>(gridDim.x) * kThreads * kEPT;
    for (int64_t e0 = (static_cast<int64_t>(blockIdx.x) * kThreads + threadIdx.x) * kEPT; e0 < n; e0 += stride) {
        const int4 v = ld_stream_v4(index + e0);
        uint32_t idx[kEPT] = {static_cast<uint32_t>(v.x), static_cast<uint32_t>(v.y),
                              static_cast<uint32_t>(v.z), static_cast<uint32_t>(v.w)};
        for (int c = 0; c < mr.n_cells; ++c) {
            const uint32_t radix = mr.radix[c];
            uint32_t w = 0;
#pragma unroll
            for (int e = 0; e < kEPT; ++e) {
                const int level = static_cast<int>(idx[e] % radix) + mr.min[c];
                w |= (static_cast<uint32_t>(level) & 0xFFu) << (8 * e);
                idx[e] /= radix;
            }
            st_stream_u32(cells + c * ld + e0, w);
        }
    }
}

}

cudaError_t gc_launch_encode_mixed(int64_t n, int64_t ld, int n_cells, const int32_t *radix, const int32_t *min,
                                   const int8_t *cells, uint32_t *index, cudaStream_t st)
{
    MixedRadix mr = {};
    for (int c = 0; c < n_cells; ++c) { mr.radix[c] = static_cast<uint32_t>(radix[c]); mr.min[c] = min ? min[c] : 0; }
    mr.n_cells = n_cells;
    const int64_t need = (n + kThreads * kEPT - 1) / (kThreads * kEPT);
    encode_mixed_kernel<<<static_cast<int>(need < 1 ? 1 : (need > 65535 ? 65535 : need)), kThreads, 0, st>>>(mr, n, ld, cells, index);
    return cudaGetLastError();
}

cudaError_t gc_launch_decode_mixed(int64_t n, int64_t ld, int n_cells, const int32_t *radix, const int32_t *min,
                                   const uint32_t *index, int8_t *cells, cudaStream_t st)
{
    MixedRadix mr = {};
    for (int c = 0; c < n_cells; ++c) { mr.radix[c] = static_cast<uint32_t>(radix[c]); mr.min[c] = min ? min[c] : 0; }
    mr.n_cells = n_cells;
    const int64_t need = (n + kThreads * kEPT - 1) / (kThreads * kEPT);
    decode_mixed_kernel<<<static_cast<int>(need < 1 ? 1 : (need > 65535 ? 65535 : need)), kThreads, 0, st>>>(mr, n, ld, index, cells);
    return cudaGetLastError();
}

cudaError_t gc_launch_cell_step(const CellTables &tab, const StepIO &io, int rng_mode, int n_sm, cudaStream_t st)
{
    if (tab.n_cells < 1 || tab.n_cells > GC_MAX_CELLS) return cudaErrorInvalidValue;
    const int64_t n = io.end - io.begin;
    switch (rng_mode) {
    case GC_RNG_NONE:
        cell_step_kernel<GC_RNG_NONE><<<grid_for<cell_step_kernel<GC_RNG_NONE>>(n, n_sm), kThreads, 0, st>>>(tab, io);
        break;
    case GC_RNG_PHILOX:
        cell_step_kernel<GC_RNG_PHILOX><<<grid_for<cell_step_kernel<GC_RNG_PHILOX>>(n, n_sm), kThreads, 0, st>>>(tab, io);
        break;
    default:
        cell_step_kernel<GC_RNG_REPLAY><<<grid_for<cell_step_kernel<GC_RNG_REPLAY>>(n, n_sm), kThreads, 0, st>>>(tab, io);
        break;
    }
    return cudaGetLastError();
}

cudaError_t gc_launch_reset(int n_cells, const int8_t *init, uint32_t init_index, const uint8_t *mask,
                            int8_t *state, int32_t *t, uint32_t *index, int64_t n, int64_t ld, cudaStream_t st)
{
    InitBlock ini;
    for (int c = 0; c < GC_MAX_CELLS; ++c) ini.cells[c] = c < n_cells ? init[c] : 0;
    ini.index = init_index;
    ini.n_cells = n_cells;
    const int64_t need = (n + kThreads * kEPT - 1) / (kThreads * kEPT);
    reset_kernel<<<static_cast<int>(need < 1 ? 1 : (need > 65535 ? 65535 : need)), kThreads, 0, st>>>(
        ini, mask, state, t, index, n, ld);
    return cudaGetLastError();
}

cudaError_t gc_launch_tick(uint32_t *d_step, uint32_t inc, cudaStream_t st)
{
    tick_kernel<<<1, 1, 0, st>>>(d_step, inc);
    return cudaGetLastError();
}

cudaError_t gc_launch_encode(int64_t n, int64_t ld, int n_cells, uint32_t radix, const int8_t *cells,
                             uint32_t *index, cudaStream_t st)
{
    const int64_t need = (n + kThreads * kEPT - 1) / (kThreads * kEPT);
    encode_kernel<<<static_cast<int>(need < 1 ? 1 : (need > 65535 ? 65535 : need)), kThreads, 0, st>>>(
        n, ld, n_cells, radix, cells, index);
    return cudaGetLastError();
}
// ... 10 lines not shown
```

include/gym_cellular_b200.h:

```cpp
#ifndef GYM_CELLULAR_B200_H
#define GYM_CELLULAR_B200_H

#include <stdint.h>

#ifdef __cplusplus
extern "C" {
#endif

#define GC_ABI_VERSION 2

typedef struct gc_env gc_env;

typedef enum {
    GC_OK = 0,
    GC_ERR_INVALID = -1,
    GC_ERR_CUDA = -2,
    GC_ERR_STATE = -3,
    GC_ERR_ACTION = -4
} gc_status;

#define GC_KIND_CELLULAR  0
#define GC_KIND_GRIDWORLD 1

#define GC_F_NOISE        1u
#define GC_F_RNG_EPISODIC 4u
#define GC_F_REWARD_LOG2  16u
#define GC_F_GENERIC_KERNEL 32u

#define GC_MAX_CELLS   16
#define GC_MAX_LEVELS  8
#define GC_N_STATS     8

#define GC_STAT_STEPS       0
#define GC_STAT_UNSAFE      1
#define GC_STAT_COUNT       2
#define GC_STAT_TRUNCATED   3
#define GC_STAT_REWARD_Q24  4

typedef struct {
    uint32_t struct_size;
    int32_t  kind;
    int32_t  device;
    int32_t  n_cells;
    int32_t  n_states;
    int32_t  n_actions;
    int32_t  max_episode_steps;
    uint32_t flags;
    int64_t  n_envs;
    int64_t  ld;
    int64_t  env_id_offset;
    uint64_t seed;
    double   noise_prob;
    double   dispersal_prob;
} gc_config;

typedef struct {
    const int8_t  *move;
    const int8_t  *noisy;
    const uint8_t *draws;
    const float   *reward;
    const int8_t  *side_effects;
    const uint8_t *counted;
    const int8_t  *initial_state;
    const float   *reward_noisy;
    const int32_t *radix;
} gc_cell_tables;

int         gc_abi_version(void);
const char *gc_last_error(void);

int gc_create(const gc_config *cfg, gc_env **out);
int gc_destroy(gc_env *env);
int gc_set_tables(gc_env *env, const gc_cell_tables *tables);

int gc_set_final_obs(gc_env *env, int8_t *final_state);

int gc_set_global_step(gc_env *env, int64_t step);
int64_t gc_get_global_step(const gc_env *env);
int gc_sync_global_step(gc_env *env, void *stream);
int64_t gc_launch_count(const gc_env *env);

int gc_reset(gc_env *env, const uint8_t *mask, int8_t *state, int32_t *t, uint32_t *index, void *stream);

int gc_step(gc_env *env, int64_t env_begin, int64_t env_count, const int8_t *actions, int8_t *state,
            int32_t *t, float *reward, uint32_t *index, uint8_t *terminated, uint8_t *truncated,
            uint8_t *unsafe, uint8_t *count, int8_t *se_row, const double *replay_u, int64_t *stats,
            void *stream);

#define GC_MAX_BINDINGS 16
int gc_bind_step(gc_env *env, int32_t slot, const int8_t *actions, int8_t *state, int32_t *t, float *reward,
                 uint32_t *index, uint8_t *terminated, uint8_t *truncated, uint8_t *unsafe, uint8_t *count,
                 int8_t *se_row, int64_t *stats);
int gc_step_bound(gc_env *env, int32_t slot, void *stream);
int gc_step_many(gc_env *env, const int32_t *slots, int32_t n_slots, int32_t n_steps, void *stream);
int gc_prepare_step_many(gc_env *env, const int32_t *slots, int32_t n_slots);

int gc_step_host(gc_env *env, const int8_t *h_actions, int8_t *h_state, float *h_reward,
                 uint32_t *h_index, uint8_t *h_terminated, uint8_t *h_truncated, uint8_t *h_unsafe,
                 uint8_t *h_count, int8_t *h_se_row, int8_t *d_actions, int8_t *d_state, int32_t *d_t,
                 float *d_reward, uint32_t *d_index, uint8_t *d_terminated, uint8_t *d_truncated,
                 uint8_t *d_unsafe, uint8_t *d_count, int8_t *d_se_row, int64_t *d_stats,
                 int64_t chunk_envs);

#define GC_FLAG_UNSAFE      1u
#define GC_FLAG_TRUNCATED   2u
#define GC_FLAG_COUNT_SHIFT 2
int gc_reset_packed(gc_env *env, const uint8_t *mask, uint32_t *state, int32_t *t, uint32_t *index, void *stream);
int gc_step_packed(gc_env *env, int64_t env_begin, int64_t env_count, const uint32_t *actions, uint32_t *state,
                   int32_t *t, float *reward, uint32_t *index, uint8_t *flags, uint32_t *final_state,
                   uint32_t *se_row, int64_t *stats, void *stream);
int gc_bind_step_packed(gc_env *env, int32_t slot, const uint32_t *actions, uint32_t *state, int32_t *t,
                        float *reward, uint32_t *index, uint8_t *flags, uint32_t *final_state, uint32_t *se_row,
                        int64_t *stats);
int gc_step_host_packed(gc_env *env, const uint32_t *h_actions, uint32_t *h_state, float *h_reward,
                        uint32_t *h_index, uint8_t *h_flags, uint32_t *d_actions, uint32_t *d_state, int32_t *d_t,
                        float *d_reward, uint32_t *d_index, uint8_t *d_flags, int64_t *d_stats, int64_t chunk_envs);
int gc_pack_cells(int device, int64_t n, int64_t ld, int32_t n_cells, const int8_t *cells, uint32_t *packed, void *stream);
int gc_unpack_cells(int device, int64_t n, int64_t ld, int32_t n_cells, const uint32_t *packed, int8_t *cells, void *stream);

#define GC_POLICY_RANDOM 0
#define GC_POLICY_TABLE  1
int gc_rollout(gc_env *env, int32_t n_steps, int32_t policy_kind, const int32_t *policy, int8_t *state,
               int32_t *t, uint32_t *index, float *ret, int32_t *n_unsafe, int64_t *stats, void *stream);

typedef struct {
    uint32_t  struct_size;
    uint32_t *obs;
    uint32_t *action;
    float    *reward;
    uint8_t  *flags;
    uint32_t *next_obs;
} gc_record;

int gc_collect(gc_env *env, int32_t n_steps, int32_t policy_kind, const int32_t *policy, double epsilon,
               int8_t *state, int32_t *t, uint32_t *index, const gc_record *record, int64_t *stats, void *stream);

int gc_poll_status(gc_env *env, void *stream);

int gc_encode(int device, int64_t n, int64_t ld, int32_t n_cells, int32_t radix, const int8_t *cells,
              uint32_t *index, void *stream);
int gc_decode(int device, int64_t n, int64_t ld, int32_t n_cells, int32_t radix, const uint32_t *index,
              int8_t *cells, void *stream);

int gc_encode_mixed(int device, int64_t n, int64_t ld, int32_t n_cells, const int32_t *radix, const int32_t *min,
                    const int8_t *cells, uint32_t *index, void *stream);
int gc_decode_mixed(int device, int64_t n, int64_t ld, int32_t n_cells, const int32_t *radix, const int32_t *min,
                    const uint32_t *index, int8_t *cells, void *stream);

#ifdef __cplusplus
}
#endif
#endif
```

Before: 86.76 billion.

## Alternate sweep direction across launches and keep tail outputs hot in L2

```diff
diff --git a/gym_cellular_b200/_lib.py b/gym_cellular_b200/_lib.py
--- a/gym_cellular_b200/_lib.py
+++ b/gym_cellular_b200/_lib.py
@@ -13,7 +13,7 @@
 POLICY_RANDOM, POLICY_TABLE = 0, 1
 
 EXPORTS = ["gc_abi_version", "gc_last_error", "gc_create", "gc_destroy", "gc_set_tables", "gc_set_final_obs",
-           "gc_set_global_step", "gc_get_global_step", "gc_sync_global_step", "gc_launch_count", "gc_reset", "gc_step",
+           "gc_set_global_step", "gc_get_global_step", "gc_sync_global_step", "gc_launch_count", "gc_reversed_launch_count", "gc_reset", "gc_step",
            "gc_bind_step", "gc_step_bound", "gc_step_many", "gc_prepare_step_many", "gc_step_host", "gc_rollout", "gc_collect", "gc_poll_status", "gc_encode",
            "gc_decode", "gc_encode_mixed", "gc_decode_mixed", "gc_reset_packed", "gc_step_packed", "gc_bind_step_packed",
            "gc_step_host_packed", "gc_pack_cells", "gc_unpack_cells"]
@@ -71,6 +71,8 @@
     L.gc_sync_global_step.argtypes = [vp, vp]
     L.gc_launch_count.argtypes = [vp]
     L.gc_launch_count.restype = i64
+    L.gc_reversed_launch_count.argtypes = [vp]
+    L.gc_reversed_launch_count.restype = i64
     L.gc_reset.argtypes = [vp] * 6
     L.gc_step.argtypes = [vp, i64, i64] + [vp] * 13
     L.gc_bind_step.argtypes = [vp, C.c_int32] + [vp] * 11
diff --git a/gym_cellular_b200/csrc/gc_api.cu b/gym_cellular_b200/csrc/gc_api.cu
--- a/gym_cellular_b200/csrc/gc_api.cu
+++ b/gym_cellular_b200/csrc/gc_api.cu
@@ -75,8 +75,11 @@
     GridParams grid;
     bool tables_set;
     int n_sm;
+    int64_t l2_bytes;
     int64_t global_step;
     int64_t launches;
+    bool sweep_reverse;
+    int64_t reversed_launches;
     unsigned long long *d_status;
     uint32_t *d_step;
     uint32_t *d_done;
@@ -141,6 +144,7 @@
     io.done_ctr = nullptr;
     io.episodic = (env->cfg.flags & GC_F_RNG_EPISODIC) ? 1 : 0;
     io.max_episode_steps = env->cfg.max_episode_steps;
+    io.reverse = 0;
     return io;
 }
 
@@ -165,7 +169,22 @@
     io.done_ctr = nullptr;
     io.episodic = (env->cfg.flags & GC_F_RNG_EPISODIC) ? 1 : 0;
     io.max_episode_steps = env->cfg.max_episode_steps;
+    io.reverse = 0;
+    io.keep_words = 0;
     return io;
+}
+
+template <class IO>
+bool set_sweep(gc_env *env, IO &io, int64_t step_bytes)
+{
+    if (io.done_ctr == nullptr) return false;
+    const char *v = std::getenv("GC_B200_SWEEP_ALTERNATE");
+    const bool on = v ? v[0] != '0' : env->cfg.n_envs * step_bytes > env->l2_bytes;
+    if (!on) return false;
+    io.reverse = env->sweep_reverse ? 1 : 0;
+    env->sweep_reverse = !env->sweep_reverse;
+    env->reversed_launches += io.reverse;
+    return true;
 }
 
 int check_packed(const gc_env *env)
@@ -176,9 +195,14 @@
     return GC_OK;
 }
 
-int launch_packed(gc_env *env, const PackedIO &io, cudaStream_t st)
+int launch_packed(gc_env *env, PackedIO io, cudaStream_t st)
 {
     if (io.end <= io.begin) return GC_OK;
+    const int64_t out_bytes = 13 + (io.index ? 4 : 0) + (io.final_state ? 4 : 0) + (io.se_row ? 4 : 0);
+    if (set_sweep(env, io, 12 + out_bytes)) {
+        const int64_t keep = env->l2_bytes / out_bytes / 4;
+        io.keep_words = static_cast<uint32_t>(keep < (int64_t(1) << 30) ? keep : (int64_t(1) << 30));
+    }
     const bool draws = (env->cfg.flags & GC_F_NOISE) && env->tab.noise_thr_nz;
     cudaError_t e = gc_launch_cell_packed_step(env->tab, io, env->d_packed_lut, draws, env->n_sm, st);
     if (e != cudaSuccess) return fail(GC_ERR_CUDA, "packed step kernel launch failed: %s", cudaGetErrorString(e));
@@ -224,9 +248,11 @@
     return GC_OK;
 }
 
-int launch_step(gc_env *env, const StepIO &io, cudaStream_t st)
+int launch_step(gc_env *env, StepIO io, cudaStream_t st)
 {
     if (io.end <= io.begin) return GC_OK;
+    const int C = env->cfg.n_cells;
+    set_sweep(env, io, 3 * C + 20 + (io.se_row ? C : 0) + (io.final_state ? C : 0));
     cudaError_t e;
     if (env->cfg.kind == GC_KIND_CELLULAR) {
         const bool draws = (env->cfg.flags & GC_F_NOISE) && env->tab.noise_thr_nz;
@@ -289,13 +315,15 @@
     if (cfg->device < 0 || cfg->device >= n_dev)
         return fail(GC_ERR_INVALID, "device %d not in [0, %d)", cfg->device, n_dev);
     GC_ON_DEVICE(cfg->device);
-    int n_sm = 0;
+    int n_sm = 0, l2 = 0;
     GC_CUDA(cudaDeviceGetAttribute(&n_sm, cudaDevAttrMultiProcessorCount, cfg->device));
+    GC_CUDA(cudaDeviceGetAttribute(&l2, cudaDevAttrL2CacheSize, cfg->device));
     gc_env *env = new (std::nothrow) gc_env();
     if (!env) return fail(GC_ERR_INVALID, "out of host memory");
     std::memset(env, 0, sizeof(*env));
     env->cfg = *cfg;
     env->n_sm = n_sm;
+    env->l2_bytes = l2;
     env->grid.dispersal_thr = threshold_of(cfg->dispersal_prob);
     env->grid.dispersal_thr_nz = env->grid.dispersal_thr != 0ull;
     env->grid.dispersal_thr_m1 = env->grid.dispersal_thr_nz ? static_cast<uint32_t>(env->grid.dispersal_thr - 1ull) : 0u;
@@ -489,6 +517,8 @@
 
 int64_t gc_launch_count(const gc_env *env) { return env ? env->launches : -1; }
 
+int64_t gc_reversed_launch_count(const gc_env *env) { return env ? env->reversed_launches : -1; }
+
 int gc_reset(gc_env *env, const uint8_t *mask, int8_t *state, int32_t *t, uint32_t *index, void *stream)
 {
     GC_NVTX("gc_reset");
@@ -589,14 +619,14 @@
     }();
     const int32_t passes = (graph_steps + n_slots - 1) / n_slots;
     cudaStream_t cap = env->hstream[0];
-    const int64_t launches = env->launches, step = env->global_step;
+    const int64_t launches = env->launches, step = env->global_step, reversed = env->reversed_launches;
     if (cudaStreamBeginCapture(cap, cudaStreamCaptureModeRelaxed) != cudaSuccess) { cudaGetLastError(); return nullptr; }
     int rc = GC_OK;
     for (int32_t p = 0; p < passes && rc == GC_OK; ++p)
         for (int32_t i = 0; i < n_slots && rc == GC_OK; ++i) rc = launch_bound(env, slots[i], cap);
     cudaGraph_t graph = nullptr;
     cudaError_t e = cudaStreamEndCapture(cap, &graph);
-    env->launches = launches; env->global_step = step;
+    env->launches = launches; env->global_step = step; env->reversed_launches = reversed;
     cudaGraphExec_t exec = nullptr;
     if (rc == GC_OK && e == cudaSuccess && graph) e = cudaGraphInstantiate(&exec, graph, 0);
     if (graph) cudaGraphDestroy(graph);
diff --git a/gym_cellular_b200/csrc/gc_cell_fast.cu b/gym_cellular_b200/csrc/gc_cell_fast.cu
--- a/gym_cellular_b200/csrc/gc_cell_fast.cu
+++ b/gym_cellular_b200/csrc/gc_cell_fast.cu
@@ -156,13 +156,14 @@
 
     __shared__ StepCounterShared s_ctr;
 
-    const uint32_t stride = gridDim.x * kThreads * kEPT, e_end = static_cast<uint32_t>(io.end);
+    const Sweep sweep = sweep_of(io);
+    const uint32_t wstride = gridDim.x * kThreads, e_end = static_cast<uint32_t>(io.end);
 #ifndef GC_PAIR_PREFETCH_WIDE
 #define GC_PAIR_PREFETCH_WIDE 0
 #endif
     constexpr bool PREFETCH = NG == 0 || GC_PAIR_PREFETCH_WIDE;
     constexpr int G0 = NG > 0 ? 4 : R;
-    uint32_t e0 = static_cast<uint32_t>(io.begin) + (blockIdx.x * kThreads + threadIdx.x) * kEPT;
+    uint32_t w = blockIdx.x * kThreads + threadIdx.x;
     constexpr int LUT_PER_THREAD = N_PAIR / kThreads;
     uint2 lut_pair[LUT_PER_THREAD], lut_single = make_uint2(0u, 0u);
 #pragma unroll
@@ -172,7 +173,8 @@
     pdl_wait();
     uint32_t ps[4], pa[4];
     int4 pt = make_int4(0, 0, 0, 0);
-    if constexpr (PREFETCH) if (e0 < e_end) {
+    if constexpr (PREFETCH) if (w < sweep.words) {
+        const uint32_t e0 = sweep_env(sweep, w);
         load_cells<G0>(io, 0, e0, ps, pa);
         pt = ld_stream_v4(io.t + e0);
     }
@@ -192,7 +194,8 @@
     uint32_t st_steps = 0, st_unsafe = 0, st_count = 0, st_trunc = 0;
     long long st_reward = 0;
 #pragma unroll 1
-    for (; e0 < e_end; e0 += stride) {
+    for (; w < sweep.words; w += wstride) {
+        const uint32_t e0 = sweep_env(sweep, w);
         const int rem = static_cast<int>(e_end - e0 < kEPT ? e_end - e0 : kEPT);
         const uint64_t gid0 = static_cast<uint64_t>(io.env_id_offset) + e0;
         const uint32_t gid_lo = static_cast<uint32_t>(gid0), gid_hi = static_cast<uint32_t>(gid0 >> 32);
@@ -204,9 +207,10 @@
             for (int i = 0; i < 4; ++i) { sa[i] = ps[i]; aa[i] = pa[i]; }
             t4 = pt;
             if (NG > 1) load_cells<4>(io, 4, e0, sb, ab); else if (NG == 1 && R > 0) load_cells<R>(io, 4, e0, sb, ab);
-            if (e0 + stride < e_end) {
-                load_cells<G0>(io, 0, e0 + stride, ps, pa);
-                pt = ld_stream_v4(io.t + (e0 + stride));
+            if (w + wstride < sweep.words) {
+                const uint32_t en = sweep_env(sweep, w + wstride);
+                load_cells<G0>(io, 0, en, ps, pa);
+                pt = ld_stream_v4(io.t + en);
             }
         } else {
             load_cells<4>(io, 0, e0, sa, aa);
diff --git a/gym_cellular_b200/csrc/gc_cell_packed.cu b/gym_cellular_b200/csrc/gc_cell_packed.cu
--- a/gym_cellular_b200/csrc/gc_cell_packed.cu
+++ b/gym_cellular_b200/csrc/gc_cell_packed.cu
@@ -34,6 +34,15 @@
 __host__ __device__ constexpr int packed_min_blocks(int c, int rng, bool extra)
 {
     return (rng != GC_RNG_NONE || extra || c == 15) ? (GC_PACKED_MINB < 3 ? GC_PACKED_MINB : 3) : GC_PACKED_MINB;
+}
+
+__device__ __forceinline__ void st_out_u32(void *p, uint32_t v, bool hot)
+{
+    if (hot) *reinterpret_cast<uint32_t *>(p) = v; else st_stream_u32(p, v);
+}
+__device__ __forceinline__ void st_out_v4(void *p, int4 v, bool hot)
+{
+    if (hot) *reinterpret_cast<int4 *>(p) = v; else st_stream_v4(p, v);
 }
 
 template <int C, int RNG, bool EXTRA>
@@ -42,7 +51,7 @@
                                             uint32_t gid_lo, uint32_t gid_hi, uint32_t step_counter,
                                             const uint32_t (&sw4)[kEPT], const uint32_t (&aw4)[kEPT], const int (&tin)[kEPT],
                                             uint32_t &st_steps, uint32_t &st_unsafe, uint32_t &st_count, uint32_t &st_trunc,
-                                            long long &st_reward, uint32_t (&nstate)[kEPT], int (&tn)[kEPT])
+                                            long long &st_reward, uint32_t (&nstate)[kEPT], int (&tn)[kEPT], bool hot = false)
 {
     constexpr int NP = C / 2;
     constexpr bool ODD = (C & 1) != 0;
@@ -140,17 +149,17 @@
         st_trunc += __popc(fw & 0x02020202u);
         st_count = add_bytes((fw >> 2) & 0x1F1F1F1Fu, st_count);
     }
-    st_stream_v4(io.state + e0, make_int4(nstate[0], nstate[1], nstate[2], nstate[3]));
-    st_stream_v4(io.t + e0, make_int4(tn[0], tn[1], tn[2], tn[3]));
-    st_stream_v4(io.reward + e0, make_int4(__float_as_int(rout[0]), __float_as_int(rout[1]),
-                                           __float_as_int(rout[2]), __float_as_int(rout[3])));
-    st_stream_u32(io.flags + e0, flags_w);
+    st_out_v4(io.state + e0, make_int4(nstate[0], nstate[1], nstate[2], nstate[3]), hot);
+    st_out_v4(io.t + e0, make_int4(tn[0], tn[1], tn[2], tn[3]), hot);
+    st_out_v4(io.reward + e0, make_int4(__float_as_int(rout[0]), __float_as_int(rout[1]),
+                                        __float_as_int(rout[2]), __float_as_int(rout[3])), hot);
+    st_out_u32(io.flags + e0, flags_w, hot);
     if (EXTRA) {
-        if (io.index) st_stream_v4(io.index + e0, make_int4(idx[0], idx[1], idx[2], idx[3]));
-        if (io.final_state) st_stream_v4(io.final_state + e0, make_int4(fin[0], fin[1], fin[2], fin[3]));
-        if (io.se_row) st_stream_v4(io.se_row + e0, make_int4(sew[0], sew[1], sew[2], sew[3]));
+        if (io.index) st_out_v4(io.index + e0, make_int4(idx[0], idx[1], idx[2], idx[3]), hot);
+        if (io.final_state) st_out_v4(io.final_state + e0, make_int4(fin[0], fin[1], fin[2], fin[3]), hot);
+        if (io.se_row) st_out_v4(io.se_row + e0, make_int4(sew[0], sew[1], sew[2], sew[3]), hot);
     } else if (io.index) {
-        st_stream_v4(io.index + e0, make_int4(nstate[0], nstate[1], nstate[2], nstate[3]));
+        st_out_v4(io.index + e0, make_int4(nstate[0], nstate[1], nstate[2], nstate[3]), hot);
     }
 }
 
@@ -168,8 +177,10 @@
     __shared__ StepCounterShared s_ctr;
     const uint32_t REP = 1u << REP_LOG2;
 
-    const uint32_t stride = gridDim.x * kPackThreads * kEPT, e_end = static_cast<uint32_t>(io.end);
-    uint32_t e0 = static_cast<uint32_t>(io.begin) + (blockIdx.x * kPackThreads + threadIdx.x) * kEPT;
+    const Sweep sweep = sweep_of(io);
+    const uint32_t hot_from = sweep.words > io.keep_words ? sweep.words - io.keep_words : 0u;
+    const uint32_t wstride = gridDim.x * kPackThreads, e_end = static_cast<uint32_t>(io.end);
+    uint32_t w = blockIdx.x * kPackThreads + threadIdx.x;
     for (int i = threadIdx.x; i < (N_PAIR << REP_LOG2); i += kPackThreads) s_pair[i] = lut[i >> REP_LOG2];
     for (int i = threadIdx.x; i < (N_SINGLE << REP_LOG2); i += kPackThreads) s_single[i] = lut[GC_PAIR_LUT_PAIRS + (i >> REP_LOG2)];
     if (EXTRA && io.se_row)
@@ -178,7 +189,8 @@
     pdl_launch_dependents();
     pdl_wait();
     int4 ps = make_int4(0, 0, 0, 0), pa = ps, pt = ps;
-    if (e0 < e_end) {
+    if (w < sweep.words) {
+        const uint32_t e0 = sweep_env(sweep, w);
         ps = ld_stream_v4(io.state + e0);
         pa = ld_stream_v4(io.actions + e0);
         pt = ld_stream_v4(io.t + e0);
@@ -194,22 +206,24 @@
 
     uint32_t st_steps = 0, st_unsafe = 0, st_count = 0, st_trunc = 0;
     long long st_reward = 0;
-    for (; e0 < e_end; e0 += stride) {
+    for (; w < sweep.words; w += wstride) {
+        const uint32_t e0 = sweep_env(sweep, w);
         const int rem = static_cast<int>(e_end - e0 < kEPT ? e_end - e0 : kEPT);
         const uint64_t gid0 = static_cast<uint64_t>(io.env_id_offset) + e0;
         const uint32_t gid_lo = static_cast<uint32_t>(gid0), gid_hi = static_cast<uint32_t>(gid0 >> 32);
         const uint32_t sw4[kEPT] = {(uint32_t)ps.x, (uint32_t)ps.y, (uint32_t)ps.z, (uint32_t)ps.w};
         const uint32_t aw4[kEPT] = {(uint32_t)pa.x, (uint32_t)pa.y, (uint32_t)pa.z, (uint32_t)pa.w};
         const int tin[kEPT] = {pt.x, pt.y, pt.z, pt.w};
-        if (e0 + stride < e_end) {
-            ps = ld_stream_v4(io.state + (e0 + stride));
-            pa = ld_stream_v4(io.actions + (e0 + stride));
-            pt = ld_stream_v4(io.t + (e0 + stride));
+        if (w + wstride < sweep.words) {
+            const uint32_t en = sweep_env(sweep, w + wstride);
+            ps = ld_stream_v4(io.state + en);
+            pa = ld_stream_v4(io.actions + en);
+            pt = ld_stream_v4(io.t + en);
         }
         uint32_t nstate[kEPT];
         int tn[kEPT];
         packed_word<C, RNG, EXTRA>(tab, io, s_se, pair_base, single_base, lut_mul, e0, rem, gid_lo, gid_hi, step_counter, sw4, aw4, tin,
-                                   st_steps, st_unsafe, st_count, st_trunc, st_reward, nstate, tn);
+                                   st_steps, st_unsafe, st_count, st_trunc, st_reward, nstate, tn, w >= hot_from);
     }
     if (io.stats) {
         const ThreadStats ts = {st_steps, st_unsafe, st_count, st_trunc, st_reward};
diff --git a/gym_cellular_b200/csrc/gc_cell_pair8.cu b/gym_cellular_b200/csrc/gc_cell_pair8.cu
--- a/gym_cellular_b200/csrc/gc_cell_pair8.cu
+++ b/gym_cellular_b200/csrc/gc_cell_pair8.cu
@@ -22,8 +22,8 @@
     __shared__ StepCounterShared s_ctr;
     const int C = tab.n_cells;
     const uint32_t ld = static_cast<uint32_t>(io.ld);
-    const uint32_t stride = gridDim.x * kThreads * kEPT, e_end = static_cast<uint32_t>(io.end);
-    uint32_t e0 = static_cast<uint32_t>(io.begin) + (blockIdx.x * kThreads + threadIdx.x) * kEPT;
+    const Sweep sweep = sweep_of(io);
+    const uint32_t wstride = gridDim.x * kThreads, e_end = static_cast<uint32_t>(io.end);
 
     if constexpr (!NOISE)
         for (int i = threadIdx.x; i < GC_PAIR8_PAIRS; i += kThreads) s_pair[i] = lut[i];
@@ -40,7 +40,8 @@
     uint32_t st_steps = 0, st_unsafe = 0, st_count = 0, st_trunc = 0;
     long long st_reward = 0;
 #pragma unroll 1
-    for (; e0 < e_end; e0 += stride) {
+    for (uint32_t w = blockIdx.x * kThreads + threadIdx.x; w < sweep.words; w += wstride) {
+        const uint32_t e0 = sweep_env(sweep, w);
         const int rem = static_cast<int>(e_end - e0 < kEPT ? e_end - e0 : kEPT);
         uint32_t sw[4] = {0, 0, 0, 0}, aw[4] = {0, 0, 0, 0};
 #pragma unroll
diff --git a/gym_cellular_b200/csrc/gc_device.cuh b/gym_cellular_b200/csrc/gc_device.cuh
--- a/gym_cellular_b200/csrc/gc_device.cuh
+++ b/gym_cellular_b200/csrc/gc_device.cuh
@@ -110,6 +110,23 @@
 }
 __device__ __forceinline__ int4 ld_stream_v4(const void *p) { return __ldcs(reinterpret_cast<const int4 *>(p)); }
 __device__ __forceinline__ void st_stream_v4(void *p, int4 v) { __stcs(reinterpret_cast<int4 *>(p), v); }
+
+struct Sweep {
+    uint32_t words;
+    uint32_t first, step;
+};
+
+template <class IO>
+__device__ __forceinline__ Sweep sweep_of(const IO &io)
+{
+    Sweep s;
+    s.words = static_cast<uint32_t>((io.end - io.begin + kEPT - 1) / kEPT);
+    s.first = static_cast<uint32_t>(io.begin) + (io.reverse ? (s.words - 1u) * kEPT : 0u);
+    s.step = io.reverse ? static_cast<uint32_t>(-kEPT) : static_cast<uint32_t>(kEPT);
+    return s;
+}
+__device__ __forceinline__ uint32_t sweep_env(const Sweep &s, uint32_t w) { return s.first + w * s.step; }
+
 
 struct ThreadStats {
     uint32_t steps, unsafe, count, truncated;
diff --git a/gym_cellular_b200/csrc/gc_grid.cu b/gym_cellular_b200/csrc/gc_grid.cu
--- a/gym_cellular_b200/csrc/gc_grid.cu
+++ b/gym_cellular_b200/csrc/gc_grid.cu
@@ -27,9 +27,9 @@
     __shared__ unsigned long long s_stats[5];
     __shared__ StepCounterShared s_ctr;
     const uint32_t ld = static_cast<uint32_t>(io.ld);
-    const uint32_t w_lo = blockIdx.x * kGridThreads, e_end = static_cast<uint32_t>(io.end);
-    const uint32_t stride = gridDim.x * kGridThreads * kEPT;
-    uint32_t e0 = static_cast<uint32_t>(io.begin) + (w_lo + threadIdx.x) * kEPT;
+    const Sweep sweep = sweep_of(io);
+    const uint32_t e_end = static_cast<uint32_t>(io.end), wstride = gridDim.x * kGridThreads;
+    uint32_t w = blockIdx.x * kGridThreads + threadIdx.x;
     constexpr int LUT_VEC = GC_GRID_LUT_ENTRIES / 4, LUT_PER_THREAD = (LUT_VEC + kGridThreads - 1) / kGridThreads;
     uint4 lut_reg[LUT_GLOBAL ? 1 : LUT_PER_THREAD];
     if (!LUT_GLOBAL) {
@@ -44,7 +44,8 @@
     pdl_wait();
     uint32_t p_s0 = 0, p_s1 = 0, p_a0 = 0, p_a1 = 0;
     int4 p_t = make_int4(0, 0, 0, 0);
-    if (e0 < e_end) {
+    if (w < sweep.words) {
+        const uint32_t e0 = sweep_env(sweep, w);
         p_s0 = ld_stream_u32(io.state + e0); p_s1 = ld_stream_u32(io.state + (ld + e0));
         p_a0 = ld_stream_u32(io.actions + e0); p_a1 = ld_stream_u32(io.actions + (ld + e0));
         p_t = ld_stream_v4(io.t + e0);
@@ -63,14 +64,15 @@
 
     const uint32_t step_counter = step_counter_arrive(io, &s_ctr);
     uint32_t st_count = 0, st_trunc = 0, st_reward = 0, bad_bits = 0;
-    for (; e0 < e_end; e0 += stride) {
+    for (; w < sweep.words; w += wstride) {
+        const uint32_t e0 = sweep_env(sweep, w);
         const int rem = static_cast<int>(e_end - e0 < kEPT ? e_end - e0 : kEPT);
         const uint64_t gid0 = static_cast<uint64_t>(io.env_id_offset) + e0;
         const uint32_t s0w = p_s0, s1w = p_s1;
         uint32_t a0w = p_a0, a1w = p_a1;
         const int4 t4 = p_t;
-        if (e0 + stride < e_end) {
-            const uint32_t en = e0 + stride;
+        if (w + wstride < sweep.words) {
+            const uint32_t en = sweep_env(sweep, w + wstride);
             p_s0 = ld_stream_u32(io.state + en); p_s1 = ld_stream_u32(io.state + (ld + en));
             p_a0 = ld_stream_u32(io.actions + en); p_a1 = ld_stream_u32(io.actions + (ld + en));
             p_t = ld_stream_v4(io.t + en);
diff --git a/gym_cellular_b200/csrc/gc_internal.h b/gym_cellular_b200/csrc/gc_internal.h
--- a/gym_cellular_b200/csrc/gc_internal.h
+++ b/gym_cellular_b200/csrc/gc_internal.h
@@ -34,6 +34,7 @@
     uint32_t *done_ctr;
     int32_t  episodic;
     int32_t  max_episode_steps;
+    int32_t  reverse;
 };
 
 struct ManyIO {
@@ -60,6 +61,8 @@
     const uint32_t *step_ctr;
     uint32_t *done_ctr;
     int32_t episodic, max_episode_steps;
+    int32_t reverse;
+    uint32_t keep_words;
 };
 
 struct PackedManyIO {
diff --git a/gym_cellular_b200/csrc/gc_kernels.cu b/gym_cellular_b200/csrc/gc_kernels.cu
--- a/gym_cellular_b200/csrc/gc_kernels.cu
+++ b/gym_cellular_b200/csrc/gc_kernels.cu
@@ -23,9 +23,10 @@
     uint32_t st_steps = 0, st_unsafe = 0, st_count = 0, st_trunc = 0;
     long long st_reward = 0;
     const uint32_t ld = static_cast<uint32_t>(io.ld);
-    const uint32_t stride = gridDim.x * kThreads * kEPT, e_end = static_cast<uint32_t>(io.end);
-    for (uint32_t e0 = static_cast<uint32_t>(io.begin) + (blockIdx.x * kThreads + threadIdx.x) * kEPT;
-         e0 < e_end; e0 += stride) {
+    const Sweep sweep = sweep_of(io);
+    const uint32_t wstride = gridDim.x * kThreads, e_end = static_cast<uint32_t>(io.end);
+    for (uint32_t w = blockIdx.x * kThreads + threadIdx.x; w < sweep.words; w += wstride) {
+        const uint32_t e0 = sweep_env(sweep, w);
         const int rem = static_cast<int>(e_end - e0 < kEPT ? e_end - e0 : kEPT);
         const uint64_t gid0 = static_cast<uint64_t>(io.env_id_offset) + e0;
         const uint32_t gid_lo = static_cast<uint32_t>(gid0), gid_hi = static_cast<uint32_t>(gid0 >> 32);
diff --git a/include/gym_cellular_b200.h b/include/gym_cellular_b200.h
--- a/include/gym_cellular_b200.h
+++ b/include/gym_cellular_b200.h
@@ -79,6 +79,7 @@
 int64_t gc_get_global_step(const gc_env *env);
 int gc_sync_global_step(gc_env *env, void *stream);
 int64_t gc_launch_count(const gc_env *env);
+int64_t gc_reversed_launch_count(const gc_env *env);
 
 int gc_reset(gc_env *env, const uint8_t *mask, int8_t *state, int32_t *t, uint32_t *index, void *stream);
 
```

New measurement: 87.88 billion, median of 6. 1.3% higher.
